# hasenbanck/opus-native

Measured on NVIDIA B200. Metric: concurrent_realtime_48k_streams_decoded, higher is better.
Workload: dtype u32+f32

## Files before the change

opus-native_b200/csrc/frame_warp.cuh:

```cuda
#pragma once
#include "imdct_warp.cuh"
#include "symbols.cuh"

namespace opn {

template <int C> struct WSmp;
template <> struct WSmp<1> {
    float a;
    __device__ __forceinline__ static WSmp ld(const float *p) { return WSmp{*p}; }
    __device__ __forceinline__ WSmp operator+(WSmp o) const { return WSmp{a + o.a}; }
    __device__ __forceinline__ WSmp scaled(float g) const { return WSmp{g * a}; }
};
template <> struct WSmp<2> {
    float a, b;
    __device__ __forceinline__ static WSmp ld(const float *p)
    {
        const float2 v = *reinterpret_cast<const float2 *>(p);
        return WSmp{v.x, v.y};
    }
    __device__ __forceinline__ WSmp operator+(WSmp o) const
    {
        const float2 r = p_add(make_float2(a, b), make_float2(o.a, o.b));
        return WSmp{r.x, r.y};
    }
// ... 55 lines not shown
        rows[i] = v.a;
        if constexpr (C == 2) rows[CHF + i] = v.b;
    }
    __device__ __forceinline__ S ld_hist(int i) const
    {
        int j = pos + i;
        if (j < 0) j += RING_SAMPLES;
        return S::ld(ring + (size_t)j * C);
    }
    __device__ __forceinline__ S ld(int i) const { return i >= 0 ? ld_row(i) : ld_hist(i); }
};

template <int C, int CHF, bool TS = false>
__device__ __forceinline__ void w_comb_ring(const FrameView<C, CHF> &V, int t0, int t1, int n, float g0, float g1, int tap0, int tap1,
                                            int overlap, int lane, const float *win_sq, const CombGains &kg)
{
    using S = WSmp<C>;
    if (g0 == 0.0f && g1 == 0.0f) return;
    t0 = max(t0, 15);
    t1 = max(t1, 15);
    const float g00 = kg.g00, g01 = kg.g01, g02 = kg.g02, g10 = kg.g10, g11 = kg.g11, g12 = kg.g12;
    if (fabsf(g0 - g1) < 1.1920929e-7f && t0 == t1 && tap0 == tap1) overlap = 0;
    const bool has0 = g0 != 0.0f, has1 = g1 != 0.0f;

    if (overlap > 0) {
        const int tmin = min(has0 ? t0 : 1 << 20, has1 ? t1 : 1 << 20);
        const int W = min(tmin - 2, 32);
        for (int base = 0; base < overlap; base += W) {
            const int i = base + lane;
            if (lane < W && i < overlap) {
                const float f = tab_ld<TS>(win_sq + i);
                S a[5], b[5];
#pragma unroll
                for (int k = 0; k < 5; k++) {
                    a[k] = has0 ? V.ld(i - t0 - 2 + k) : S{};
                    b[k] = has1 ? V.ld(i - t1 - 2 + k) : S{};
                }
                V.st_row(i, w_xfade<C>(V.ld_row(i), a, b, has0, has1, f, g00, g01, g02, g10, g11, g12));
            }
            __syncwarp();
        }
    }
    if (!has1) return;

    int at = overlap;
    {
        const int hend = max(at, min(n, t1 - 2));
        for (int base = at; base < hend; base += 128) {
#pragma unroll
            for (int e = 0; e < 4; e++) {
                const int i = base + lane + 32 * e;
                if (i < hend) {
                    int j = V.pos + i - t1 - 2;
                    if (j < 0) j += RING_SAMPLES;
                    if (j + 4 < RING_SAMPLES) {
                        const float *hp = V.ring + (size_t)j * C;
                        V.st_row(i, w_comb5<C>(V.ld_row(i), S::ld(hp + 4 * C), S::ld(hp + 3 * C), S::ld(hp + 2 * C), S::ld(hp + C), S::ld(hp), g10, g11, g12));
                    } else {
                        const int p = i - t1;
                        V.st_row(i, w_comb5<C>(V.ld_row(i), V.ld_hist(p + 2), V.ld_hist(p + 1), V.ld_hist(p), V.ld_hist(p - 1), V.ld_hist(p - 2),
                                               g10, g11, g12));
                    }
                }
            }
        }
        at = hend;
        __syncwarp();
    }
    const int W2 = min(t1 - 2, 128);
    const int rounds = (W2 + 31) >> 5;
    for (int base = at; base < n; base += W2) {
        const bool mixed = base - t1 - 2 < 0;
        for (int e = 0; e < rounds; e++) {
            const int l = lane + 32 * e, i = base + l;
            if (l < W2 && i < n) {
                const int p = i - t1;
                if (mixed)
                    V.st_row(i, w_comb5<C>(V.ld_row(i), V.ld(p + 2), V.ld(p + 1), V.ld(p), V.ld(p - 1), V.ld(p - 2), g10, g11, g12));
                else
                    V.st_row(i, w_comb5<C>(V.ld_row(i), V.ld_row(p + 2), V.ld_row(p + 1), V.ld_row(p), V.ld_row(p - 1), V.ld_row(p - 2), g10,
                                           g11, g12));
            }
        }
        __syncwarp();
    }
}

__device__ __forceinline__ void prefetch_l1(const void *p) { asm volatile("prefetch.global.L1 [%0];" ::"l"(p)); }
__device__ __forceinline__ void prefetch_l2(const void *p) { asm volatile("prefetch.global.L2 [%0];" ::"l"(p)); }

#ifndef OPN_FRAME_WARPS
#define OPN_FRAME_WARPS 5
#endif
#ifndef OPN_FRAME_CTAS
#define OPN_FRAME_CTAS 4
#endif
constexpr int FRAME_WARPS = OPN_FRAME_WARPS, FRAME_CTAS = OPN_FRAME_CTAS;
#ifndef OPN_STORE_UNROLL
#define OPN_STORE_UNROLL 3
#endif
constexpr int STORE_UNROLL = OPN_STORE_UNROLL;
__host__ __device__ constexpr size_t frame_warp_bytes(int lm, int channels) { return (size_t)channels * w_ch_floats(lm) * 4 + 16 + 48; }
__host__ __device__ constexpr size_t frame_smem_bytes(int lm, int channels, size_t blob_bytes)
{
    return 16 + blob_bytes + (size_t)FRAME_WARPS * frame_warp_bytes(lm, channels);
}

enum { FRAME_ROWS = 0, FRAME_SYNTH1 = 1, FRAME_SYNTH2 = 2 };
template <int LM, int C, int MODE, int CS = C>
__device__ __forceinline__ void frame_cta(const FrameArgs &A, uint32_t first_item, uint32_t item_end)
{
    constexpr bool EXPAND = MODE != FRAME_ROWS;
    constexpr int R = C > CS ? C : CS;
    static_assert(EXPAND || CS == C, "coefficient rows from memory are the decoder's channels already");
    extern __shared__ __align__(16) uint8_t smem[];
    constexpr int NF = 120 << LM;
    constexpr int CHF = w_ch_floats(LM);
    const int lane = threadIdx.x & 31, warp = threadIdx.x >> 5;
    uint64_t *tbar = reinterpret_cast<uint64_t *>(smem);
    const uint8_t *blob = smem + 16;
    const FBlobHdr H = g_tab.fblob_hdr[LM][CS - 1];
    float *o = reinterpret_cast<float *>(smem + 16 + H.total + (size_t)warp * frame_warp_bytes(LM, R));
    uint64_t *bar = reinterpret_cast<uint64_t *>(o + R * CHF);
    uint4 *stash = reinterpret_cast<uint4 *>(o + R * CHF + 4);

    if (threadIdx.x == 0) {
        mbar_init(tbar, 1);
        mbar_expect_tx(tbar, H.total);
        bulk_g2s(smem + 16, g_fblob[LM][CS - 1], H.total, tbar);
    }
    const uint32_t item = first_item + warp;
    const bool in_range = item < item_end;
    const uint32_t stream = in_range ? (A.stream_idx ? A.stream_idx[item] : item) : 0u;
    if constexpr (!EXPAND) {
        if (lane == 0 && in_range) {
            mbar_init(bar, 1);
            mbar_expect_tx(bar, C * NF * 4);
#pragma unroll
            for (int c = 0; c < C; c++) bulk_g2s(o + c * CHF, A.coef + ((size_t)stream * C + c) * NF, NF * 4, bar);
        }
    }
    const int32_t status = in_range ? A.status[stream] : -1;
    {
        uint4 v = make_uint4(0u, 0u, 0u, 0u);
        if (in_range) {
            if (lane == 0) v = A.hdr[stream];
            else if (lane == 1) v = *reinterpret_cast<const uint4 *>(A.pf + stream);
            else if (lane == 2) v.x = A.ring_pos[stream];
        }
        if (lane < 3) stash[lane] = v;
    }
    __syncwarp();
    const uint32_t hdr_x = stash[0].x;
    [[maybe_unused]] uint32_t ix0 = 0u, ix1 = 0u, ix2 = 0u;
    if constexpr (MODE == FRAME_SYNTH1) {
        if (in_range) {
            const uint32_t *ip = A.idx + (size_t)stream * SYNTH_MAX_ENTRIES;
            ix0 = __ldg(ip + lane);
            ix1 = __ldg(ip + 32 + lane);
            if (lane < SYNTH_MAX_ENTRIES - 64) ix2 = __ldg(ip + 64 + lane);
        }
    }
    float *carry_g = A.carry + (size_t)stream * C * 60;
    float4 carry = make_float4(0.f, 0.f, 0.f, 0.f);
    if (in_range && lane < 15 * C) carry = *reinterpret_cast<const float4 *>(carry_g + 4 * lane);
    float *ring = A.ring + (size_t)stream * RING_SAMPLES * C;
    if (in_range && status >= 0 && A.postfilter) {
        const int t_old = (int)stash[1].x, t_new = (hdr_x >> 1) & 1u ? (int)(hdr_x >> 16) : 0;
        const int pos0 = (int)stash[2].x;
        const int need = max(max(t_old, t_new), 15) + 2;
        for (int l = lane * (128 / (4 * C)); l < need + 128 / (4 * C); l += 32 * (128 / (4 * C))) {
            int j = pos0 - need + l;
            if (j >= pos0) j = pos0 - 1;
            if (j < 0) j += RING_SAMPLES;
            prefetch_l2(ring + (size_t)j * C);
        }
    }
    if constexpr (EXPAND) {
#pragma unroll
        for (int c = 0; c < R; c++)
            for (int i = lane; i < NF / 4; i += 32) reinterpret_cast<float4 *>(o + c * CHF)[i] = make_float4(0.f, 0.f, 0.f, 0.f);
    }
    __syncthreads();
    mbar_wait(tbar, 0);
    if (status < 0) {
        if (in_range && lane == 0 && A.result) A.result[stream] = status;
        if constexpr (!EXPAND) {
            if (in_range) mbar_wait(bar, 0);
        }
        return;
    }
    const float2 *t_long = reinterpret_cast<const float2 *>(blob + H.tp_long), *t_short = reinterpret_cast<const float2 *>(blob + H.tp_short);
    const float2 *t_tw = reinterpret_cast<const float2 *>(blob + H.tw);
    const float *t_win = reinterpret_cast<const float *>(blob + H.win), *t_winsq = reinterpret_cast<const float *>(blob + H.win_sq);
    const bool lost = status == ITEM_LOST;
    const int lmt = (LM > 0 && ((hdr_x >> 2) & 1u)) ? LM : 0;
    if constexpr (MODE == FRAME_SYNTH1) {
        if (!lost && !(hdr_x & 1u)) {
            const ExpandTables T{reinterpret_cast<const uint32_t *>(blob + H.pvq_u), reinterpret_cast<const uint2 *>(blob + H.pvq_cw),
                                 reinterpret_cast<const uint16_t *>(blob + H.pvq_row), blob + H.pvq_nmax,
                                 reinterpret_cast<const SynthEntry *>(blob + H.ent), blob + H.slots, (int)H.n_slots};
            w_expand<CS>(T, LM, (uint32_t)lane, [&](uint32_t e) {
                const int src = (int)(e & 31u);
                const uint32_t a = __shfl_sync(0xFFFFFFFFu, ix0, src), b2 = __shfl_sync(0xFFFFFFFFu, ix1, src), c2 = __shfl_sync(0xFFFFFFFFu, ix2, src);
                return e == 0xFFu ? 0u : e < 32u ? a : e < 64u ? b2 : c2;
            }, o, CHF, nullptr, lmt);
        }
        __syncwarp();
    } else if constexpr (MODE == FRAME_SYNTH2) {
        if (!lost && !(hdr_x & 1u)) {
            const ExpandTables T{g_tab.pvq_u_data, g_tab.pvq_cw_data, g_tab.pvq_u_row, g_tab.pvq_ev_nmax, nullptr, nullptr, 0};
            w_expand2<CS>(T, LM, (uint32_t)lane, A.parts + (size_t)stream * CELT2_MAX_PARTS, stash[0].w, A.bande + (size_t)stream * 42, o, CHF, nullptr, lmt);
        }
        __syncwarp();
    } else {
        mbar_wait(bar, 0);
    }
    if constexpr (CS == 1 && C == 2) {
        for (int i = lane; i < NF / 4; i += 32) reinterpret_cast<float4 *>(o + CHF)[i] = reinterpret_cast<const float4 *>(o)[i];
        __syncwarp();
    } else if constexpr (CS == 2 && C == 1) {
        for (int i = lane; i < NF / 4; i += 32) {
            const float4 a = reinterpret_cast<const float4 *>(o)[i], b = reinterpret_cast<const float4 *>(o + CHF)[i];
            reinterpret_cast<float4 *>(o)[i] = make_float4(0.5f * (a.x + b.x), 0.5f * (a.y + b.y), 0.5f * (a.z + b.z), 0.5f * (a.w + b.w));
        }
        __syncwarp();
    }
    if constexpr (LM > 0) {
        if ((hdr_x >> 2) & 1u) w_imdct<3, (1 << LM), C, true, EXPAND>(o, lane, carry, t_short, t_tw, t_win);
        else w_imdct<3 - LM, 1, C, true>(o, lane, carry, t_long, t_tw, t_win);
    } else {
        w_imdct<3, 1, C, true>(o, lane, carry, t_long, t_tw, t_win);
    }

    const uint4 hdr = stash[0];
    PfState old;
    {
        const uint4 q = stash[1];
        old.period = (int32_t)q.x;
        old.tapset = (int32_t)q.y;
        old.gain = __uint_as_float(q.z);
        old.pad = 0;
    }
    const uint32_t pos = stash[2].x;
    const int s_on = (hdr.x >> 1) & 1u, s_tapset = (hdr.x >> 4) & 15u, s_gain = (hdr.x >> 8) & 15u, s_period = hdr.x >> 16;
    int t1 = old.period, tap1 = old.tapset;
    float g1 = old.gain;
    if (!lost) {
        t1 = s_on ? s_period : 0;
        g1 = s_on ? 0.09375f * (float)(s_gain + 1) : 0.0f;
        tap1 = s_on ? s_tapset : 0;
    }
    const bool comb_on = A.postfilter && (old.gain != 0.0f || g1 != 0.0f);

    if (lane < 15 * C) {
        const int ch = (C == 2 && lane >= 15) ? 1 : 0;
        *reinterpret_cast<float4 *>(carry_g + 4 * lane) = *reinterpret_cast<const float4 *>(o + ch * CHF + NF + 4 * (lane - 15 * ch));
    }
    if (comb_on) {
        const FrameView<C, CHF> V{o, ring, (int)pos};
        w_comb_ring<C, CHF, true>(V, old.period, t1, NF, old.gain, g1, old.tapset, tap1, 120, lane, t_winsq,
                                  w_comb_gains(old.gain, g1, old.tapset, tap1));
        __syncwarp();
        if (A.hist_samples && lane == 0) atomicAdd(A.hist_samples, (unsigned long long)(C * (max(max(old.period, t1), 15) + 2)));
    }
    const uint32_t dense_off = (A.dense && A.dense_off) ? A.dense_off[item] : 0u;
    float *dense = A.dense ? A.dense + (size_t)stream * A.dense_stride + dense_off : nullptr;
    const float gain = A.gain;
    constexpr int VEC = C == 2 ? NF / 2 : NF / 4;
    constexpr int SPV = C == 2 ? 2 : 4;
    const int wrap_at = (int)(RING_SAMPLES - pos) / SPV;
    float4 *r0 = reinterpret_cast<float4 *>(ring + (size_t)pos * C);
    float4 *r1 = reinterpret_cast<float4 *>(ring) - wrap_at;
#pragma unroll STORE_UNROLL
    for (int i = lane; i < VEC; i += 32) {
        float4 v;
        if (C == 2) {
            const float2 a = *reinterpret_cast<const float2 *>(o + 2 * i), b = *reinterpret_cast<const float2 *>(o + CHF + 2 * i);
            v = make_float4(a.x, b.x, a.y, b.y);
        } else {
            v = *reinterpret_cast<const float4 *>(o + 4 * i);
        }
        (i < wrap_at ? r0 : r1)[i] = v;
        if (dense) {
            if (gain != 1.0f) { v.x *= gain; v.y *= gain; v.z *= gain; v.w *= gain; }
            reinterpret_cast<float4 *>(dense)[i] = v;
        }
    }
    if (lane == 0) {
        uint32_t np = pos + (uint32_t)NF;
        if (np >= RING_SAMPLES) np -= RING_SAMPLES;
        A.ring_pos[stream] = np;
        PfState nw;
        nw.period = t1;
        nw.tapset = tap1;
        nw.gain = g1;
        nw.pad = 0;
        A.pf[stream] = nw;
        if (A.result) A.result[stream] = NF;
        if (A.final_range) A.final_range[stream] = lost ? 0u : hdr.y;
        if (A.softclip_reset && !lost) *reinterpret_cast<float2 *>(A.softclip_reset + 2 * (size_t)stream) = make_float2(0.f, 0.f);
    }
}

template <int LM, int C, int MODE, int CS = C> __global__ void __launch_bounds__(32 * FRAME_WARPS, FRAME_CTAS) k_frame_w(FrameArgs A)
{
    frame_cta<LM, C, MODE, CS>(A, A.item0 + blockIdx.x * FRAME_WARPS, A.item_end);
}

template <int C, int MODE> __global__ void __launch_bounds__(32 * FRAME_WARPS, FRAME_CTAS) k_frame_mix(FrameArgs A)
{
    const MixPlan &P = *A.plan;
    const int g = A.group;
    const uint32_t c = blockIdx.x;
    if (c >= P.cta0[g][4]) return;
    const int j = (c >= P.cta0[g][1]) + (c >= P.cta0[g][2]) + (c >= P.cta0[g][3]), lm = 3 - j;
    const uint32_t first = P.start[g][lm] + (c - P.cta0[g][j]) * FRAME_WARPS, end = P.start[g][lm] + P.count[g][lm];
    switch (lm) {
    case 0: frame_cta<0, C, MODE>(A, first, end); break;
    case 1: frame_cta<1, C, MODE>(A, first, end); break;
    case 2: frame_cta<2, C, MODE>(A, first, end); break;
    default: frame_cta<3, C, MODE>(A, first, end); break;
    }
}

__global__ void __launch_bounds__(256) k_mix_key(MixArgs A)
{
    const uint32_t s = blockIdx.x * 256u + threadIdx.x;
    const bool on = s < A.n_streams;
    uint32_t key = MIX_NO_ITEM;
    int32_t err = 0;
    if (on) {
        const uint32_t len = A.lens[s];
        int lm = -1;
        if (len == 0u) {
            const uint32_t l = A.last_lm[s];
            lm = l != MIX_NO_ITEM ? (int)l : (A.capacity >= 960u ? 3 : A.capacity >= 480u ? 2 : A.capacity >= 240u ? 1 : 0);
        } else {
            const uint32_t toc = A.arena[A.offsets[s]];
            if ((toc & 0x80u) == 0u) err = OPN_ERR_UNIMPLEMENTED;
            else if ((toc & 0x3u) != 0u) err = OPN_ERR_UNIMPLEMENTED;
            else if (((toc & 0x4u) ? 2 : 1) != A.channels) err = OPN_ERR_UNIMPLEMENTED;
            else lm = (int)((toc >> 3) & 0x3u);
        }
        if (lm >= 0 && (120u << lm) > A.capacity) {
            err = OPN_ERR_FRAME_SIZE_TOO_SMALL;
            lm = -1;
        }
        if (lm >= 0) {
            uint32_t g = 0u;
            if (A.n_groups > 1) {
                const uint32_t G = (uint32_t)A.n_groups;
                g = (uint32_t)(((uint64_t)s * G) / A.n_streams);
                if (g + 1u < G && (uint32_t)(((uint64_t)A.n_streams * (g + 1u)) / G) <= s) g += 1u;
            }
            key = g * 4u + (uint32_t)lm;
            if (len > 1u) A.last_lm[s] = (uint8_t)lm;
        }
    }
    const uint32_t peers = __match_any_sync(0xFFFFFFFFu, key);
    uint32_t rank = 0u;
    if (key != MIX_NO_ITEM) {
        const int leader = __ffs(peers) - 1;
        uint32_t base = 0u;
// ... 82 lines not shown
```

opus-native_b200/csrc/host_runtime.cpp:

```cpp
#include <algorithm>
#include <cmath>
#include <cstdio>
#include <cstdlib>
#include <cstring>
#include <new>
#include <string>
#include <vector>

#include <nvtx3/nvToolsExt.h>

#include "opn_internal.h"
#include "celt2.cuh"

using namespace opn;

namespace {

thread_local std::string g_cuda_err;

int cuda_fail(cudaError_t e, const char *what)
{
    char buf[256];
    std::snprintf(buf, sizeof(buf), "%s: %s", what, cudaGetErrorString(e));
    g_cuda_err = buf;
    return OPN_ERR_CUDA;
}

#define CU(call)                                          \
    do {                                                  \
        cudaError_t e_ = (call);                          \
        if (e_ != cudaSuccess) return cuda_fail(e_, #call); \
    } while (0)

int lm_of_frame(size_t nf)
{
    switch (nf) {
    case 120: return 0;
    case 240: return 1;
    case 480: return 2;
    case 960: return 3;
    default: return -1;
    }
}

int select_device(int device)
{
    int n = 0;
    cudaError_t e = cudaGetDeviceCount(&n);
    if (e != cudaSuccess) return cuda_fail(e, "cudaGetDeviceCount");
    if (n == 0 || device < 0 || device >= n) return cuda_fail(cudaErrorInvalidDevice, "no such CUDA device");
    CU(cudaSetDevice(device));
    cudaDeviceProp p;
    CU(cudaGetDeviceProperties(&p, device));
    if (p.major < 10) {
        g_cuda_err = std::string("device '") + p.name + "' is not sm_100-class; libopusb200 ships sm_100a code only";
        return OPN_ERR_CUDA;
    }
    CU(upload_tables(device));
    return OPN_OK;
}

struct EventRing {
    static constexpr int N = 512;
    cudaEvent_t a[N], b[N];
    int used = 0;
    bool made = false;
    double ms = 0.0;
    uint64_t launches = 0;
    int make()
    {
        if (made) return OPN_OK;
        for (int i = 0; i < N; i++) {
            CU(cudaEventCreate(&a[i]));
            CU(cudaEventCreate(&b[i]));
        }
        made = true;
        return OPN_OK;
    }
    int resolve()
    {
        for (int i = 0; i < used; i++) {
            CU(cudaEventSynchronize(b[i]));
            float t = 0;
            CU(cudaEventElapsedTime(&t, a[i], b[i]));
            ms += t;
        }
        used = 0;
        return OPN_OK;
    }
    void destroy()
    {
        if (!made) return;
        for (int i = 0; i < N; i++) {
            cudaEventDestroy(a[i]);
            cudaEventDestroy(b[i]);
        }
        made = false;
    }
};

struct Item {
    uint32_t stream, offset, len, dense_off;
    int lm, wave;
    int cs;
};

}

struct opn_batch {
    int device = 0;
    uint32_t n = 0;
    opn_config cfg{};
    float gain = 1.0f;
    cudaStream_t stream = nullptr;
#ifndef OPN_NSETS
#define OPN_NSETS 8
#endif
#ifndef OPN_NRD
#define OPN_NRD 8
#endif
    static constexpr int NSETS = OPN_NSETS, NRD = OPN_NRD;
    cudaStream_t stream_rd[NRD] = {};
    cudaStream_t stream_ex = nullptr;
#ifndef OPN_FRAME_GROUPS
#define OPN_FRAME_GROUPS 3
#endif
    static constexpr int NGROUPS = OPN_FRAME_GROUPS;
    static constexpr uint32_t GROUP_MIN_ITEMS = 2048;
    cudaStream_t stream_fr[NGROUPS] = {};
    cudaEvent_t ev_fr[NSETS][NGROUPS] = {};
    cudaEvent_t ev_sw = nullptr;
    cudaEvent_t ev_tm[NGROUPS] = {};
    bool fr_pending[NGROUPS] = {};
    int fr_last_set[NGROUPS] = {};
    cudaEvent_t ev_k1[NSETS] = {};
    bool k1_recorded[NSETS] = {};
    bool k1_grouped[NSETS] = {};
    cudaEvent_t ev_rd[NSETS] = {};
    cudaEvent_t ev_ex[NSETS] = {};
    cudaEvent_t ev_in = nullptr;
    static constexpr int MAX_CHUNKS = 8;
    cudaStream_t stream_up = nullptr, stream_dn = nullptr;
    cudaEvent_t ev_chunk[MAX_CHUNKS] = {};
    int set = 0;
    bool unfused = false;
    float *d_carry = nullptr, *d_ring = nullptr, *d_coef[NSETS] = {};
    uint32_t *d_ring_pos = nullptr, *d_final = nullptr, *d_idx[NSETS] = {};
    PfState *d_pf = nullptr;
    uint4 *d_hdr[NSETS] = {};
    int32_t *d_status[NSETS] = {};
    Celt2Part *d_parts[NSETS] = {};
    int16_t *d_bande[NSETS] = {};
    struct Staging {
        uint8_t *d_arena = nullptr;
        size_t arena_cap = 0;
        uint32_t *d_items = nullptr, *h_items = nullptr;
        size_t items_cap = 0;
        float *d_dense = nullptr;
        size_t dense_cap = 0;
        void *d_conv = nullptr;
        size_t conv_cap = 0, conv_esize = 0;
        int32_t *d_cliplen = nullptr, *h_cliplen = nullptr;
        uint32_t *d_trans = nullptr, *h_trans = nullptr;
        cudaEvent_t done = nullptr;
        bool pending = false;
    } stg[2];
    int stg_next = 0;
    float *d_softclip = nullptr;
    uint8_t *d_last_lm = nullptr, *d_mix_key = nullptr;
    uint32_t *d_mix_rank = nullptr;
    uint32_t *d_mix_items[NSETS] = {};
    uint8_t *d_mix_lm[NSETS] = {};
    MixPlan *d_mix_plan[NSETS] = {};
    cudaEvent_t ev_mix[NSETS] = {};
    bool silk = false;
    SilkState d_silk{};
    SilkRec *d_silk_rec[NSETS] = {};
    std::vector<uint8_t> silk_cs;
    unsigned long long *d_hist_samples = nullptr;
    std::vector<int32_t> last_nf, bandwidth, last_duration, have_mode;
    bool timing = false;
    EventRing ev[3];
    uint64_t launches[3] = {0, 0, 0};
};

namespace {

struct Range {
    explicit Range(const char *name) { nvtxRangePushA(name); }
    ~Range() { nvtxRangePop(); }
    Range(const Range &) = delete;
    Range &operator=(const Range &) = delete;
};

int batch_alloc_staging(opn_batch *b, opn_batch::Staging &g, size_t arena_bytes, size_t n_items, size_t dense_floats, size_t conv_esize)
{
    if (!g.done) CU(cudaEventCreateWithFlags(&g.done, cudaEventDisableTiming));
    if (arena_bytes > g.arena_cap) {
        if (g.d_arena) cudaFree(g.d_arena);
        g.arena_cap = arena_bytes + arena_bytes / 4 + 256;
        CU(cudaMalloc(&g.d_arena, g.arena_cap));
    }
    if (n_items > g.items_cap) {
        if (g.d_items) cudaFree(g.d_items);
        if (g.h_items) cudaFreeHost(g.h_items);
        g.items_cap = n_items + n_items / 4 + 64;
        CU(cudaMalloc(&g.d_items, g.items_cap * 4 * sizeof(uint32_t)));
        CU(cudaMallocHost(&g.h_items, g.items_cap * 4 * sizeof(uint32_t)));
    }
    if (dense_floats > g.dense_cap) {
        if (g.d_dense) cudaFree(g.d_dense);
        g.dense_cap = dense_floats;
        CU(cudaMalloc(&g.d_dense, (size_t)b->n * (g.dense_cap + (b->silk ? 240 * (size_t)b->cfg.channels : 0)) * sizeof(float)));
    }
    if (conv_esize && (g.dense_cap > g.conv_cap || conv_esize > g.conv_esize)) {
        if (g.d_conv) cudaFree(g.d_conv);
        g.d_conv = nullptr;
        g.conv_cap = g.dense_cap;
        g.conv_esize = std::max(conv_esize, g.conv_esize);
        CU(cudaMalloc(&g.d_conv, (size_t)b->n * g.conv_cap * g.conv_esize));
    }
    if (conv_esize && !g.d_cliplen) {
        CU(cudaMalloc(&g.d_cliplen, (size_t)b->n * sizeof(int32_t)));
        CU(cudaMallocHost(&g.h_cliplen, (size_t)b->n * sizeof(int32_t)));
    }
    return OPN_OK;
}

int timed_launch(opn_batch *b, int kind, cudaError_t (*fn)(opn_batch *, const void *), const void *args)
{
    EventRing &r = b->ev[kind];
    if (b->timing) {
        if (r.used == EventRing::N) {
            int rc = r.resolve();
            if (rc) return rc;
        }
        CU(cudaEventRecord(r.a[r.used], b->stream));
    }
    CU(fn(b, args));
    if (b->timing) {
        CU(cudaEventRecord(r.b[r.used], b->stream));
        r.used++;
        r.launches++;
    }
    b->launches[kind]++;
    return OPN_OK;
}

cudaError_t do_rangedec(opn_batch *b, const void *a)
{
    const SymbolArgs &s = *static_cast<const SymbolArgs *>(a);
    return b->cfg.bitstream == OPN_BITSTREAM_SYNTH_CELT_2 ? launch_celt2_rangedec(s, b->stream) : launch_synth_rangedec(s, b->stream);
}
cudaError_t do_expand(opn_batch *b, const void *a) { return launch_synth_expand(*static_cast<const SymbolArgs *>(a), b->stream); }
bool frame_grouped(const opn_batch *b, const FrameArgs &m)
{
    return !b->unfused && opn_batch::NGROUPS > 1 && m.n_items >= opn_batch::GROUP_MIN_ITEMS && !m.stream_idx;
}
uint32_t group_first(uint32_t n, int g, int G) { return (uint32_t)((uint64_t)n * (uint32_t)g / (uint32_t)G); }
int mix_groups(const opn_batch *b) { return (opn_batch::NGROUPS > 1 && b->n >= opn_batch::GROUP_MIN_ITEMS) ? opn_batch::NGROUPS : 1; }
cudaError_t do_frame(opn_batch *b, const void *a)
{
    FrameArgs m = *static_cast<const FrameArgs *>(a);
    if (m.plan) {
        const int G = mix_groups(b);
        if (G == 1) return launch_frame_mix(m, b->n, b->stream);
        cudaError_t e = cudaEventRecord(b->ev_sw, b->stream);
        for (int g = 0; g < G && e == cudaSuccess; g++) {
            cudaStream_t st = g == 0 ? b->stream : b->stream_fr[g];
            if (g > 0) e = cudaStreamWaitEvent(st, b->ev_sw, 0);
            m.group = g;
            if (e == cudaSuccess) e = launch_frame_mix(m, group_first(b->n, g + 1, G) - group_first(b->n, g, G), st);
            if (g > 0 && e == cudaSuccess) e = cudaEventRecord(b->ev_tm[g], st);
            if (g > 0 && e == cudaSuccess) e = cudaStreamWaitEvent(b->stream, b->ev_tm[g], 0);
        }
        return e;
    }
    if (!frame_grouped(b, m)) return launch_frame(m, b->stream);
    cudaError_t e = cudaEventRecord(b->ev_sw, b->stream);
    const uint32_t n_items = m.n_items;
    for (int g = 0; g < opn_batch::NGROUPS && e == cudaSuccess; g++) {
        cudaStream_t st = g == 0 ? b->stream : b->stream_fr[g];
        if (g > 0) e = cudaStreamWaitEvent(st, b->ev_sw, 0);
        m.item0 = (uint32_t)((uint64_t)n_items * g / opn_batch::NGROUPS);
        m.item_end = (uint32_t)((uint64_t)n_items * (g + 1) / opn_batch::NGROUPS);
        if (e == cudaSuccess) e = launch_frame(m, st);
        if (g > 0 && e == cudaSuccess) e = cudaEventRecord(b->ev_tm[g], st);
        if (g > 0 && e == cudaSuccess) e = cudaStreamWaitEvent(b->stream, b->ev_tm[g], 0);
    }
    return e;
}

int join_groups(opn_batch *b)
{
    for (int g = 1; g < opn_batch::NGROUPS; g++)
        if (b->fr_pending[g]) {
            CU(cudaStreamWaitEvent(b->stream, b->ev_fr[b->fr_last_set[g]][g], 0));
            b->fr_pending[g] = false;
        }
    return OPN_OK;
}

int sync_pipeline(opn_batch *b)
{
    for (int q = 0; q < opn_batch::NRD; q++) CU(cudaStreamSynchronize(b->stream_rd[q]));
    CU(cudaStreamSynchronize(b->stream_ex));
    for (int g = 1; g < opn_batch::NGROUPS; g++) {
        CU(cudaStreamSynchronize(b->stream_fr[g]));
        b->fr_pending[g] = false;
    }
    CU(cudaStreamSynchronize(b->stream_up));
    CU(cudaStreamSynchronize(b->stream));
    CU(cudaStreamSynchronize(b->stream_dn));
    return OPN_OK;
}

int run_bucket(opn_batch *b, const uint8_t *d_arena, const uint32_t *d_offsets, const uint32_t *d_lens,
               const uint32_t *d_stream_idx, const uint32_t *d_dense_off, uint32_t n_items, int lm, int has_toc,
               uint32_t pkt_cap, float *dense, size_t dense_stride, int32_t *d_result, int inputs_on, bool softclip_reset,
               int stream_channels = 0)
{
    Range nv("opn: step (range decode + frame kernel)");
    if (stream_channels == 0) stream_channels = b->cfg.channels;
    if (stream_channels != b->cfg.channels && b->unfused) return OPN_ERR_UNIMPLEMENTED;
    const int p = b->set;
    b->set = (p + 1) % opn_batch::NSETS;
    cudaStream_t srd = b->stream_rd[p % opn_batch::NRD];
    SymbolArgs s{};
    s.arena = d_arena;
    s.offsets = d_offsets;
    s.lens = d_lens;
    s.stream_idx = d_stream_idx;
    s.n_items = n_items;
    s.lm = lm;
    s.channels = stream_channels;
    s.has_toc = has_toc;
    s.side = nullptr;
    s.hdr = b->d_hdr[p];
    s.status = b->d_status[p];
    s.coef = b->unfused ? b->d_coef[p] : nullptr;
    s.y_out = nullptr;
    s.idx = b->d_idx[p];
    s.pkt_cap = pkt_cap;
    s.parts = b->d_parts[p];
    s.bande = b->d_bande[p];
    s.side2 = nullptr;
    const bool celt2 = b->cfg.bitstream == OPN_BITSTREAM_SYNTH_CELT_2;
    int rc;
    if (b->timing) {
        if (inputs_on == 2) {
            CU(cudaEventRecord(b->ev_in, b->stream_up));
            CU(cudaStreamWaitEvent(b->stream, b->ev_in, 0));
        }
        rc = timed_launch(b, 0, do_rangedec, &s);
        if (rc) return rc;
        if (b->unfused) {
            rc = timed_launch(b, 2, do_expand, &s);
            if (rc) return rc;
        }
    } else {
        if (inputs_on == 1) {
            CU(cudaEventRecord(b->ev_in, b->stream));
            CU(cudaStreamWaitEvent(srd, b->ev_in, 0));
        } else if (inputs_on == 2) {
            CU(cudaEventRecord(b->ev_in, b->stream_up));
            CU(cudaStreamWaitEvent(srd, b->ev_in, 0));
        }
        if (b->k1_recorded[p]) {
            CU(cudaStreamWaitEvent(srd, b->ev_k1[p], 0));
            if (b->k1_grouped[p])
                for (int g = 1; g < opn_batch::NGROUPS; g++) CU(cudaStreamWaitEvent(srd, b->ev_fr[p][g], 0));
        }
        CU(celt2 ? launch_celt2_rangedec(s, srd) : launch_synth_rangedec(s, srd));
        CU(cudaEventRecord(b->ev_rd[p], srd));
        b->launches[0]++;
        if (b->unfused) {
            CU(cudaStreamWaitEvent(b->stream_ex, b->ev_rd[p], 0));
            CU(launch_synth_expand(s, b->stream_ex));
            CU(cudaEventRecord(b->ev_ex[p], b->stream_ex));
            CU(cudaStreamWaitEvent(b->stream, b->ev_ex[p], 0));
            b->launches[2]++;
        } else {
            CU(cudaStreamWaitEvent(b->stream, b->ev_rd[p], 0));
        }
    }
    FrameArgs m{};
    m.coef = b->unfused ? b->d_coef[p] : nullptr;
    m.idx = celt2 ? nullptr : b->d_idx[p];
    m.parts = celt2 ? b->d_parts[p] : nullptr;
    m.bande = b->d_bande[p];
    m.hdr = b->d_hdr[p];
    m.status = b->d_status[p];
    m.stream_idx = d_stream_idx;
    m.dense_off = d_dense_off;
    m.n_items = n_items;
    m.item0 = 0;
    m.item_end = n_items;
    m.lm = lm;
    m.channels = b->cfg.channels;
    m.stream_channels = stream_channels;
    m.postfilter = b->cfg.postfilter;
    m.carry = b->d_carry;
    m.ring = b->d_ring;
    m.ring_pos = b->d_ring_pos;
    m.pf = b->d_pf;
    m.dense = dense;
    m.dense_stride = dense_stride;
    m.gain = b->gain;
    m.result = d_result;
    m.final_range = b->d_final;
    m.softclip_reset = softclip_reset ? b->d_softclip : nullptr;
    m.hist_samples = b->timing ? b->d_hist_samples : nullptr;
    const bool grouped = !b->timing && frame_grouped(b, m);
    if (b->timing) {
        rc = join_groups(b);
        if (rc) return rc;
        rc = timed_launch(b, 1, do_frame, &m);
        if (rc) return rc;
        if (frame_grouped(b, m)) b->launches[1] += opn_batch::NGROUPS - 1;
    } else if (!grouped) {
        rc = join_groups(b);
        if (rc) return rc;
        CU(launch_frame(m, b->stream));
        b->launches[1]++;
    } else {
        CU(cudaEventRecord(b->ev_sw, b->stream));
        for (int g = 0; g < opn_batch::NGROUPS; g++) {
            cudaStream_t st = g == 0 ? b->stream : b->stream_fr[g];
            if (g > 0) {
                if (!b->fr_pending[g]) CU(cudaStreamWaitEvent(st, b->ev_sw, 0));
                CU(cudaStreamWaitEvent(st, b->ev_rd[p], 0));
            }
            m.item0 = (uint32_t)((uint64_t)n_items * g / opn_batch::NGROUPS);
            m.item_end = (uint32_t)((uint64_t)n_items * (g + 1) / opn_batch::NGROUPS);
            CU(launch_frame(m, st));
            b->launches[1]++;
            if (g > 0) {
                CU(cudaEventRecord(b->ev_fr[p][g], st));
                b->fr_pending[g] = true;
                b->fr_last_set[g] = p;
            }
        }
    }
    CU(cudaEventRecord(b->ev_k1[p], b->stream));
    b->k1_recorded[p] = true;
    b->k1_grouped[p] = grouped;
    return OPN_OK;
}

cudaError_t do_silk_rangedec(opn_batch *b, const void *a) { return launch_silk_rangedec(*static_cast<const SilkArgs *>(a), b->stream); }
cudaError_t do_silk_frame(opn_batch *b, const void *a) { return launch_silk_frame(*static_cast<const SilkArgs *>(a), b->stream); }

int run_silk_bucket(opn_batch *b, const uint8_t *d_arena, const uint32_t *d_offsets, const uint32_t *d_lens, const uint32_t *d_stream_idx,
                    const uint32_t *d_dense_off, uint32_t n_items, int frame_ms, int has_toc, int bandwidth, int stream_channels,
                    float *dense, size_t dense_stride, int32_t *d_result, int inputs_on, bool softclip_reset, int fec = 0)
{
    Range nv("opn: SILK step (range decode + frame kernel)");
    if (!b->silk) return OPN_ERR_UNIMPLEMENTED;
    const int p = b->set;
    b->set = (p + 1) % opn_batch::NSETS;
    cudaStream_t srd = b->stream_rd[p % opn_batch::NRD];
    SilkArgs a{};
    a.arena = d_arena;
    a.offsets = d_offsets;
    a.lens = d_lens;
    a.stream_idx = d_stream_idx;
    a.n_items = n_items;
    a.frame_ms = frame_ms;
    a.stream_channels = stream_channels;
    a.channels = b->cfg.channels;
    a.has_toc = has_toc;
    a.bandwidth = bandwidth;
    a.fec = fec;
    a.rec = b->d_silk_rec[p];
    a.hdr = b->d_hdr[p];
    a.status = b->d_status[p];
    a.st = b->d_silk;
    a.ring = b->d_ring;
    a.ring_pos = b->d_ring_pos;
    a.dense = dense;
    a.dense_stride = dense_stride;
    a.dense_off = d_dense_off;
    a.gain = b->gain;
    a.result = d_result;
    a.final_range = b->d_final;
    a.softclip_reset = softclip_reset ? b->d_softclip : nullptr;
    const bool grouped = !b->timing && opn_batch::NGROUPS > 1 && !d_stream_idx && n_items == b->n && n_items >= opn_batch::GROUP_MIN_ITEMS;
    int rc = OPN_OK;
    if (!grouped) rc = join_groups(b);
    if (rc) return rc;
    if (b->timing) {
        if (inputs_on == 2) {
            CU(cudaEventRecord(b->ev_in, b->stream_up));
            CU(cudaStreamWaitEvent(b->stream, b->ev_in, 0));
        }
        rc = timed_launch(b, 0, do_silk_rangedec, &a);
        if (rc) return rc;
        rc = timed_launch(b, 1, do_silk_frame, &a);
        if (rc) return rc;
    } else {
        if (inputs_on == 1) {
            CU(cudaEventRecord(b->ev_in, b->stream));
            CU(cudaStreamWaitEvent(srd, b->ev_in, 0));
        } else if (inputs_on == 2) {
            CU(cudaEventRecord(b->ev_in, b->stream_up));
            CU(cudaStreamWaitEvent(srd, b->ev_in, 0));
        }
        if (b->k1_recorded[p]) {
            CU(cudaStreamWaitEvent(srd, b->ev_k1[p], 0));
            if (b->k1_grouped[p])
                for (int g = 1; g < opn_batch::NGROUPS; g++) CU(cudaStreamWaitEvent(srd, b->ev_fr[p][g], 0));
        }
        CU(launch_silk_rangedec(a, srd));
        CU(cudaEventRecord(b->ev_rd[p], srd));
        b->launches[0]++;
        if (!grouped) {
            CU(cudaStreamWaitEvent(b->stream, b->ev_rd[p], 0));
            CU(launch_silk_frame(a, b->stream));
            b->launches[1]++;
        } else {
            CU(cudaEventRecord(b->ev_sw, b->stream));
            for (int g = 0; g < opn_batch::NGROUPS; g++) {
                cudaStream_t st = g == 0 ? b->stream : b->stream_fr[g];
                if (g > 0 && !b->fr_pending[g]) CU(cudaStreamWaitEvent(st, b->ev_sw, 0));
                CU(cudaStreamWaitEvent(st, b->ev_rd[p], 0));
                a.item0 = group_first(n_items, g, opn_batch::NGROUPS);
                a.item_end = group_first(n_items, g + 1, opn_batch::NGROUPS);
                CU(launch_silk_frame(a, st));
                b->launches[1]++;
                if (g > 0) {
                    CU(cudaEventRecord(b->ev_fr[p][g], st));
                    b->fr_pending[g] = true;
                    b->fr_last_set[g] = p;
                }
            }
        }
    }
    CU(cudaEventRecord(b->ev_k1[p], b->stream));
    b->k1_recorded[p] = true;
    b->k1_grouped[p] = grouped;
    return OPN_OK;
}

int mix_alloc(opn_batch *b)
{
    if (b->d_last_lm) return OPN_OK;
    const size_t n = b->n, cap = mix_item_cap(b->n);
    CU(cudaMalloc(&b->d_mix_key, n));
    CU(cudaMalloc(&b->d_mix_rank, n * sizeof(uint32_t)));
    for (int q = 0; q < opn_batch::NSETS; q++) {
        CU(cudaMalloc(&b->d_mix_items[q], 3 * cap * sizeof(uint32_t)));
        CU(cudaMalloc(&b->d_mix_lm[q], cap));
        CU(cudaMalloc(&b->d_mix_plan[q], sizeof(MixPlan)));
        CU(cudaEventCreateWithFlags(&b->ev_mix[q], cudaEventDisableTiming));
    }
    uint8_t *p = nullptr;
    CU(cudaMalloc(&p, n));
    CU(cudaMemsetAsync(p, MIX_NO_ITEM, n, b->stream_ex));
    b->d_last_lm = p;
    return OPN_OK;
}

int run_mixed(opn_batch *b, const uint8_t *d_arena, const uint32_t *d_offsets, const uint32_t *d_lens, size_t capacity, float *dense,
              size_t dense_stride, int32_t *d_result, int inputs_on, bool softclip_reset)
{
    if (b->unfused) return OPN_ERR_UNIMPLEMENTED;
    Range nv("opn: mixed-frame step (bucketing + range decode + frame kernel)");
    int rc = mix_alloc(b);
    if (rc) return rc;
    const int p = b->set;
    b->set = (p + 1) % opn_batch::NSETS;
    cudaStream_t srd = b->stream_rd[p % opn_batch::NRD];
    const uint32_t cap = mix_item_cap(b->n);
    const int G = mix_groups(b);
    MixArgs x{};
    x.arena = d_arena;
    x.offsets = d_offsets;
    x.lens = d_lens;
    x.n_streams = b->n;
    x.channels = b->cfg.channels;
    x.n_groups = G;
    x.capacity = (uint32_t)std::min<size_t>(capacity, 1u << 20);
    x.last_lm = b->d_last_lm;
    x.key = b->d_mix_key;
    x.rank = b->d_mix_rank;
    x.plan = b->d_mix_plan[p];
    x.item_offsets = b->d_mix_items[p];
    x.item_lens = b->d_mix_items[p] + cap;
    x.item_stream = b->d_mix_items[p] + 2 * (size_t)cap;
    x.item_lm = b->d_mix_lm[p];
    x.result = d_result;
    SymbolArgs s{};
    s.arena = d_arena;
    s.offsets = x.item_offsets;
    s.lens = x.item_lens;
    s.stream_idx = x.item_stream;
    s.item_lm = x.item_lm;
    s.n_items = cap;
    s.lm = 0;
    s.channels = b->cfg.channels;
    s.has_toc = 1;
    s.hdr = b->d_hdr[p];
    s.status = b->d_status[p];
    s.idx = b->d_idx[p];
    s.pkt_cap = 1280u;
    s.parts = b->d_parts[p];
    s.bande = b->d_bande[p];
    const bool celt2 = b->cfg.bitstream == OPN_BITSTREAM_SYNTH_CELT_2;
    FrameArgs m{};
    m.idx = celt2 ? nullptr : b->d_idx[p];
    m.parts = celt2 ? b->d_parts[p] : nullptr;
    m.bande = b->d_bande[p];
    m.hdr = b->d_hdr[p];
    m.status = b->d_status[p];
    m.stream_idx = x.item_stream;
    m.n_items = cap;
    m.channels = b->cfg.channels;
    m.postfilter = b->cfg.postfilter;
    m.carry = b->d_carry;
    m.ring = b->d_ring;
    m.ring_pos = b->d_ring_pos;
    m.pf = b->d_pf;
    m.dense = dense;
    m.dense_stride = dense_stride;
    m.gain = b->gain;
    m.result = d_result;
    m.final_range = b->d_final;
    m.softclip_reset = softclip_reset ? b->d_softclip : nullptr;
    m.hist_samples = b->timing ? b->d_hist_samples : nullptr;
    m.plan = b->d_mix_plan[p];
    if (b->timing) {
        rc = join_groups(b);
        if (rc) return rc;
        CU(cudaStreamSynchronize(b->stream_ex));
        CU(launch_mix_plan(x, b->stream));
        b->launches[2] += 2;
        rc = timed_launch(b, 0, do_rangedec, &s);
        if (rc) return rc;
        rc = timed_launch(b, 1, do_frame, &m);
        if (rc) return rc;
        b->launches[1] += G - 1;
    } else {
        cudaStream_t sx = b->stream_ex;
        if (inputs_on == 1) {
            CU(cudaEventRecord(b->ev_in, b->stream));
            CU(cudaStreamWaitEvent(sx, b->ev_in, 0));
        }
        if (b->k1_recorded[p]) {
            CU(cudaStreamWaitEvent(sx, b->ev_k1[p], 0));
            if (b->k1_grouped[p])
                for (int g = 1; g < opn_batch::NGROUPS; g++) CU(cudaStreamWaitEvent(sx, b->ev_fr[p][g], 0));
        }
        CU(launch_mix_plan(x, sx));
        b->launches[2] += 2;
        CU(cudaEventRecord(b->ev_mix[p], sx));
        CU(cudaStreamWaitEvent(srd, b->ev_mix[p], 0));
        CU(celt2 ? launch_celt2_rangedec(s, srd) : launch_synth_rangedec(s, srd));
        CU(cudaEventRecord(b->ev_rd[p], srd));
        b->launches[0]++;
        if (G == 1) {
            rc = join_groups(b);
            if (rc) return rc;
            CU(cudaStreamWaitEvent(b->stream, b->ev_rd[p], 0));
            CU(launch_frame_mix(m, b->n, b->stream));
            b->launches[1]++;
        } else {
            CU(cudaEventRecord(b->ev_sw, b->stream));
            for (int g = 0; g < G; g++) {
                cudaStream_t st = g == 0 ? b->stream : b->stream_fr[g];
                if (g > 0 && !b->fr_pending[g]) CU(cudaStreamWaitEvent(st, b->ev_sw, 0));
                CU(cudaStreamWaitEvent(st, b->ev_rd[p], 0));
                m.group = g;
                CU(launch_frame_mix(m, group_first(b->n, g + 1, G) - group_first(b->n, g, G), st));
                b->launches[1]++;
                if (g > 0) {
                    CU(cudaEventRecord(b->ev_fr[p][g], st));
                    b->fr_pending[g] = true;
                    b->fr_last_set[g] = p;
                }
            }
        }
    }
    CU(cudaEventRecord(b->ev_k1[p], b->stream));
    b->k1_recorded[p] = true;
    b->k1_grouped[p] = !b->timing && G > 1;
    return OPN_OK;
}

void plc_frames(size_t frame_size, int32_t last_nf, std::vector<uint32_t> &out)
{
    size_t done = 0;
    while (done < frame_size) {
        size_t a = std::min(frame_size - done, (size_t)last_nf);
        if (a > 960) a = 960;
        else if (a < 960) {
            if (a > 480) a = 480;
            else if (a > 240 && a < 480) a = 240;
        }
        out.push_back((uint32_t)a);
        done += a;
    }
}

}

extern "C" {

const char *opn_strerror(int code)
{
    switch (code) {
    case OPN_OK: return "ok";
    case OPN_ERR_BAD_ARG: return "bad arguments";
    case OPN_ERR_BUFFER_TOO_SMALL: return "buffer is too small";
    case OPN_ERR_INTERNAL: return "internal error";
    case OPN_ERR_INVALID_PACKET: return "invalid packet";
    case OPN_ERR_FRAME_SIZE_TOO_SMALL: return "the frame size is too small for the packet";
    case OPN_ERR_UNIMPLEMENTED: return "not implemented (the reference crate stubs this path too)";
    case OPN_ERR_CUDA: return "CUDA error";
    default: return "unknown error";
    }
}

const char *opn_last_cuda_error(void) { return g_cuda_err.c_str(); }

int opn_device_count(void)
{
    int n = 0;
    if (cudaGetDeviceCount(&n) != cudaSuccess) return 0;
    return n;
}

void *opn_host_alloc(size_t bytes)
{
    void *p = nullptr;
    if (bytes == 0 || cudaMallocHost(&p, bytes) != cudaSuccess) {
        cudaGetLastError();
        return nullptr;
    }
    return p;
}

void opn_host_free(void *p)
{
    if (p) cudaFreeHost(p);
}

int opn_host_register(void *p, size_t bytes)
{
    if (!p || bytes == 0) return OPN_ERR_BAD_ARG;
    CU(cudaHostRegister(p, bytes, cudaHostRegisterPortable));
    return OPN_OK;
}

int opn_host_unregister(void *p)
{
    if (!p) return OPN_ERR_BAD_ARG;
    CU(cudaHostUnregister(p));
    return OPN_OK;
}

int opn_batch_create(int device, uint32_t n_streams, const opn_config *cfg, opn_batch **out)
{
    if (!out || !cfg || n_streams == 0) return OPN_ERR_BAD_ARG;
    if (cfg->channels < 1 || cfg->channels > 2) return OPN_ERR_BAD_ARG;
    if (cfg->bitstream & ~(OPN_BITSTREAM_CELT_MASK | OPN_BITSTREAM_SYNTH_SILK_1)) return OPN_ERR_BAD_ARG;
    const int32_t celt_bitstream = cfg->bitstream & OPN_BITSTREAM_CELT_MASK;
    if (celt_bitstream != OPN_BITSTREAM_OPUS && celt_bitstream != OPN_BITSTREAM_SYNTH_CELT_1 && celt_bitstream != OPN_BITSTREAM_SYNTH_CELT_2)
        return OPN_ERR_BAD_ARG;
    switch (cfg->fs_hz) {
    case 48000: break;
    case 8000: case 12000: case 16000: case 24000: return OPN_ERR_UNIMPLEMENTED;
    default: return OPN_ERR_BAD_ARG;
    }
    int rc = select_device(device);
    if (rc) return rc;
    if (kernels_frame_groups() != OPN_FRAME_GROUPS) return OPN_ERR_INTERNAL;
    opn_batch *b = new (std::nothrow) opn_batch();
    if (!b) return OPN_ERR_INTERNAL;
    b->device = device;
    b->n = n_streams;
    b->cfg = *cfg;
    b->cfg.bitstream = celt_bitstream;
    b->silk = (cfg->bitstream & OPN_BITSTREAM_SYNTH_SILK_1) != 0;
    b->gain = host_gain_from_q8(cfg->gain_q8);
    const char *uf = std::getenv("OPN_UNFUSED_EXPAND");
    b->unfused = uf && uf[0] == '1' && celt_bitstream == OPN_BITSTREAM_SYNTH_CELT_1;
    const size_t n = n_streams, C = (size_t)cfg->channels;
    cudaError_t e = cudaStreamCreateWithFlags(&b->stream, cudaStreamNonBlocking);
    {
        const char *pr = std::getenv("OPN_RD_PRIORITY");
        const bool high = pr ? pr[0] == '1' : celt_bitstream == OPN_BITSTREAM_SYNTH_CELT_2;
        int lo_p = 0, hi_p = 0;
        if (high) cudaDeviceGetStreamPriorityRange(&lo_p, &hi_p);
        for (int q = 0; q < opn_batch::NRD && e == cudaSuccess; q++)
            e = cudaStreamCreateWithPriority(&b->stream_rd[q], cudaStreamNonBlocking, high ? hi_p : 0);
    }
    for (int q = 0; q < opn_batch::NSETS && e == cudaSuccess; q++) {
        e = cudaEventCreateWithFlags(&b->ev_rd[q], cudaEventDisableTiming);
        if (e == cudaSuccess) e = cudaEventCreateWithFlags(&b->ev_ex[q], cudaEventDisableTiming);
        if (e == cudaSuccess) e = cudaEventCreateWithFlags(&b->ev_k1[q], cudaEventDisableTiming);
        for (int g = 1; g < opn_batch::NGROUPS && e == cudaSuccess; g++) e = cudaEventCreateWithFlags(&b->ev_fr[q][g], cudaEventDisableTiming);
        if (e == cudaSuccess) e = cudaMalloc(&b->d_idx[q], n * 72 * sizeof(uint32_t));
        if (e == cudaSuccess && b->unfused) e = cudaMalloc(&b->d_coef[q], n * C * 960 * sizeof(float));
        if (e == cudaSuccess) e = cudaMalloc(&b->d_hdr[q], n * sizeof(uint4));
        if (e == cudaSuccess && celt_bitstream == OPN_BITSTREAM_SYNTH_CELT_2) e = cudaMalloc(&b->d_parts[q], n * CELT2_MAX_PARTS * sizeof(Celt2Part));
        if (e == cudaSuccess && b->silk) e = cudaMalloc(&b->d_silk_rec[q], n * 2 * sizeof(SilkRec));
        if (e == cudaSuccess && celt_bitstream == OPN_BITSTREAM_SYNTH_CELT_2) e = cudaMalloc(&b->d_bande[q], n * 42 * sizeof(int16_t));
        if (e == cudaSuccess) e = cudaMalloc(&b->d_status[q], n * sizeof(int32_t));
    }
    if (e == cudaSuccess) e = cudaStreamCreateWithFlags(&b->stream_ex, cudaStreamNonBlocking);
    for (int g = 1; g < opn_batch::NGROUPS && e == cudaSuccess; g++) e = cudaStreamCreateWithFlags(&b->stream_fr[g], cudaStreamNonBlocking);
    if (e == cudaSuccess) e = cudaEventCreateWithFlags(&b->ev_sw, cudaEventDisableTiming);
    for (int g = 1; g < opn_batch::NGROUPS && e == cudaSuccess; g++) e = cudaEventCreateWithFlags(&b->ev_tm[g], cudaEventDisableTiming);
    if (e == cudaSuccess) e = cudaEventCreateWithFlags(&b->ev_in, cudaEventDisableTiming);
    if (e == cudaSuccess) e = cudaStreamCreateWithFlags(&b->stream_up, cudaStreamNonBlocking);
    if (e == cudaSuccess) e = cudaStreamCreateWithFlags(&b->stream_dn, cudaStreamNonBlocking);
    for (int q = 0; q < opn_batch::MAX_CHUNKS && e == cudaSuccess; q++) e = cudaEventCreateWithFlags(&b->ev_chunk[q], cudaEventDisableTiming);
    if (e == cudaSuccess) e = cudaMalloc(&b->d_carry, n * C * 60 * sizeof(float));
    if (e == cudaSuccess) e = cudaMalloc(&b->d_ring, n * C * RING_SAMPLES * sizeof(float));
    if (e == cudaSuccess) e = cudaMalloc(&b->d_ring_pos, n * sizeof(uint32_t));
    if (e == cudaSuccess) e = cudaMalloc(&b->d_final, n * sizeof(uint32_t));
    if (e == cudaSuccess) e = cudaMalloc(&b->d_pf, n * sizeof(PfState));
    if (e == cudaSuccess) e = cudaMalloc(&b->d_softclip, n * 2 * sizeof(float));
    if (b->silk) {
        if (e == cudaSuccess) e = cudaMalloc(&b->d_silk.slpc, n * 2 * 16 * sizeof(int32_t));
        if (e == cudaSuccess) e = cudaMalloc(&b->d_silk.hist, n * 2 * SILK_HIST * sizeof(int32_t));
        if (e == cudaSuccess) e = cudaMalloc(&b->d_silk.a_q12, n * 2 * 16 * sizeof(int16_t));
        if (e == cudaSuccess) e = cudaMalloc(&b->d_silk.gain, n * 2 * sizeof(int32_t));
        if (e == cudaSuccess) e = cudaMalloc(&b->d_silk.rs, n * 2 * 8 * sizeof(float));
        if (e == cudaSuccess) e = cudaMalloc(&b->d_silk.fs, n * 2);
    }
    if (e == cudaSuccess) e = cudaMalloc(&b->d_hist_samples, sizeof(unsigned long long));
    if (e == cudaSuccess) e = cudaMemset(b->d_hist_samples, 0, sizeof(unsigned long long));
    if (e != cudaSuccess) {
        opn_batch_destroy(b);
        return cuda_fail(e, "opn_batch_create: allocation");
    }
    b->last_nf.assign(n, 120);
    b->bandwidth.assign(n, -1);
    b->last_duration.assign(n, -1);
    b->have_mode.assign(n, 0);
    b->silk_cs.assign(n, 0);
    *out = b;
    rc = opn_batch_reset(b);
    if (rc) {
        opn_batch_destroy(b);
        *out = nullptr;
    }
    return rc;
}

void opn_batch_destroy(opn_batch *b)
{
    if (!b) return;
    cudaSetDevice(b->device);
    for (int q = 0; q < opn_batch::NRD; q++)
        if (b->stream_rd[q]) cudaStreamSynchronize(b->stream_rd[q]);
    for (cudaStream_t st : {b->stream_ex, b->stream_up, b->stream, b->stream_dn})
        if (st) cudaStreamSynchronize(st);
    for (int g = 1; g < opn_batch::NGROUPS; g++)
        if (b->stream_fr[g]) {
            cudaStreamSynchronize(b->stream_fr[g]);
            cudaStreamDestroy(b->stream_fr[g]);
        }
    if (b->ev_sw) cudaEventDestroy(b->ev_sw);
    for (int g = 1; g < opn_batch::NGROUPS; g++)
        if (b->ev_tm[g]) cudaEventDestroy(b->ev_tm[g]);
    for (int q = 0; q < opn_batch::NSETS; q++) {
        for (int g = 1; g < opn_batch::NGROUPS; g++)
            if (b->ev_fr[q][g]) cudaEventDestroy(b->ev_fr[q][g]);
        if (b->ev_rd[q]) cudaEventDestroy(b->ev_rd[q]);
        if (b->ev_ex[q]) cudaEventDestroy(b->ev_ex[q]);
        if (b->ev_k1[q]) cudaEventDestroy(b->ev_k1[q]);
        cudaFree(b->d_idx[q]);
        cudaFree(b->d_coef[q]);
        cudaFree(b->d_hdr[q]);
        cudaFree(b->d_parts[q]);
        cudaFree(b->d_bande[q]);
        cudaFree(b->d_status[q]);
        cudaFree(b->d_silk_rec[q]);
    }
    cudaFree(b->d_silk.slpc);
    cudaFree(b->d_silk.hist);
    cudaFree(b->d_silk.a_q12);
    cudaFree(b->d_silk.gain);
    cudaFree(b->d_silk.rs);
    cudaFree(b->d_silk.fs);
    if (b->ev_in) cudaEventDestroy(b->ev_in);
    for (int q = 0; q < opn_batch::MAX_CHUNKS; q++)
        if (b->ev_chunk[q]) cudaEventDestroy(b->ev_chunk[q]);
    for (cudaStream_t st : {b->stream_ex, b->stream_up, b->stream_dn})
        if (st) cudaStreamDestroy(st);
    for (int q = 0; q < opn_batch::NRD; q++)
        if (b->stream_rd[q]) cudaStreamDestroy(b->stream_rd[q]);
    for (int k = 0; k < 3; k++) b->ev[k].destroy();
    cudaFree(b->d_carry);
    cudaFree(b->d_ring);
    cudaFree(b->d_ring_pos);
    cudaFree(b->d_final);
    cudaFree(b->d_pf);
    cudaFree(b->d_softclip);
    cudaFree(b->d_last_lm);
    cudaFree(b->d_mix_key);
    cudaFree(b->d_mix_rank);
    for (int q = 0; q < opn_batch::NSETS; q++) {
        cudaFree(b->d_mix_items[q]);
        cudaFree(b->d_mix_lm[q]);
        cudaFree(b->d_mix_plan[q]);
        if (b->ev_mix[q]) cudaEventDestroy(b->ev_mix[q]);
    }
    cudaFree(b->d_hist_samples);
    for (auto &g : b->stg) {
        cudaFree(g.d_arena);
        cudaFree(g.d_items);
        cudaFree(g.d_dense);
        cudaFree(g.d_conv);
        cudaFree(g.d_cliplen);
        cudaFree(g.d_trans);
        if (g.h_trans) cudaFreeHost(g.h_trans);
        if (g.h_cliplen) cudaFreeHost(g.h_cliplen);
        if (g.h_items) cudaFreeHost(g.h_items);
        if (g.done) cudaEventDestroy(g.done);
    }
    if (b->stream) cudaStreamDestroy(b->stream);
    delete b;
}

int opn_batch_reset(opn_batch *b)
{
    if (!b) return OPN_ERR_BAD_ARG;
    CU(cudaSetDevice(b->device));
    int rc = sync_pipeline(b);
    if (rc) return rc;
    for (auto &g : b->stg) g.pending = false;
    const size_t n = b->n, C = (size_t)b->cfg.channels;
    CU(cudaMemsetAsync(b->d_carry, 0, n * C * 60 * sizeof(float), b->stream));
    CU(cudaMemsetAsync(b->d_ring, 0, n * C * RING_SAMPLES * sizeof(float), b->stream));
    CU(cudaMemsetAsync(b->d_ring_pos, 0, n * sizeof(uint32_t), b->stream));
    CU(cudaMemsetAsync(b->d_final, 0, n * sizeof(uint32_t), b->stream));
    CU(cudaMemsetAsync(b->d_pf, 0, n * sizeof(PfState), b->stream));
    for (int q = 0; q < opn_batch::NSETS; q++) {
        CU(cudaMemsetAsync(b->d_hdr[q], 0, n * sizeof(uint4), b->stream));
        CU(cudaMemsetAsync(b->d_status[q], 0, n * sizeof(int32_t), b->stream));
        b->k1_recorded[q] = false;
    }
    b->set = 0;
    CU(cudaMemsetAsync(b->d_softclip, 0, n * 2 * sizeof(float), b->stream));
    if (b->d_last_lm) CU(cudaMemsetAsync(b->d_last_lm, MIX_NO_ITEM, n, b->stream));
    if (b->silk) {
        CU(cudaMemsetAsync(b->d_silk.slpc, 0, n * 2 * 16 * sizeof(int32_t), b->stream));
        CU(cudaMemsetAsync(b->d_silk.hist, 0, n * 2 * SILK_HIST * sizeof(int32_t), b->stream));
        CU(cudaMemsetAsync(b->d_silk.a_q12, 0, n * 2 * 16 * sizeof(int16_t), b->stream));
        CU(cudaMemsetAsync(b->d_silk.gain, 0, n * 2 * sizeof(int32_t), b->stream));
        CU(cudaMemsetAsync(b->d_silk.rs, 0, n * 2 * 8 * sizeof(float), b->stream));
        CU(cudaMemsetAsync(b->d_silk.fs, 0, n * 2, b->stream));
    }
    CU(cudaStreamSynchronize(b->stream));
    std::fill(b->last_nf.begin(), b->last_nf.end(), 120);
    std::fill(b->bandwidth.begin(), b->bandwidth.end(), -1);
    std::fill(b->last_duration.begin(), b->last_duration.end(), -1);
    std::fill(b->have_mode.begin(), b->have_mode.end(), 0);
    std::fill(b->silk_cs.begin(), b->silk_cs.end(), 0);
    return OPN_OK;
}

static int batch_decode_host(opn_batch *b, const uint8_t *arena, const uint32_t *offsets, const uint32_t *lens, float *pcm,
                             size_t pcm_stride, size_t frame_size, int32_t *results, uint32_t flags,
                             void *pcm_conv = nullptr, int sample_format = OPN_SAMPLE_F32)
{
    Range nv_call("opn: host-buffer call (parse, upload, decode, download)");
    const uint32_t n = b->n;
    const int C = b->cfg.channels;
    size_t arena_end = 0, items_ub = 0;
    for (uint32_t i = 0; i < n; i++) {
        if (lens[i] == 0) {
            items_ub += frame_size / 120;
            continue;
        }
        arena_end = std::max(arena_end, (size_t)offsets[i] + lens[i]);
        const int fc = opn_packet_frame_count(arena + offsets[i], lens[i]);
        items_ub += (fc > 0 ? (size_t)fc : 1) + (b->silk ? 1 : 0);
    }
    const size_t dense_stride = (frame_size * (size_t)C + 3) & ~(size_t)3;
    const int slot = b->stg_next;
    b->stg_next ^= 1;
    opn_batch::Staging &g = b->stg[slot];
    if (g.pending) {
        CU(cudaEventSynchronize(g.done));
        g.pending = false;
    }
    const size_t esize = pcm_conv ? opn_sample_size(sample_format) : 0;
    if (pcm_conv && esize == 0) return OPN_ERR_BAD_ARG;
    int rc = batch_alloc_staging(b, g, arena_end, items_ub, dense_stride, esize);
    if (rc) return rc;
    const bool want_pcm = (pcm != nullptr || pcm_conv != nullptr) && !(flags & OPN_FLAG_NO_PCM_COPY);
    if (arena_end) CU(cudaMemcpyAsync(g.d_arena, arena, arena_end, cudaMemcpyHostToDevice, b->stream_up));

    const uint32_t n_chunks = std::min<uint32_t>(opn_batch::MAX_CHUNKS, std::max<uint32_t>(1u, n / 1024u));
    const size_t cap = g.items_cap;
    std::vector<Item> items;
    items.reserve(items_ub / n_chunks + 64);
    std::vector<int32_t> res(n, 0);
    std::vector<uint32_t> plc;
    std::vector<uint32_t> silk_resets, celt_resets;
    size_t kbase = 0;
    for (uint32_t ch = 0; ch < n_chunks; ch++) {
        const uint32_t s0 = (uint32_t)((uint64_t)n * ch / n_chunks), s1 = (uint32_t)((uint64_t)n * (ch + 1) / n_chunks);
        Range nv_chunk("opn: chunk (host parse -> enqueue)");
        items.clear();
        silk_resets.clear();
        celt_resets.clear();
        bool any_gap = false;
        uint32_t max_len = 8;
        for (uint32_t i = s0; i < s1; i++) {
            const uint32_t len = lens[i];
            auto conceal = [&](uint32_t i, size_t n_samples, uint32_t at0, int w0) -> int {
                if (!b->have_mode[i]) return -1;
                plc.clear();
                plc_frames(n_samples, b->last_nf[i], plc);
                uint32_t at = at0;
                int w = w0;
                if (b->have_mode[i] == 1 + OPN_MODE_SILK) {
                    bool ok = b->silk;
                    for (uint32_t a : plc) ok = ok && (a == 480 || a == 960);
                    if (!ok) return -2;
                    for (uint32_t a : plc) {
                        items.push_back(Item{i, 0u, 0u, at * (uint32_t)C, 8 + (a == 960 ? 1 : 0), w++, (int)b->silk_cs[i]});
// ... 544 lines not shown
    CU(cudaMemcpy(out, dOut.p, (size_t)n_packets * n_ops * sizeof(opn_op_out), cudaMemcpyDeviceToHost));
    if (y_out && y_stride) CU(cudaMemcpy(y_out, dY.p, (size_t)n_packets * y_stride * 4, cudaMemcpyDeviceToHost));
    return OPN_OK;
}

int opn_op_imdct_tdac(int device, const float *input, size_t in_stride, float *output, size_t out_stride, uint32_t n_rows,
                      int shift, int stride, int blocks)
{
    if (!input || !output || n_rows == 0 || shift < 0 || shift > 3 || blocks < 1 || stride != blocks) return OPN_ERR_BAD_ARG;
    const size_t n2 = 960u >> shift;
    if (n2 * (size_t)blocks > 960 || in_stride < n2 * (size_t)blocks || out_stride < n2 * (size_t)blocks + 60) return OPN_ERR_BAD_ARG;
    int rc = select_device(device);
    if (rc) return rc;
    DevBuf dI, dO;
    CU(dI.alloc((size_t)n_rows * in_stride * 4));
    CU(dO.alloc((size_t)n_rows * out_stride * 4));
    CU(cudaMemcpy(dI.p, input, (size_t)n_rows * in_stride * 4, cudaMemcpyHostToDevice));
    CU(cudaMemcpy(dO.p, output, (size_t)n_rows * out_stride * 4, cudaMemcpyHostToDevice));
    CU(launch_op_imdct(dI.as<float>(), in_stride, dO.as<float>(), out_stride, n_rows, shift, blocks, nullptr));
    CU(cudaDeviceSynchronize());
    CU(cudaMemcpy(output, dO.p, (size_t)n_rows * out_stride * 4, cudaMemcpyDeviceToHost));
    return OPN_OK;
}

static int comb_args_ok(size_t offset, size_t n, uint32_t n_rows, const int32_t *p, const float *g, size_t row_stride,
                        size_t overlap)
{
    if (!p || !g || n_rows == 0 || offset + n > row_stride || overlap > 120 || overlap > n) return 0;
    for (uint32_t r = 0; r < n_rows; r++) {
        const int32_t t0 = std::max(p[4 * r], 15), t1 = std::max(p[4 * r + 1], 15);
        if (t0 > 1022 || t1 > 1022 || p[4 * r + 2] < 0 || p[4 * r + 2] > 2 || p[4 * r + 3] < 0 || p[4 * r + 3] > 2) return 0;
        if ((size_t)std::max(t0, t1) + 2 > offset) return 0;
    }
    return 1;
}

int opn_op_comb_filter_inplace(int device, float *y, size_t row_stride, size_t y_offset, size_t n, uint32_t n_rows,
                               const int32_t *params4, const float *gains2, size_t overlap)
{
    if (!y || !comb_args_ok(y_offset, n, n_rows, params4, gains2, row_stride, overlap)) return OPN_ERR_BAD_ARG;
    int rc = select_device(device);
    if (rc) return rc;
    DevBuf dY, dP, dG;
    CU(dY.alloc((size_t)n_rows * row_stride * 4));
    CU(dP.alloc((size_t)n_rows * 16));
    CU(dG.alloc((size_t)n_rows * 8));
    CU(cudaMemcpy(dY.p, y, (size_t)n_rows * row_stride * 4, cudaMemcpyHostToDevice));
    CU(cudaMemcpy(dP.p, params4, (size_t)n_rows * 16, cudaMemcpyHostToDevice));
    CU(cudaMemcpy(dG.p, gains2, (size_t)n_rows * 8, cudaMemcpyHostToDevice));
    CU(launch_op_comb_inplace(dY.as<float>(), row_stride, (int)y_offset, (int)n, n_rows, dP.as<int32_t>(), dG.as<float>(),
                              (int)overlap, nullptr));
    CU(cudaDeviceSynchronize());
    CU(cudaMemcpy(y, dY.p, (size_t)n_rows * row_stride * 4, cudaMemcpyDeviceToHost));
    return OPN_OK;
}

int opn_op_comb_filter(int device, float *y, const float *x, size_t row_stride, size_t offset, size_t n, uint32_t n_rows,
                       const int32_t *params4, const float *gains2, size_t overlap)
{
    if (!y || !x || !comb_args_ok(offset, n, n_rows, params4, gains2, row_stride, overlap)) return OPN_ERR_BAD_ARG;
    int rc = select_device(device);
    if (rc) return rc;
    DevBuf dY, dX, dP, dG;
    CU(dY.alloc((size_t)n_rows * row_stride * 4));
    CU(dX.alloc((size_t)n_rows * row_stride * 4));
    CU(dP.alloc((size_t)n_rows * 16));
    CU(dG.alloc((size_t)n_rows * 8));
    CU(cudaMemcpy(dY.p, y, (size_t)n_rows * row_stride * 4, cudaMemcpyHostToDevice));
    CU(cudaMemcpy(dX.p, x, (size_t)n_rows * row_stride * 4, cudaMemcpyHostToDevice));
    CU(cudaMemcpy(dP.p, params4, (size_t)n_rows * 16, cudaMemcpyHostToDevice));
    CU(cudaMemcpy(dG.p, gains2, (size_t)n_rows * 8, cudaMemcpyHostToDevice));
    CU(launch_op_comb(dY.as<float>(), dX.as<float>(), row_stride, (int)offset, (int)n, n_rows, dP.as<int32_t>(), dG.as<float>(),
                      (int)overlap, nullptr));
    CU(cudaDeviceSynchronize());
    CU(cudaMemcpy(y, dY.p, (size_t)n_rows * row_stride * 4, cudaMemcpyDeviceToHost));
    return OPN_OK;
}

int opn_op_pcm_soft_clip(int device, float *pcm, size_t row_stride, size_t row_len, int channels, uint32_t n_rows,
                         float *softclip_mem)
{
    if (!pcm || !softclip_mem || n_rows == 0 || channels < 1 || row_len > row_stride) return OPN_ERR_BAD_ARG;
    int rc = select_device(device);
    if (rc) return rc;
    DevBuf dP, dM;
    CU(dP.alloc((size_t)n_rows * row_stride * 4));
    CU(dM.alloc((size_t)n_rows * channels * 4));
    CU(cudaMemcpy(dP.p, pcm, (size_t)n_rows * row_stride * 4, cudaMemcpyHostToDevice));
    CU(cudaMemcpy(dM.p, softclip_mem, (size_t)n_rows * channels * 4, cudaMemcpyHostToDevice));
    CU(launch_op_soft_clip(dP.as<float>(), row_stride, row_len, channels, n_rows, dM.as<float>(), nullptr));
    CU(cudaDeviceSynchronize());
    CU(cudaMemcpy(pcm, dP.p, (size_t)n_rows * row_stride * 4, cudaMemcpyDeviceToHost));
    CU(cudaMemcpy(softclip_mem, dM.p, (size_t)n_rows * channels * 4, cudaMemcpyDeviceToHost));
    return OPN_OK;
}

int opn_op_smooth_fade(int device, const float *in1, const float *in2, float *out, size_t row_stride, size_t overlap, int channels,
                       int32_t fs_hz, uint32_t n_rows)
{
    if (!in1 || !in2 || !out || n_rows == 0 || channels < 1 || channels > 2 || overlap * (size_t)channels > row_stride) return OPN_ERR_BAD_ARG;
    if (fs_hz <= 0 || 48000 % fs_hz != 0 || (overlap > 0 && (overlap - 1) * (size_t)(48000 / fs_hz) >= 120)) return OPN_ERR_BAD_ARG;
    int rc = select_device(device);
    if (rc) return rc;
    const size_t bytes = (size_t)n_rows * row_stride * 4;
    DevBuf d1, d2;
    CU(d1.alloc(bytes));
    CU(d2.alloc(bytes));
    CU(cudaMemcpy(d1.p, in1, bytes, cudaMemcpyHostToDevice));
    CU(cudaMemcpy(d2.p, in2, bytes, cudaMemcpyHostToDevice));
    CU(launch_op_smooth_fade(d1.as<float>(), d2.as<float>(), d1.as<float>(), row_stride, (int)overlap, channels, fs_hz, n_rows, nullptr));
    CU(cudaDeviceSynchronize());
    CU(cudaMemcpy(out, d1.p, bytes, cudaMemcpyDeviceToHost));
    return OPN_OK;
}

int opn_op_bitexact_trig(int device, const int16_t *x, int16_t *cos_out, uint32_t n_cos, const int32_t *isin, const int32_t *icos,
                         int32_t *log2tan_out, uint32_t n_log2tan)
{
    if ((n_cos && (!x || !cos_out)) || (n_log2tan && (!isin || !icos || !log2tan_out))) return OPN_ERR_BAD_ARG;
    int rc = select_device(device);
    if (rc) return rc;
    DevBuf dX, dC, dS, dK, dL;
    CU(dX.alloc((size_t)n_cos * 2));
    CU(dC.alloc((size_t)n_cos * 2));
    CU(dS.alloc((size_t)n_log2tan * 4));
    CU(dK.alloc((size_t)n_log2tan * 4));
    CU(dL.alloc((size_t)n_log2tan * 4));
    if (n_cos) CU(cudaMemcpy(dX.p, x, (size_t)n_cos * 2, cudaMemcpyHostToDevice));
    if (n_log2tan) {
        CU(cudaMemcpy(dS.p, isin, (size_t)n_log2tan * 4, cudaMemcpyHostToDevice));
        CU(cudaMemcpy(dK.p, icos, (size_t)n_log2tan * 4, cudaMemcpyHostToDevice));
    }
    CU(launch_op_bitexact_trig(dX.as<int16_t>(), dC.as<int16_t>(), n_cos, dS.as<int32_t>(), dK.as<int32_t>(), dL.as<int32_t>(),
                               n_log2tan, nullptr));
    CU(cudaDeviceSynchronize());
    if (n_cos) CU(cudaMemcpy(cos_out, dC.p, (size_t)n_cos * 2, cudaMemcpyDeviceToHost));
    if (n_log2tan) CU(cudaMemcpy(log2tan_out, dL.p, (size_t)n_log2tan * 4, cudaMemcpyDeviceToHost));
    return OPN_OK;
}

int opn_op_synth_symbols(int device, const uint8_t *arena, const uint32_t *offsets, const uint32_t *lens, uint32_t n_packets,
                         int lm, int channels, opn_synth_side *side_out, int32_t *y_out, float *coef_out)
{
    if (!arena || !offsets || !lens || n_packets == 0 || lm < 0 || lm > 3 || channels < 1 || channels > 2) return OPN_ERR_BAD_ARG;
    int rc = select_device(device);
    if (rc) return rc;
    size_t arena_end = 0;
    uint32_t max_len = 8;
    for (uint32_t i = 0; i < n_packets; i++) {
        arena_end = std::max(arena_end, (size_t)offsets[i] + lens[i]);
        max_len = std::max(max_len, lens[i]);
    }
    const size_t row = (size_t)channels * (120u << lm);
    DevBuf dA, dO, dL, dS, dSt, dY, dC, dI, dH;
    CU(dA.alloc(arena_end));
    CU(dO.alloc(n_packets * 4));
    CU(dL.alloc(n_packets * 4));
    CU(dS.alloc((size_t)n_packets * sizeof(opn_synth_side)));
    CU(dSt.alloc(n_packets * 4));
    CU(dH.alloc((size_t)n_packets * sizeof(uint4)));
    CU(dY.alloc((size_t)n_packets * row * 4));
    CU(dC.alloc((size_t)n_packets * row * 4));
    CU(dI.alloc((size_t)n_packets * 72 * 4));
    CU(cudaMemcpy(dA.p, arena, arena_end, cudaMemcpyHostToDevice));
    CU(cudaMemcpy(dO.p, offsets, n_packets * 4, cudaMemcpyHostToDevice));
    CU(cudaMemcpy(dL.p, lens, n_packets * 4, cudaMemcpyHostToDevice));
    CU(cudaMemset(dS.p, 0, (size_t)n_packets * sizeof(opn_synth_side)));
    SymbolArgs s{};
    s.arena = dA.as<uint8_t>();
    s.offsets = dO.as<uint32_t>();
    s.lens = dL.as<uint32_t>();
    s.n_items = n_packets;
    s.lm = lm;
    s.channels = channels;
    s.has_toc = 0;
    s.side = dS.as<opn_synth_side>();
    s.hdr = dH.as<uint4>();
    s.status = dSt.as<int32_t>();
    s.coef = dC.as<float>();
    s.y_out = dY.as<int32_t>();
    s.idx = dI.as<uint32_t>();
    s.pkt_cap = (max_len + 15u) & ~15u;
    CU(launch_synth_symbols(s, nullptr));
    CU(cudaDeviceSynchronize());
    if (side_out) CU(cudaMemcpy(side_out, dS.p, (size_t)n_packets * sizeof(opn_synth_side), cudaMemcpyDeviceToHost));
    if (y_out) CU(cudaMemcpy(y_out, dY.p, (size_t)n_packets * row * 4, cudaMemcpyDeviceToHost));
    if (coef_out) CU(cudaMemcpy(coef_out, dC.p, (size_t)n_packets * row * 4, cudaMemcpyDeviceToHost));
    return OPN_OK;
}

int opn_op_celt2_symbols(int device, const uint8_t *arena, const uint32_t *offsets, const uint32_t *lens, uint32_t n_packets,
                         int lm, int channels, opn_celt2_side *side_out, int32_t *y_out, float *coef_out)
{
    if (!arena || !offsets || !lens || n_packets == 0 || lm < 0 || lm > 3 || channels < 1 || channels > 2) return OPN_ERR_BAD_ARG;
    int rc = select_device(device);
    if (rc) return rc;
    size_t arena_end = 0;
    for (uint32_t i = 0; i < n_packets; i++) arena_end = std::max(arena_end, (size_t)offsets[i] + lens[i]);
    const size_t row = (size_t)channels * (120u << lm);
    DevBuf dA, dO, dL, dS, dSt, dY, dC, dH, dP, dE;
    CU(dE.alloc((size_t)n_packets * 42 * sizeof(int16_t)));
    CU(dA.alloc(arena_end + 8));
    CU(dO.alloc(n_packets * 4));
    CU(dL.alloc(n_packets * 4));
    CU(dS.alloc((size_t)n_packets * sizeof(Celt2Side)));
    CU(dSt.alloc(n_packets * 4));
    CU(dH.alloc((size_t)n_packets * sizeof(uint4)));
    CU(dP.alloc((size_t)n_packets * CELT2_MAX_PARTS * sizeof(Celt2Part)));
    CU(dY.alloc((size_t)n_packets * row * 4));
    CU(dC.alloc((size_t)n_packets * row * 4));
    CU(cudaMemcpy(dA.p, arena, arena_end, cudaMemcpyHostToDevice));
    CU(cudaMemcpy(dO.p, offsets, n_packets * 4, cudaMemcpyHostToDevice));
    CU(cudaMemcpy(dL.p, lens, n_packets * 4, cudaMemcpyHostToDevice));
    CU(cudaMemset(dY.p, 0, (size_t)n_packets * row * 4));
    CU(cudaMemset(dC.p, 0, (size_t)n_packets * row * 4));
    SymbolArgs s{};
    s.arena = dA.as<uint8_t>();
    s.offsets = dO.as<uint32_t>();
    s.lens = dL.as<uint32_t>();
    s.n_items = n_packets;
    s.lm = lm;
    s.channels = channels;
    s.has_toc = 0;
    s.hdr = dH.as<uint4>();
    s.status = dSt.as<int32_t>();
    s.coef = dC.as<float>();
    s.y_out = dY.as<int32_t>();
    s.parts = dP.as<Celt2Part>();
    s.side2 = dS.as<Celt2Side>();
    s.bande = dE.as<int16_t>();
    CU(launch_celt2_rangedec(s, nullptr));
    CU(launch_celt2_expand(s, nullptr));
    CU(cudaDeviceSynchronize());
    if (side_out) CU(cudaMemcpy(side_out, dS.p, (size_t)n_packets * sizeof(Celt2Side), cudaMemcpyDeviceToHost));
    if (y_out) CU(cudaMemcpy(y_out, dY.p, (size_t)n_packets * row * 4, cudaMemcpyDeviceToHost));
    if (coef_out) CU(cudaMemcpy(coef_out, dC.p, (size_t)n_packets * row * 4, cudaMemcpyDeviceToHost));
    return OPN_OK;
}

int opn_op_silk_frames(int device, const uint8_t *arena, const uint32_t *offsets, const uint32_t *lens, uint32_t n_packets,
                       int stream_channels, int channels, size_t frame_size, int decode_fec, opn_silk_side *side_out, int32_t *exc_out,
                       int16_t *out16, float *pcm_out, int32_t *result)
{
    if (!arena || !offsets || !lens || n_packets == 0 || channels < 1 || channels > 2 || stream_channels < 1 || stream_channels > 2)
        return OPN_ERR_BAD_ARG;
    if (frame_size != 480 && frame_size != 960) return OPN_ERR_BAD_ARG;
    int rc = select_device(device);
    if (rc) return rc;
    size_t arena_end = 0;
    for (uint32_t i = 0; i < n_packets; i++) arena_end = std::max(arena_end, (size_t)offsets[i] + lens[i]);
    const size_t n = n_packets, row = frame_size * (size_t)channels;
    DevBuf dA, dO, dL, dS, dSt, dH, dR, dX, dY, dP, dRes, dRing, dPos, dFin;
    DevBuf sL, sH, sA, sG, sR, sF;
    CU(dA.alloc(arena_end + 8));
    CU(dO.alloc(n * 4));
    CU(dL.alloc(n * 4));
    CU(dS.alloc(n * sizeof(opn_silk_side)));
    CU(dSt.alloc(n * 4));
    CU(dH.alloc(n * sizeof(uint4)));
    CU(dR.alloc(n * 2 * sizeof(SilkRec)));
    CU(dX.alloc(n * 2 * SILK_MAX_FRAME * 4));
    CU(dY.alloc(n * 2 * SILK_MAX_FRAME * 2));
    CU(dP.alloc(n * row * 4));
    CU(dRes.alloc(n * 4));
    CU(dRing.alloc(n * (size_t)channels * RING_SAMPLES * 4));
    CU(dPos.alloc(n * 4));
    CU(dFin.alloc(n * 4));
    CU(sL.alloc(n * 2 * 16 * 4));
    CU(sH.alloc(n * 2 * SILK_HIST * 4));
    CU(sA.alloc(n * 2 * 16 * 2));
    CU(sG.alloc(n * 2 * 4));
    CU(sR.alloc(n * 2 * 8 * 4));
    CU(sF.alloc(n * 2));
    CU(cudaMemcpy(dA.p, arena, arena_end, cudaMemcpyHostToDevice));
    CU(cudaMemcpy(dO.p, offsets, n * 4, cudaMemcpyHostToDevice));
    CU(cudaMemcpy(dL.p, lens, n * 4, cudaMemcpyHostToDevice));
    CU(cudaMemset(dS.p, 0, n * sizeof(opn_silk_side)));
    CU(cudaMemset(dX.p, 0, n * 2 * SILK_MAX_FRAME * 4));
    CU(cudaMemset(dY.p, 0, n * 2 * SILK_MAX_FRAME * 2));
    CU(cudaMemset(dP.p, 0, n * row * 4));
    CU(cudaMemset(dPos.p, 0, n * 4));
    CU(cudaMemset(sL.p, 0, n * 2 * 16 * 4));
    CU(cudaMemset(sH.p, 0, n * 2 * SILK_HIST * 4));
    CU(cudaMemset(sA.p, 0, n * 2 * 16 * 2));
    CU(cudaMemset(sG.p, 0, n * 2 * 4));
    CU(cudaMemset(sR.p, 0, n * 2 * 8 * 4));
    CU(cudaMemset(sF.p, 0, n * 2));
    SilkArgs a{};
    a.arena = dA.as<uint8_t>();
    a.offsets = dO.as<uint32_t>();
    a.lens = dL.as<uint32_t>();
    a.n_items = n_packets;
    a.frame_ms = frame_size == 960 ? 20 : 10;
    a.stream_channels = stream_channels;
    a.channels = channels;
    a.has_toc = 1;
    a.bandwidth = -1;
    a.fec = decode_fec ? 1 : 0;
    a.rec = dR.as<SilkRec>();
    a.hdr = dH.as<uint4>();
    a.status = dSt.as<int32_t>();
    a.st = SilkState{sL.as<int32_t>(), sH.as<int32_t>(), sA.as<int16_t>(), sG.as<int32_t>(), sR.as<float>(), sF.as<uint8_t>()};
    a.ring = dRing.as<float>();
    a.ring_pos = dPos.as<uint32_t>();
    a.dense = dP.as<float>();
    a.dense_stride = row;
    a.gain = 1.0f;
    a.result = dRes.as<int32_t>();
    a.final_range = dFin.as<uint32_t>();
    a.side = dS.as<opn_silk_side>();
    a.exc_out = dX.as<int32_t>();
    a.out16 = dY.as<int16_t>();
    CU(launch_silk_rangedec(a, nullptr));
    CU(launch_silk_frame(a, nullptr));
    CU(cudaDeviceSynchronize());
    if (side_out) CU(cudaMemcpy(side_out, dS.p, n * sizeof(opn_silk_side), cudaMemcpyDeviceToHost));
    if (exc_out) CU(cudaMemcpy(exc_out, dX.p, n * 2 * SILK_MAX_FRAME * 4, cudaMemcpyDeviceToHost));
    if (out16) CU(cudaMemcpy(out16, dY.p, n * 2 * SILK_MAX_FRAME * 2, cudaMemcpyDeviceToHost));
    if (pcm_out) CU(cudaMemcpy(pcm_out, dP.p, n * row * 4, cudaMemcpyDeviceToHost));
    if (result) CU(cudaMemcpy(result, dRes.p, n * 4, cudaMemcpyDeviceToHost));
    return OPN_OK;
}

}
```

opus-native_b200/csrc/opn_device.cuh:

```cuda
#pragma once
#include <cuda_runtime.h>
#include <stdint.h>

#include "../../include/opusb200.h"

namespace opn {

struct alignas(16) SynthEntry {
    uint32_t ft_minus1;
    uint32_t magic;
    uint16_t base;
    uint16_t ft1;
    uint8_t n, k;
    uint8_t ftb;
    uint8_t sh;
};
constexpr int SYNTH_MAX_ENTRIES = 72;
constexpr int SYNTH_SLOTS = 3;

struct FBlobHdr {
    uint16_t tp_long;
    uint16_t tp_short;
    uint16_t tw;
    uint16_t win;
    uint16_t win_sq;
    uint16_t pvq_u;
    uint16_t pvq_cw;
    uint16_t pvq_row;
    uint16_t pvq_nmax;
    uint16_t ent;
    uint16_t slots;
    uint16_t total;
    uint16_t n_slots, n_entries, cols, pad;
};
constexpr int FBLOB_MAX_BYTES = 20 * 1024;

struct DevTables {
    float trig[1800];
    float window[120];
    float window_sq[120];
    float2 twiddles[480];
    float2 trig_pair[900];
    uint16_t bitrev[4][480];
    alignas(16) uint32_t pvq_u_data[1272];
    uint16_t pvq_u_row[16];
    alignas(16) uint2 pvq_cw_data[1272];
    uint8_t pvq_ev_nmax[16];
    uint8_t e_bands[24];
    uint8_t synth_sched[4][21][3];
    SynthEntry synth_entries[4][2][SYNTH_MAX_ENTRIES];
    uint8_t synth_n_entries[4][2];
    uint8_t synth_entry_of[4][2][2 * 960];
    uint8_t synth_slot_entries[4][2][SYNTH_SLOTS][32];
    uint8_t synth_slot_maxn[4][2][SYNTH_SLOTS];
    uint8_t synth_n_slots[4][2];
    uint8_t tapset_icdf[4];
    float comb_gains[9];
    FBlobHdr fblob_hdr[4][2];
    uint8_t log_n[24];
    uint8_t alloc_vectors[232];
    int16_t cache_index[106];
    uint8_t cache_bits[392];
    uint8_t cache_caps[168];
    uint8_t log2_frac[24];
};

__device__ DevTables g_tab;
__device__ __align__(128) uint8_t g_fblob[4][2][FBLOB_MAX_BYTES];
__device__ float g_exp2_q9[512];

}
```

opus-native_b200/csrc/opn_internal.h:

```cpp
#pragma once
#include <cuda_runtime.h>
#include <stddef.h>
#include <stdint.h>

#include "../../include/opusb200.h"

namespace opn {

struct Celt2Part;
struct Celt2Side;

constexpr int SYM_WARPS_PER_CTA = 4;
#ifndef OPN_RD_WARPS
#define OPN_RD_WARPS 1
#endif
constexpr int RANGEDEC_WARPS_PER_CTA = OPN_RD_WARPS;
#ifndef OPN_EXPAND_WARPS
#define OPN_EXPAND_WARPS 4
#endif
constexpr int EXPAND_WARPS_PER_CTA = OPN_EXPAND_WARPS;
constexpr int IM_TPC = 128;
constexpr int RING_SAMPLES = 2880;
constexpr int32_t ITEM_OK = 0, ITEM_LOST = 1;

struct PfState {
    int32_t period, tapset;
    float gain;
    int32_t pad;
};

__host__ __device__ inline uint32_t hdr_pack(uint32_t silence, uint32_t postfilter, uint32_t transient, uint32_t intra, uint32_t tapset,
                                             uint32_t gain_idx, uint32_t octave, uint32_t period)
{
    return silence | postfilter << 1 | transient << 2 | intra << 3 | tapset << 4 | gain_idx << 8 | octave << 12 | period << 16;
}

#ifndef OPN_FRAME_GROUPS
#define OPN_FRAME_GROUPS 3
#endif
constexpr int MIX_GROUPS = OPN_FRAME_GROUPS > 1 ? OPN_FRAME_GROUPS : 1;
constexpr uint32_t MIX_PAD = 32u * OPN_RD_WARPS;
constexpr uint8_t MIX_NO_ITEM = 0xFF;
struct MixPlan {
    uint32_t count[MIX_GROUPS][4];
    uint32_t start[MIX_GROUPS][4];
    uint32_t cta0[MIX_GROUPS][5];
    uint32_t items_padded;
};
__host__ __device__ constexpr uint32_t mix_item_cap(uint32_t n_streams) { return n_streams + MIX_GROUPS * 4u * MIX_PAD; }

struct SymbolArgs {
    const uint8_t *arena;
    const uint32_t *offsets;
    const uint32_t *lens;
    const uint32_t *stream_idx;
    uint32_t n_items;
    int lm, channels, has_toc;
    opn_synth_side *side;
    uint4 *hdr;
    int32_t *status;
    float *coef;
    int32_t *y_out;
    uint32_t *idx;
    uint32_t pkt_cap;
    struct Celt2Part *parts;
    struct Celt2Side *side2;
    int16_t *bande;
    const uint8_t *item_lm;
};

struct FrameArgs {
    const float *coef;
    const uint32_t *idx;
    const struct Celt2Part *parts;
    const uint4 *hdr;
    const int32_t *status;
    const uint32_t *stream_idx;
    uint32_t n_items;
    uint32_t item0, item_end;
    int lm, channels, postfilter;
    int stream_channels;
    float *carry;
    float *ring;
    uint32_t *ring_pos;
    PfState *pf;
    float *dense;
    size_t dense_stride;
    const uint32_t *dense_off;
    float gain;
    int32_t *result;
    uint32_t *final_range;
    float *softclip_reset;
    unsigned long long *hist_samples;
    const int16_t *bande;
    const MixPlan *plan;
    int group;
};

struct MixArgs {
    const uint8_t *arena;
    const uint32_t *offsets, *lens;
    uint32_t n_streams;
    int channels, n_groups;
    uint32_t capacity;
    uint8_t *last_lm;
    uint8_t *key;
    uint32_t *rank;
    MixPlan *plan;
    uint32_t *item_offsets, *item_lens, *item_stream;
    uint8_t *item_lm;
    int32_t *result;
};

constexpr int SILK_MAX_FRAME = 320;
constexpr int SILK_HIST = 320;
constexpr int SILK_ROWS = 32;
constexpr int SILK_WARPS = 8;
constexpr int SILK_RS = 33;

struct alignas(16) SilkRec {
    uint32_t index[20];
    uint16_t lag[4];
    uint8_t pulses[20];
    uint8_t rc[16];
    uint8_t gidx[4], ltp[4];
    uint8_t type, seed, pad[2];
    uint32_t pad2[2];
};
static_assert(sizeof(SilkRec) == 144, "SilkRec layout");

struct SilkState {
    int32_t *slpc;
    int32_t *hist;
    int16_t *a_q12;
    int32_t *gain;
    float *rs;
    uint8_t *fs;
};

struct SilkArgs {
    const uint8_t *arena;
    const uint32_t *offsets, *lens, *stream_idx;
    uint32_t n_items;
    uint32_t item0, item_end;
    int frame_ms;
    int stream_channels;
    int channels;
    int has_toc;
    int bandwidth;
    int fec;
    SilkRec *rec;
    uint4 *hdr;
    int32_t *status;
    SilkState st;
    float *ring;
    uint32_t *ring_pos;
    float *dense;
    size_t dense_stride;
    const uint32_t *dense_off;
    float gain;
    int32_t *result;
    uint32_t *final_range;
    float *softclip_reset;
    opn_silk_side *side;
    int32_t *exc_out;
    int16_t *out16;
    unsigned long long *phase_clk;
};

cudaError_t upload_tables(int device);
cudaError_t launch_rangedec_script(const uint8_t *arena, const uint32_t *offsets, const uint32_t *lens, uint32_t n_packets,
                                   const opn_op *ops, uint32_t n_ops, const uint8_t *icdf_pool, opn_op_out *out,
                                   int32_t *y_out, uint32_t y_stride, uint32_t pkt_cap, cudaStream_t st);
cudaError_t launch_synth_symbols(const SymbolArgs &a, cudaStream_t st);
cudaError_t launch_synth_rangedec(const SymbolArgs &a, cudaStream_t st);
cudaError_t launch_synth_expand(const SymbolArgs &a, cudaStream_t st);
cudaError_t launch_celt2_rangedec(const SymbolArgs &a, cudaStream_t st);
cudaError_t launch_celt2_expand(const SymbolArgs &a, cudaStream_t st);
cudaError_t launch_frame(const FrameArgs &a, cudaStream_t st);
cudaError_t launch_mix_plan(const MixArgs &a, cudaStream_t st);
cudaError_t launch_op_smooth_fade(const float *in1, const float *in2, float *out, size_t row_stride, int overlap, int channels, int fs,
                                  uint32_t n_rows, cudaStream_t st);
cudaError_t launch_silk_rangedec(const SilkArgs &a, cudaStream_t st);
cudaError_t launch_silk_frame(const SilkArgs &a, cudaStream_t st);
cudaError_t launch_transition_fade(float *dense, size_t dense_stride, const uint32_t *d_streams, uint32_t n_streams, uint32_t n_rows, int channels,
                                   cudaStream_t st);
int kernels_frame_groups();
cudaError_t launch_frame_mix(const FrameArgs &a, uint32_t n_streams_in_group, cudaStream_t st);
cudaError_t launch_op_imdct(const float *in, size_t in_stride, float *out, size_t out_stride, uint32_t n_rows, int shift,
                            int nblk, cudaStream_t st);
cudaError_t launch_op_comb_inplace(float *y, size_t row_stride, int y_offset, int n, uint32_t n_rows, const int32_t *params4,
                                   const float *gains2, int overlap, cudaStream_t st);
cudaError_t launch_op_comb(float *y, const float *x, size_t row_stride, int offset, int n, uint32_t n_rows,
                           const int32_t *params4, const float *gains2, int overlap, cudaStream_t st);
cudaError_t launch_op_bitexact_trig(const int16_t *x, int16_t *out_cos, uint32_t n_cos, const int32_t *isin, const int32_t *icos,
                                    int32_t *out_l2t, uint32_t n_l2t, cudaStream_t st);
cudaError_t launch_softclip_convert(int sample_format, const float *dense, size_t dense_stride, const int32_t *clip_len, int channels,
                                    uint32_t row_floats, uint32_t first_row, uint32_t n_rows, float *mem, void *out, size_t out_stride,
                                    cudaStream_t st);
cudaError_t launch_op_soft_clip(float *pcm, size_t row_stride, size_t row_len, int channels, uint32_t n_rows, float *mem,
                                cudaStream_t st);

float host_gain_from_q8(int16_t gain_q8);

}
```

opus-native_b200/csrc/opn_kernels.cu:

```cuda
#include <algorithm>
#include <cstdio>
#include <cstdlib>
#include <cstring>
#include <mutex>
#include <vector>

#include "imdct.cuh"
#include "imdct_warp.cuh"
#include "frame_warp.cuh"
#include "mathops.cuh"
#include "opn_tables.h"
#include "softclip.cuh"
#include "symbols.cuh"
#include "silk.cuh"

namespace opn {


static std::mutex g_tab_mutex;
static int g_sm_count = 148;
constexpr int W_CARVEOUT_PCT = 100;
static bool g_tab_done[64];
static uint16_t g_fblob_bytes[4][2];

template <int LM, int C> static cudaError_t set_carveout()
{
    const int smem = (int)frame_smem_bytes(LM, C, g_fblob_bytes[LM][C - 1]);
    cudaError_t e = cudaFuncSetAttribute(k_frame_w<LM, C, FRAME_SYNTH1>, cudaFuncAttributePreferredSharedMemoryCarveout, W_CARVEOUT_PCT);
    if (e == cudaSuccess) e = cudaFuncSetAttribute(k_frame_w<LM, C, FRAME_SYNTH1>, cudaFuncAttributeMaxDynamicSharedMemorySize, smem);
    if (e == cudaSuccess) e = cudaFuncSetAttribute(k_frame_w<LM, C, FRAME_SYNTH2>, cudaFuncAttributePreferredSharedMemoryCarveout, W_CARVEOUT_PCT);
    if (e == cudaSuccess) e = cudaFuncSetAttribute(k_frame_w<LM, C, FRAME_SYNTH2>, cudaFuncAttributeMaxDynamicSharedMemorySize, smem);
    if (e == cudaSuccess) e = cudaFuncSetAttribute(k_frame_w<LM, C, FRAME_ROWS>, cudaFuncAttributePreferredSharedMemoryCarveout, W_CARVEOUT_PCT);
    if (e == cudaSuccess) e = cudaFuncSetAttribute(k_frame_w<LM, C, FRAME_ROWS>, cudaFuncAttributeMaxDynamicSharedMemorySize, smem);
    return e;
}
template <int LM, int C, int CS> static cudaError_t set_carveout_cross()
{
    const int smem = (int)frame_smem_bytes(LM, 2, g_fblob_bytes[LM][CS - 1]);
    cudaError_t e = cudaFuncSetAttribute(k_frame_w<LM, C, FRAME_SYNTH1, CS>, cudaFuncAttributePreferredSharedMemoryCarveout, W_CARVEOUT_PCT);
    if (e == cudaSuccess) e = cudaFuncSetAttribute(k_frame_w<LM, C, FRAME_SYNTH1, CS>, cudaFuncAttributeMaxDynamicSharedMemorySize, smem);
    if (e == cudaSuccess) e = cudaFuncSetAttribute(k_frame_w<LM, C, FRAME_SYNTH2, CS>, cudaFuncAttributePreferredSharedMemoryCarveout, W_CARVEOUT_PCT);
    if (e == cudaSuccess) e = cudaFuncSetAttribute(k_frame_w<LM, C, FRAME_SYNTH2, CS>, cudaFuncAttributeMaxDynamicSharedMemorySize, smem);
    return e;
}
static size_t mix_smem_bytes(int C)
{
    size_t m = 0;
    for (int lm = 0; lm < 4; lm++) m = std::max(m, frame_smem_bytes(lm, C, g_fblob_bytes[lm][C - 1]));
    return m;
}
template <int C> static cudaError_t set_carveout_mix()
{
    const int smem = (int)mix_smem_bytes(C);
    cudaError_t e = cudaFuncSetAttribute(k_frame_mix<C, FRAME_SYNTH1>, cudaFuncAttributePreferredSharedMemoryCarveout, W_CARVEOUT_PCT);
    if (e == cudaSuccess) e = cudaFuncSetAttribute(k_frame_mix<C, FRAME_SYNTH1>, cudaFuncAttributeMaxDynamicSharedMemorySize, smem);
    if (e == cudaSuccess) e = cudaFuncSetAttribute(k_frame_mix<C, FRAME_SYNTH2>, cudaFuncAttributePreferredSharedMemoryCarveout, W_CARVEOUT_PCT);
    if (e == cudaSuccess) e = cudaFuncSetAttribute(k_frame_mix<C, FRAME_SYNTH2>, cudaFuncAttributeMaxDynamicSharedMemorySize, smem);
    return e;
}
static cudaError_t set_warp_kernel_attributes()
{
    cudaError_t e = set_carveout<0, 1>();
    if (e == cudaSuccess) e = set_carveout_cross<0, 1, 2>();
    if (e == cudaSuccess) e = set_carveout_cross<0, 2, 1>();
    if (e == cudaSuccess) e = set_carveout_cross<1, 1, 2>();
    if (e == cudaSuccess) e = set_carveout_cross<1, 2, 1>();
    if (e == cudaSuccess) e = set_carveout_cross<2, 1, 2>();
    if (e == cudaSuccess) e = set_carveout_cross<2, 2, 1>();
    if (e == cudaSuccess) e = set_carveout_cross<3, 1, 2>();
    if (e == cudaSuccess) e = set_carveout_cross<3, 2, 1>();
    if (e == cudaSuccess) e = set_carveout_mix<1>();
    if (e == cudaSuccess) e = set_carveout_mix<2>();
    if (e == cudaSuccess) e = set_carveout<0, 2>();
    if (e == cudaSuccess) e = set_carveout<1, 1>();
    if (e == cudaSuccess) e = set_carveout<1, 2>();
    if (e == cudaSuccess) e = set_carveout<2, 1>();
    if (e == cudaSuccess) e = set_carveout<2, 2>();
    if (e == cudaSuccess) e = set_carveout<3, 1>();
    if (e == cudaSuccess) e = set_carveout<3, 2>();
    return e;
}

cudaError_t upload_tables(int device)
{
    std::lock_guard<std::mutex> lock(g_tab_mutex);
    if (device < 0 || device >= 64) return cudaErrorInvalidDevice;
    if (g_tab_done[device]) return cudaSuccess;
    static DevTables h;
    for (int i = 0; i < 1800; i++) h.trig[i] = OPN_TRIG[i];
    for (int i = 0; i < 120; i++) {
        h.window[i] = OPN_WINDOW[i];
        h.window_sq[i] = OPN_WINDOW[i] * OPN_WINDOW[i];
    }
    for (int i = 0; i < 480; i++) h.twiddles[i] = make_float2(OPN_TWIDDLES[2 * i], OPN_TWIDDLES[2 * i + 1]);
    for (int s = 0, trigp = 0, nn = 1920; s < 4; s++) {
        const int n4 = 480 >> s;
        for (int i = 0; i < n4; i++) h.trig_pair[trig_pair_off(s) + i] = make_float2(OPN_TRIG[trigp + i], OPN_TRIG[trigp + n4 + i]);
        nn >>= 1;
        trigp += nn;
    }
    for (int i = 0; i < 480; i++) h.bitrev[0][i] = OPN_BITREV_480[i];
    for (int i = 0; i < 240; i++) h.bitrev[1][i] = OPN_BITREV_240[i];
    for (int i = 0; i < 120; i++) h.bitrev[2][i] = OPN_BITREV_120[i];
    for (int i = 0; i < 60; i++) h.bitrev[3][i] = OPN_BITREV_60[i];
    for (int i = 0; i < 1272; i++) h.pvq_u_data[i] = OPN_PVQ_U_DATA[i];
    for (int i = 0; i < 15; i++) h.pvq_u_row[i] = OPN_PVQ_U_ROW[i];
    for (int k = 0; k < 15; k++) {
        const int first = OPN_PVQ_U_ROW[k] + k, end = k < 14 ? OPN_PVQ_U_ROW[k + 1] + k + 1 : 1272;
        const int next_end = k < 13 ? OPN_PVQ_U_ROW[k + 2] + k + 2 : 1272;
        uint32_t acc = 0;
        for (int i = first; i < end; i++) {
            const int m = i - OPN_PVQ_U_ROW[k];
            h.pvq_cw_data[i].x = acc;
            acc += OPN_PVQ_U_DATA[i];
            const int up = k < 14 ? OPN_PVQ_U_ROW[k + 1] + m : 1272;
            h.pvq_cw_data[i].y = (m >= k + 1 && up < next_end) ? OPN_PVQ_U_DATA[up] - OPN_PVQ_U_DATA[i] : 0u;
        }
    }
    for (int k = 0; k < 16; k++) {
        h.pvq_ev_nmax[k] = 0;
        if (k > 13) continue;
        auto last_col = [](int r) { return (r < 14 ? OPN_PVQ_U_ROW[r + 1] + r : 1271) - OPN_PVQ_U_ROW[r]; };
        const int last = std::min(last_col(k), last_col(k + 1));
        uint64_t rowsum = 0;
        for (int n = k; n <= last && n < 256; n++) {
            rowsum += OPN_PVQ_U_DATA[OPN_PVQ_U_ROW[k] + n];
            if (n > k && rowsum + OPN_PVQ_U_DATA[OPN_PVQ_U_ROW[k + 1] + n] < (1ull << 32)) h.pvq_ev_nmax[k] = (uint8_t)n;
            else if (n > k) break;
        }
    }
    for (int i = 0; i < 22; i++) h.e_bands[i] = OPN_E_BANDS[i];
    for (int l = 0; l < 4; l++)
        for (int b = 0; b < 21; b++)
            for (int k = 0; k < 3; k++) h.synth_sched[l][b][k] = OPN_SYNTH_SCHED[l][b][k];
    for (int lm = 0; lm < 4; lm++)
        for (int C = 1; C <= 2; C++) {
            int ne = 0;
            const int nf = 120 << lm;
            for (int b = 0; b < 21; b++)
                for (int c = 0; c < C; c++) {
                    const uint32_t n = OPN_SYNTH_SCHED[lm][b][0], parts = OPN_SYNTH_SCHED[lm][b][1], k = OPN_SYNTH_SCHED[lm][b][2];
                    for (uint32_t p = 0; p < parts; p++) {
                        SynthEntry &e = h.synth_entries[lm][C - 1][ne++];
                        e.base = (uint16_t)(c * nf + ((int)OPN_E_BANDS[b] << lm) + (int)(p * n));
                        e.n = (uint8_t)n;
                        e.k = (uint8_t)k;
                        e.ft_minus1 = 0; e.magic = 0; e.ft1 = 0; e.ftb = 0; e.sh = 0;
                        if (n > 64 || k > 6) return cudaErrorInvalidValue;
                        if (n == 1) continue;
                        if (n > 2 && k < n) {
                            uint64_t rowsum = 0;
                            for (uint32_t j = k; j <= n; j++) rowsum += OPN_PVQ_U_DATA[OPN_PVQ_U_ROW[k] + j];
                            if (k >= 14 || rowsum + OPN_PVQ_U_DATA[OPN_PVQ_U_ROW[k + 1] + n] >= (1ull << 32)) return cudaErrorInvalidValue;
                            if (n > h.pvq_ev_nmax[k]) return cudaErrorInvalidValue;
                        }
                        auto U = [](uint32_t a, uint32_t bb) { return OPN_PVQ_U_DATA[OPN_PVQ_U_ROW[a < bb ? a : bb] + (a < bb ? bb : a)]; };
                        const uint32_t ft = U(n, k) + U(n, k + 1);
                        e.ft_minus1 = ft - 1;
                        uint32_t ftb = 32u - (uint32_t)__builtin_clz(ft - 1);
                        uint32_t ft1;
                        if (ftb > 8) { ftb -= 8; ft1 = ((ft - 1) >> ftb) + 1; } else { ftb = 0; ft1 = ft; }
                        e.ftb = (uint8_t)ftb;
                        e.ft1 = (uint16_t)ft1;
                        uint32_t sh = 0;
                        while ((1ull << sh) < ft1) sh++;
                        e.sh = (uint8_t)sh;
                        e.magic = (uint32_t)((((1ull << sh) - ft1) << 32) / ft1 + 1);
                    }
                }
            h.synth_n_entries[lm][C - 1] = (uint8_t)ne;
            uint8_t *eo = h.synth_entry_of[lm][C - 1];
            for (int i = 0; i < 2 * 960; i++) eo[i] = SYNTH_MAX_ENTRIES;
            for (int e = 0; e < ne; e++) {
                const SynthEntry &E = h.synth_entries[lm][C - 1][e];
                for (int j = 0; j < (int)E.n; j++) eo[E.base + j] = (uint8_t)e;
            }
            {
                auto walk = [&](int e) {
                    const SynthEntry &E = h.synth_entries[lm][C - 1][e];
                    return (E.n == 1 || E.k == 1) ? 0 : (int)E.n;
                };
                int order[SYNTH_MAX_ENTRIES];
                for (int e = 0; e < ne; e++) order[e] = e;
                for (int a = 1; a < ne; a++) {
                    const int v = order[a];
                    int b2 = a - 1;
                    while (b2 >= 0 && walk(order[b2]) < walk(v)) {
                        order[b2 + 1] = order[b2];
                        b2--;
                    }
                    order[b2 + 1] = v;
                }
                const int nslots = (ne + 31) / 32;
                if (nslots > SYNTH_SLOTS) return cudaErrorInvalidValue;
                h.synth_n_slots[lm][C - 1] = (uint8_t)nslots;
                for (int sl = 0; sl < SYNTH_SLOTS; sl++) {
                    h.synth_slot_maxn[lm][C - 1][sl] = 0;
                    for (int l = 0; l < 32; l++) {
                        const int r = sl * 32 + l;
                        h.synth_slot_entries[lm][C - 1][sl][l] = r < ne ? (uint8_t)order[r] : 0xFF;
                        if (r < ne && walk(order[r]) > h.synth_slot_maxn[lm][C - 1][sl]) h.synth_slot_maxn[lm][C - 1][sl] = (uint8_t)walk(order[r]);
                    }
                }
            }
        }
    for (int i = 0; i < 21; i++) h.log_n[i] = OPN_LOG_N[i];
    for (int i = 0; i < 231; i++) h.alloc_vectors[i] = OPN_ALLOC_VECTORS[i];
    for (int i = 0; i < 105; i++) h.cache_index[i] = OPN_CACHE_INDEX[i];
    for (int i = 0; i < 392; i++) h.cache_bits[i] = OPN_CACHE_BITS[i];
    for (int i = 0; i < 168; i++) h.cache_caps[i] = OPN_CACHE_CAPS[i];
    for (int i = 0; i < 24; i++) h.log2_frac[i] = OPN_LOG2_FRAC_TABLE[i];
    h.tapset_icdf[0] = 2; h.tapset_icdf[1] = 1; h.tapset_icdf[2] = 0; h.tapset_icdf[3] = 0;
    for (int i = 0; i < 9; i++) h.comb_gains[i] = OPN_COMB_GAINS[i];
    static uint8_t blobs[4][2][FBLOB_MAX_BYTES];
    for (int lm = 0; lm < 4; lm++)
        for (int C = 1; C <= 2; C++) {
            uint8_t *bl = blobs[lm][C - 1];
            std::memset(bl, 0, FBLOB_MAX_BYTES);
            FBlobHdr &H = h.fblob_hdr[lm][C - 1];
            size_t at = 0;
            auto put = [&](const void *src, size_t bytes) {
                const size_t off = at;
                if (off + bytes > FBLOB_MAX_BYTES) return (size_t)0xFFFF;
                if (src) std::memcpy(bl + off, src, bytes);
                at = (off + bytes + 15) & ~(size_t)15;
                return off;
            };
            const int shift = 3 - lm;
            H.tp_long = (uint16_t)put(h.trig_pair + trig_pair_off(shift), (size_t)(480 >> shift) * sizeof(float2));
            H.tp_short = (uint16_t)put(h.trig_pair + trig_pair_off(3), 60 * sizeof(float2));
            H.tw = (uint16_t)put(h.twiddles, 480 * sizeof(float2));
            H.win = (uint16_t)put(h.window, 120 * sizeof(float));
            H.win_sq = (uint16_t)put(h.window_sq, 120 * sizeof(float));
            const int ne = h.synth_n_entries[lm][C - 1];
            int kmax = 1, nmax = 2;
            for (int e2 = 0; e2 < ne; e2++) {
                kmax = std::max(kmax, (int)h.synth_entries[lm][C - 1][e2].k);
                nmax = std::max(nmax, (int)h.synth_entries[lm][C - 1][e2].n);
            }
            nmax = std::max(nmax, kmax + 1);
            const int rows = kmax + 2, cols = nmax + 1;
            if (rows > 15) return cudaErrorInvalidValue;
            std::vector<uint32_t> cu((size_t)rows * cols, 0u);
            std::vector<uint2> ccw((size_t)rows * cols, make_uint2(0u, 0u));
            auto last_col = [](int r) { return (r < 14 ? OPN_PVQ_U_ROW[r + 1] + r : 1271) - OPN_PVQ_U_ROW[r]; };
            for (int k = 0; k < rows; k++)
                for (int n = 0; n < cols; n++) {
                    const int lo = std::min(k, n), hi = std::max(k, n);
                    if (hi > last_col(lo)) return cudaErrorInvalidValue;
                    cu[(size_t)k * cols + n] = OPN_PVQ_U_DATA[OPN_PVQ_U_ROW[lo] + hi];
                    if (n >= k) ccw[(size_t)k * cols + n] = h.pvq_cw_data[OPN_PVQ_U_ROW[k] + n];
                }
            H.pvq_u = (uint16_t)put(cu.data(), cu.size() * sizeof(uint32_t));
            H.pvq_cw = (uint16_t)put(ccw.data(), ccw.size() * sizeof(uint2));
            uint16_t row16[16];
            for (int k = 0; k < 16; k++) row16[k] = (uint16_t)(std::min(k, rows - 1) * cols);
            H.pvq_row = (uint16_t)put(row16, sizeof(row16));
            H.pvq_nmax = (uint16_t)put(h.pvq_ev_nmax, 16);
            H.ent = (uint16_t)put(h.synth_entries[lm][C - 1], (size_t)ne * sizeof(SynthEntry));
            H.slots = (uint16_t)put(h.synth_slot_entries[lm][C - 1], SYNTH_SLOTS * 32);
            if (at > FBLOB_MAX_BYTES || at > 0xFFF0) return cudaErrorInvalidValue;
            H.total = (uint16_t)at;
            H.n_slots = h.synth_n_slots[lm][C - 1];
            H.n_entries = (uint16_t)ne;
            H.cols = (uint16_t)cols;
            H.pad = 0;
            g_fblob_bytes[lm][C - 1] = H.total;
        }
    cudaError_t e = cudaSetDevice(device);
    if (e != cudaSuccess) return e;
    e = cudaDeviceGetAttribute(&g_sm_count, cudaDevAttrMultiProcessorCount, device);
    if (e != cudaSuccess) return e;
    e = cudaMemcpyToSymbol(g_tab, &h, sizeof(h));
    if (e != cudaSuccess) return e;
    e = cudaMemcpyToSymbol(g_fblob, blobs, sizeof(blobs));
    if (e != cudaSuccess) return e;
    e = cudaMemcpyToSymbol(g_exp2_q9, OPN_EXP2_Q9, sizeof(float) * 512);
    if (e == cudaSuccess) {
        static SilkTables sk;
        std::memset(&sk, 0, sizeof(sk));
        for (int i = 0; i < 64; i++) sk.gain_q10[i] = OPN_SILK_GAIN_Q10[i];
        for (int i = 0; i < 40; i++) sk.ltp_q14[i] = OPN_SILK_LTP_Q14[i];
        for (int i = 0; i < 3; i++) sk.type_icdf[i] = OPN_SILK_TYPE_ICDF[i];
        for (int i = 0; i < 9; i++) sk.delta_icdf[i] = OPN_SILK_DELTA_GAIN_ICDF[i];
        for (int i = 0; i < 4; i++) sk.contour_icdf[i] = OPN_SILK_CONTOUR_ICDF[i];
        for (int i = 0; i < 8; i++) sk.ltp_icdf[i] = OPN_SILK_LTP_ICDF[i];
        for (int i = 0; i < 18; i++) sk.pulses_icdf[i] = OPN_SILK_PULSES_ICDF[i];
        static float up[3][48];
        std::memset(up, 0, sizeof(up));
        for (int i = 0; i < 48; i++) up[0][i] = OPN_SILK_UP6[i];
        for (int i = 0; i < 32; i++) up[1][i] = OPN_SILK_UP4[i];
        for (int i = 0; i < 24; i++) up[2][i] = OPN_SILK_UP3[i];
        e = cudaMemcpyToSymbol(g_silk, &sk, sizeof(sk));
        if (e == cudaSuccess) e = cudaMemcpyToSymbol(c_silk_up, up, sizeof(up));
        if (e == cudaSuccess) e = cudaFuncSetAttribute(k_silk_frame<1, 1>, cudaFuncAttributeMaxDynamicSharedMemorySize, (int)silk_frame_smem());
        if (e == cudaSuccess) e = cudaFuncSetAttribute(k_silk_frame<1, 2>, cudaFuncAttributeMaxDynamicSharedMemorySize, (int)silk_frame_smem());
        if (e == cudaSuccess) e = cudaFuncSetAttribute(k_silk_frame<2, 1>, cudaFuncAttributeMaxDynamicSharedMemorySize, (int)silk_frame_smem());
        if (e == cudaSuccess) e = cudaFuncSetAttribute(k_silk_frame<2, 2>, cudaFuncAttributeMaxDynamicSharedMemorySize, (int)silk_frame_smem());
    }
    if (e != cudaSuccess) return e;
    e = set_warp_kernel_attributes();
    if (e != cudaSuccess) return e;
    e = cudaFuncSetAttribute(k_rangedec_script, cudaFuncAttributeMaxDynamicSharedMemorySize, 64 * 1024);
    if (e != cudaSuccess) return e;
    e = cudaFuncSetAttribute(k_synth_expand, cudaFuncAttributeMaxDynamicSharedMemorySize, (int)synth_expand_smem());
    if (e != cudaSuccess) return e;
    g_tab_done[device] = true;
    return cudaSuccess;
}

template <int LM, int C> static cudaError_t launch_frame_w(const FrameArgs &a, cudaStream_t st)
{
    const size_t smem = frame_smem_bytes(LM, C, g_fblob_bytes[LM][C - 1]);
    const uint32_t grid = (a.item_end - a.item0 + FRAME_WARPS - 1) / FRAME_WARPS;
    if (a.coef) k_frame_w<LM, C, FRAME_ROWS><<<grid, 32 * FRAME_WARPS, smem, st>>>(a);
    else if (a.parts) k_frame_w<LM, C, FRAME_SYNTH2><<<grid, 32 * FRAME_WARPS, smem, st>>>(a);
    else k_frame_w<LM, C, FRAME_SYNTH1><<<grid, 32 * FRAME_WARPS, smem, st>>>(a);
    return cudaGetLastError();
}

template <int LM, int C, int CS> static cudaError_t launch_frame_cross(const FrameArgs &a, cudaStream_t st)
{
    if (a.coef) return cudaErrorInvalidValue;
    const size_t smem = frame_smem_bytes(LM, 2, g_fblob_bytes[LM][CS - 1]);
    const uint32_t grid = (a.item_end - a.item0 + FRAME_WARPS - 1) / FRAME_WARPS;
    if (a.parts) k_frame_w<LM, C, FRAME_SYNTH2, CS><<<grid, 32 * FRAME_WARPS, smem, st>>>(a);
    else k_frame_w<LM, C, FRAME_SYNTH1, CS><<<grid, 32 * FRAME_WARPS, smem, st>>>(a);
    return cudaGetLastError();
}

static size_t symbols_smem(uint32_t pkt_cap)
{
    return 3 * PVQ_TABLE_WORDS * 4 + 32 + 16 + (size_t)SYM_WARPS_PER_CTA * Y_STAGE * 4 + (size_t)SYM_WARPS_PER_CTA * pkt_cap;
}

cudaError_t launch_rangedec_script(const uint8_t *arena, const uint32_t *offsets, const uint32_t *lens, uint32_t n_packets,
                                   const opn_op *ops, uint32_t n_ops, const uint8_t *icdf_pool, opn_op_out *out,
                                   int32_t *y_out, uint32_t y_stride, uint32_t pkt_cap, cudaStream_t st)
{
    if (n_packets == 0) return cudaSuccess;
    const uint32_t grid = (n_packets + SYM_WARPS_PER_CTA - 1) / SYM_WARPS_PER_CTA;
    k_rangedec_script<<<grid, SYM_WARPS_PER_CTA * 32, symbols_smem(pkt_cap), st>>>(arena, offsets, lens, n_packets, ops, n_ops,
                                                                                 icdf_pool, out, y_out, y_stride, pkt_cap);
    return cudaGetLastError();
}

cudaError_t launch_synth_rangedec(const SymbolArgs &a, cudaStream_t st)
{
    if (a.n_items == 0) return cudaSuccess;
    if (!a.idx) return cudaErrorInvalidValue;
    constexpr uint32_t per_cta = RANGEDEC_WARPS_PER_CTA * 32u;
    k_synth_rangedec<<<(a.n_items + per_cta - 1u) / per_cta, per_cta, 0, st>>>(a);
    return cudaGetLastError();
}

cudaError_t launch_synth_expand(const SymbolArgs &a, cudaStream_t st)
{
    if (a.n_items == 0) return cudaSuccess;
    if (!a.idx) return cudaErrorInvalidValue;
    const uint32_t grid = (a.n_items + EXPAND_WARPS_PER_CTA - 1) / EXPAND_WARPS_PER_CTA;
    k_synth_expand<<<grid, EXPAND_WARPS_PER_CTA * 32, synth_expand_smem(), st>>>(a);
    return cudaGetLastError();
}

cudaError_t launch_celt2_rangedec(const SymbolArgs &a, cudaStream_t st)
{
    if (a.n_items == 0) return cudaSuccess;
    if (!a.parts || !a.hdr || !a.bande) return cudaErrorInvalidValue;
    k_celt2_rangedec<<<(a.n_items + C2_RD_ITEMS_PER_CTA - 1u) / C2_RD_ITEMS_PER_CTA, RANGEDEC_WARPS_PER_CTA * 32u, 0, st>>>(a);
    return cudaGetLastError();
}

cudaError_t launch_celt2_expand(const SymbolArgs &a, cudaStream_t st)
{
    if (a.n_items == 0) return cudaSuccess;
    k_celt2_expand<<<(a.n_items + 3u) / 4u, 128, 4 * 2 * 960 * sizeof(float), st>>>(a);
    return cudaGetLastError();
}

cudaError_t launch_synth_symbols(const SymbolArgs &a, cudaStream_t st)
{
    cudaError_t e = launch_synth_rangedec(a, st);
    if (e != cudaSuccess) return e;
    return launch_synth_expand(a, st);
}

cudaError_t launch_frame(const FrameArgs &a, cudaStream_t st)
{
    if (a.item_end <= a.item0) return cudaSuccess;
    if (!a.coef && !a.idx && !a.parts) return cudaErrorInvalidValue;
    if (a.stream_channels != 0 && a.stream_channels != a.channels) {
        switch (a.lm * 2 + (a.channels - 1)) {
        case 0: return launch_frame_cross<0, 1, 2>(a, st);
        case 1: return launch_frame_cross<0, 2, 1>(a, st);
        case 2: return launch_frame_cross<1, 1, 2>(a, st);
        case 3: return launch_frame_cross<1, 2, 1>(a, st);
        case 4: return launch_frame_cross<2, 1, 2>(a, st);
        case 5: return launch_frame_cross<2, 2, 1>(a, st);
        case 6: return launch_frame_cross<3, 1, 2>(a, st);
        case 7: return launch_frame_cross<3, 2, 1>(a, st);
        default: return cudaErrorInvalidValue;
        }
    }
    switch (a.lm * 2 + (a.channels - 1)) {
    case 0: return launch_frame_w<0, 1>(a, st);
    case 1: return launch_frame_w<0, 2>(a, st);
    case 2: return launch_frame_w<1, 1>(a, st);
    case 3: return launch_frame_w<1, 2>(a, st);
    case 4: return launch_frame_w<2, 1>(a, st);
    case 5: return launch_frame_w<2, 2>(a, st);
    case 6: return launch_frame_w<3, 1>(a, st);
    case 7: return launch_frame_w<3, 2>(a, st);
    default: return cudaErrorInvalidValue;
    }
}

int kernels_frame_groups() { return OPN_FRAME_GROUPS; }

cudaError_t launch_mix_plan(const MixArgs &a, cudaStream_t st)
{
    if (a.n_streams == 0) return cudaSuccess;
    if (!a.plan || !a.key || !a.rank || !a.last_lm || !a.item_lm || !a.item_offsets || !a.item_lens || !a.item_stream) return cudaErrorInvalidValue;
    if (a.n_groups != 1 && a.n_groups != MIX_GROUPS) return cudaErrorInvalidValue;
    cudaError_t e = cudaMemsetAsync(a.plan, 0, sizeof(MixPlan), st);
    if (e == cudaSuccess) e = cudaMemsetAsync(a.item_lm, MIX_NO_ITEM, mix_item_cap(a.n_streams), st);
    if (e != cudaSuccess) return e;
    const uint32_t grid = (a.n_streams + 255u) / 256u;
    k_mix_key<<<grid, 256, 0, st>>>(a);
    k_mix_place<<<grid, 256, 0, st>>>(a);
    return cudaGetLastError();
}

cudaError_t launch_frame_mix(const FrameArgs &a, uint32_t n_streams_in_group, cudaStream_t st)
{
    if (n_streams_in_group == 0) return cudaSuccess;
    if (!a.plan || a.group < 0 || a.group >= MIX_GROUPS || a.coef || (!a.idx && !a.parts) || !a.stream_idx) return cudaErrorInvalidValue;
    const uint32_t grid = (n_streams_in_group + FRAME_WARPS - 1) / FRAME_WARPS + 4u;
    const size_t smem = mix_smem_bytes(a.channels);
    if (a.channels == 2) {
        if (a.parts) k_frame_mix<2, FRAME_SYNTH2><<<grid, 32 * FRAME_WARPS, smem, st>>>(a);
        else k_frame_mix<2, FRAME_SYNTH1><<<grid, 32 * FRAME_WARPS, smem, st>>>(a);
    } else if (a.channels == 1) {
        if (a.parts) k_frame_mix<1, FRAME_SYNTH2><<<grid, 32 * FRAME_WARPS, smem, st>>>(a);
        else k_frame_mix<1, FRAME_SYNTH1><<<grid, 32 * FRAME_WARPS, smem, st>>>(a);
    } else {
        return cudaErrorInvalidValue;
    }
    return cudaGetLastError();
}

cudaError_t launch_op_imdct(const float *in, size_t in_stride, float *out, size_t out_stride, uint32_t n_rows, int shift,
                            int nblk, cudaStream_t st)
{
    if (n_rows == 0) return cudaSuccess;
    const size_t smem = (size_t)((960 >> shift) * nblk + 60) * 4;
    if (nblk == 1) {
        switch (shift) {
        case 0: k_op_imdct_w<0, 1><<<n_rows, 32, smem, st>>>(in, in_stride, out, out_stride); break;
        case 1: k_op_imdct_w<1, 1><<<n_rows, 32, smem, st>>>(in, in_stride, out, out_stride); break;
        case 2: k_op_imdct_w<2, 1><<<n_rows, 32, smem, st>>>(in, in_stride, out, out_stride); break;
        default: k_op_imdct_w<3, 1><<<n_rows, 32, smem, st>>>(in, in_stride, out, out_stride); break;
        }
    } else {
        if (shift != 3) return cudaErrorInvalidValue;
        switch (nblk) {
        case 2: k_op_imdct_w<3, 2><<<n_rows, 32, smem, st>>>(in, in_stride, out, out_stride); break;
        case 4: k_op_imdct_w<3, 4><<<n_rows, 32, smem, st>>>(in, in_stride, out, out_stride); break;
        case 8: k_op_imdct_w<3, 8><<<n_rows, 32, smem, st>>>(in, in_stride, out, out_stride); break;
        default: return cudaErrorInvalidValue;
        }
    }
    return cudaGetLastError();
}

cudaError_t launch_op_comb_inplace(float *y, size_t row_stride, int y_offset, int n, uint32_t n_rows, const int32_t *params4,
                                   const float *gains2, int overlap, cudaStream_t st)
{
    if (n_rows == 0) return cudaSuccess;
    const size_t smem = ((size_t)n * 4 + 15) & ~(size_t)15;
    if (smem > 48 * 1024) return cudaErrorInvalidValue;
    k_op_comb_inplace_w<<<n_rows, 32, smem, st>>>(y, row_stride, y_offset, n, params4, gains2, overlap);
    return cudaGetLastError();
}

cudaError_t launch_op_comb(float *y, const float *x, size_t row_stride, int offset, int n, uint32_t n_rows,
                           const int32_t *params4, const float *gains2, int overlap, cudaStream_t st)
{
    if (n_rows == 0) return cudaSuccess;
    k_op_comb<<<n_rows, IM_TPC, 0, st>>>(y, x, row_stride, offset, n, params4, gains2, overlap);
    return cudaGetLastError();
}

cudaError_t launch_op_bitexact_trig(const int16_t *x, int16_t *out_cos, uint32_t n_cos, const int32_t *isin, const int32_t *icos,
                                    int32_t *out_l2t, uint32_t n_l2t, cudaStream_t st)
{
    const uint32_t n = n_cos > n_l2t ? n_cos : n_l2t;
    if (n == 0) return cudaSuccess;
    k_op_bitexact_trig<<<(n + 255) / 256, 256, 0, st>>>(x, out_cos, n_cos, isin, icos, out_l2t, n_l2t);
    return cudaGetLastError();
}

template <typename T>
static cudaError_t launch_softclip_convert_t(const float *dense, size_t dense_stride, const int32_t *clip_len, int channels,
                                             uint32_t row_floats, uint32_t first_row, uint32_t n_rows, float *mem, void *out,
                                             size_t out_stride, cudaStream_t st)
{
    const size_t smem = (size_t)row_floats * sizeof(float);
    if (smem > 200 * 1024) return cudaErrorInvalidValue;
    if (smem > 48 * 1024) {
        cudaError_t e = cudaFuncSetAttribute(k_softclip_convert<T>, cudaFuncAttributeMaxDynamicSharedMemorySize, 200 * 1024);
        if (e != cudaSuccess) return e;
    }
    k_softclip_convert<T><<<n_rows, 32, smem, st>>>(dense, dense_stride, clip_len, channels, row_floats,
                                                                                   first_row, mem, static_cast<T *>(out), out_stride);
    return cudaGetLastError();
}

cudaError_t launch_softclip_convert(int sample_format, const float *dense, size_t dense_stride, const int32_t *clip_len, int channels,
                                    uint32_t row_floats, uint32_t first_row, uint32_t n_rows, float *mem, void *out, size_t out_stride,
                                    cudaStream_t st)
{
    if (n_rows == 0) return cudaSuccess;
    if (row_floats % 8u || (dense_stride & 3) || (out_stride & 7)) return cudaErrorInvalidValue;
    switch (sample_format) {
    case OPN_SAMPLE_F32: return launch_softclip_convert_t<float>(dense, dense_stride, clip_len, channels, row_floats, first_row, n_rows, mem, out, out_stride, st);
    case OPN_SAMPLE_I16: return launch_softclip_convert_t<int16_t>(dense, dense_stride, clip_len, channels, row_floats, first_row, n_rows, mem, out, out_stride, st);
    case OPN_SAMPLE_I32: return launch_softclip_convert_t<int32_t>(dense, dense_stride, clip_len, channels, row_floats, first_row, n_rows, mem, out, out_stride, st);
    case OPN_SAMPLE_U16: return launch_softclip_convert_t<uint16_t>(dense, dense_stride, clip_len, channels, row_floats, first_row, n_rows, mem, out, out_stride, st);
    case OPN_SAMPLE_U32: return launch_softclip_convert_t<uint32_t>(dense, dense_stride, clip_len, channels, row_floats, first_row, n_rows, mem, out, out_stride, st);
    case OPN_SAMPLE_F64: return launch_softclip_convert_t<double>(dense, dense_stride, clip_len, channels, row_floats, first_row, n_rows, mem, out, out_stride, st);
    default: return cudaErrorInvalidValue;
    }
}

cudaError_t launch_op_soft_clip(float *pcm, size_t row_stride, size_t row_len, int channels, uint32_t n_rows, float *mem,
                                cudaStream_t st)
{
    if (n_rows == 0 || channels <= 0) return cudaSuccess;
    const uint32_t total = n_rows * (uint32_t)channels;
    k_op_soft_clip<<<(total + 63) / 64, 64, 0, st>>>(pcm, row_stride, row_len, channels, n_rows, mem);
    return cudaGetLastError();
}

cudaError_t launch_op_smooth_fade(const float *in1, const float *in2, float *out, size_t row_stride, int overlap, int channels, int fs,
                                  uint32_t n_rows, cudaStream_t st)
{
    if (n_rows == 0 || overlap <= 0) return cudaSuccess;
    if (channels < 1 || fs <= 0 || 48000 % fs != 0 || (overlap - 1) * (48000 / fs) >= 120) return cudaErrorInvalidValue;
    const dim3 grid((uint32_t)(overlap * channels + 127) / 128, n_rows);
    k_op_smooth_fade<<<grid, 128, 0, st>>>(in1, in2, out, row_stride, overlap, channels, 48000 / fs);
    return cudaGetLastError();
}

cudaError_t launch_silk_rangedec(const SilkArgs &a, cudaStream_t st)
{
    if (a.n_items == 0) return cudaSuccess;
    k_silk_rangedec<<<(a.n_items + 31u) / 32u, 32, 0, st>>>(a);
    return cudaGetLastError();
}

cudaError_t launch_silk_frame(const SilkArgs &a0, cudaStream_t st)
{
    if (a0.n_items == 0) return cudaSuccess;
    SilkArgs a = a0;
    static unsigned long long *clk = [] {
        unsigned long long *p = nullptr;
        const char *e = std::getenv("OPN_SILK_CLK");
        if (e && e[0] == '1' && cudaMallocManaged(&p, 4 * sizeof(unsigned long long)) == cudaSuccess) {
            std::memset(p, 0, 4 * sizeof(unsigned long long));
            static unsigned long long *keep = p;
            std::atexit([] {
                if (keep[3]) fprintf(stderr, "k_silk_frame cycles per CTA: A %.0f  B %.0f  C %.0f  (%llu CTAs)\n", (double)keep[0] / keep[3],
                                     (double)keep[1] / keep[3], (double)keep[2] / keep[3], keep[3]);
            });
        }
        return p;
    }();
    a.phase_clk = clk;
    const int cs = a.stream_channels, c = a.channels;
    if (cs < 1 || cs > 2 || c < 1 || c > 2 || (a.frame_ms != 10 && a.frame_ms != 20)) return cudaErrorInvalidValue;
    if (a.item_end == 0) a.item_end = a.n_items;
    if (a.item_end <= a.item0) return cudaSuccess;
    const uint32_t items_per_cta = (uint32_t)(SILK_ROWS / cs), grid = (a.item_end - a.item0 + items_per_cta - 1u) / items_per_cta;
    const size_t smem = silk_frame_smem();
    if (cs == 1 && c == 1) k_silk_frame<1, 1><<<grid, 32 * SILK_WARPS, smem, st>>>(a);
    else if (cs == 1) k_silk_frame<1, 2><<<grid, 32 * SILK_WARPS, smem, st>>>(a);
    else if (c == 1) k_silk_frame<2, 1><<<grid, 32 * SILK_WARPS, smem, st>>>(a);
    else k_silk_frame<2, 2><<<grid, 32 * SILK_WARPS, smem, st>>>(a);
    return cudaGetLastError();
// ... 12 lines not shown
```

opus-native_b200/csrc/symbols.cuh:

```cuda
#pragma once
#include <type_traits>
#include "opn_device.cuh"
#include "opn_internal.h"
#include "rangedec.cuh"
#include "celt2.cuh"
#include "celt2_lane.cuh"

namespace opn {

constexpr int PVQ_TABLE_WORDS = 1272;
constexpr int Y_STAGE = 192;

__device__ __forceinline__ void stage_bytes(uint8_t *dst, const uint8_t *src, uint32_t len, uint32_t lane)
{
    if ((reinterpret_cast<uintptr_t>(src) & 3u) == 0u) {
        uint32_t words = len >> 2;
        const uint32_t *s4 = reinterpret_cast<const uint32_t *>(src);
        uint32_t *d4 = reinterpret_cast<uint32_t *>(dst);
        for (uint32_t w = lane; w < words; w += 32u) d4[w] = __ldg(s4 + w);
        for (uint32_t i = (words << 2) + lane; i < len; i += 32u) dst[i] = __ldg(src + i);
    } else {
        for (uint32_t i = lane; i < len; i += 32u) dst[i] = __ldg(src + i);
    }
    __syncwarp();
// ... 49 lines not shown
                T = n - max(k, 2u);
                const uint2 *pw = CW + rk + n;
                const uint32_t ic = i - (pw[0].x + U[rk + n]);
                uint32_t hi = T;
                while (lo < hi) {
                    const uint32_t mid = (lo + hi) >> 1;
                    const uint2 cw = pw[-(int32_t)mid];
                    const bool empty = ic + cw.x < cw.y;
                    lo = empty ? mid + 1u : lo;
                    hi = empty ? hi : mid;
                }
                if (lo) i = ic + pw[1 - (int32_t)lo].x;
            } else {
                T = 1u;
                const uint32_t p = U[rk + n];
                if (p <= i && i < U[rk1 + n]) {
                    i -= p;
                    lo = 1u;
                }
            }
            y += lo;
            n -= lo;
            if (lo < T) {
                const uint32_t q = U[rk1 + n];
                const int32_t sg = i >= q ? -1 : 0;
                i -= (uint32_t)((int32_t)q & sg);
                const uint32_t k0 = k;
                uint32_t p;
                do {
                    k -= 1u;
                    p = U[row[k] + n];
                } while (p > i);
                i -= p;
                const int32_t val = ((int32_t)k0 - (int32_t)k + sg) ^ sg;
                put(y, val);
                yy += val * val;
                rk = row[k];
                rk1 = row[k + 1u];
                y++;
                n -= 1u;
            }
        }
    }
    if (n == 2u) {
        uint32_t p = 2u * k + 1u;
        int32_t sg = i >= p ? -1 : 0;
        i -= (uint32_t)((int32_t)p & sg);
        const uint32_t k0 = k;
        k = (i + 1u) >> 1;
        if (k != 0u) i -= 2u * k - 1u;
        int32_t val = ((int32_t)k0 - (int32_t)k + sg) ^ sg;
        if (val) put(y, val);
        yy += val * val;
        sg = -(int32_t)i;
        val = ((int32_t)k + sg) ^ sg;
        if (val) put(y + 1u, val);
        yy += val * val;
    }
    return yy;
}

__global__ void __launch_bounds__(SYM_WARPS_PER_CTA * 32)
k_rangedec_script(const uint8_t *__restrict__ arena, const uint32_t *__restrict__ offsets,
                  const uint32_t *__restrict__ lens, uint32_t n_packets, const opn_op *__restrict__ ops,
                  uint32_t n_ops, const uint8_t *__restrict__ icdf_pool, opn_op_out *__restrict__ out,
                  int32_t *__restrict__ y_out, uint32_t y_stride, uint32_t pkt_cap)
{
    extern __shared__ __align__(16) uint8_t smem[];
    uint32_t *s_pvq = reinterpret_cast<uint32_t *>(smem);
    uint2 *s_cw = reinterpret_cast<uint2 *>(s_pvq + PVQ_TABLE_WORDS);
    uint16_t *s_row = reinterpret_cast<uint16_t *>(s_cw + PVQ_TABLE_WORDS);
    uint8_t *s_nmax = reinterpret_cast<uint8_t *>(s_row + 16);
    int32_t *s_y = reinterpret_cast<int32_t *>(s_nmax + 16) + (threadIdx.x >> 5) * Y_STAGE;
    uint8_t *s_pkt = reinterpret_cast<uint8_t *>(reinterpret_cast<int32_t *>(s_nmax + 16) + SYM_WARPS_PER_CTA * Y_STAGE) +
                     (threadIdx.x >> 5) * pkt_cap;
    for (int i = threadIdx.x; i < PVQ_TABLE_WORDS; i += blockDim.x) s_cw[i] = g_tab.pvq_cw_data[i];
    if (threadIdx.x < 16) s_nmax[threadIdx.x] = g_tab.pvq_ev_nmax[threadIdx.x];
    load_pvq_table(s_pvq, s_row);
    const uint32_t lane = threadIdx.x & 31u;
    const uint32_t pkt = blockIdx.x * SYM_WARPS_PER_CTA + (threadIdx.x >> 5);
    if (pkt >= n_packets) return;
    const uint32_t len = lens[pkt];
    const uint8_t *bytes = arena + offsets[pkt];
    if (len <= pkt_cap) {
        stage_bytes(s_pkt, bytes, len, lane);
        bytes = s_pkt;
    }
    PvqTable T{s_pvq, s_row};
    RangeDec d;
    d.init(bytes, len);
    uint32_t ny = 0u;
    for (uint32_t i = 0; i < n_ops; i++) {
        const uint32_t op = ops[i].op, a = ops[i].a, b = ops[i].b;
        uint32_t v = 0u;
        switch (op) {
        case OPN_OP_UINT: v = d.uint(a); break;
        case OPN_OP_BITS: v = d.bits(a); break;
        case OPN_OP_BIT_LOGP: v = d.bit_logp(a); break;
        case OPN_OP_ICDF: v = d.icdf(icdf_pool + a, b); break;
        case OPN_OP_LAPLACE: v = (uint32_t)d.laplace(a, b); break;
        case OPN_OP_BIT_VIA_DECODE: {
            uint32_t fs = d.decode(1u << a);
            uint32_t s = fs >= (1u << a) - 1u ? 1u : 0u;
            d.update(s ? (1u << a) - 1u : 0u, (1u << a) - (s ? 0u : 1u), 1u << a);
            v = s;
            break;
        }
        case OPN_OP_BIT_VIA_DECODE_BIN: {
            uint32_t fs = d.decode_bin(a);
            uint32_t s = fs >= (1u << a) - 1u ? 1u : 0u;
            d.update(s ? (1u << a) - 1u : 0u, (1u << a) - (s ? 0u : 1u), 1u << a);
            v = s;
            break;
        }
        case OPN_OP_PULSES: {
            float yy = decode_pulses_warp(d, T, s_y, a, b, lane);
            v = __float_as_uint(yy);
            if (y_out)
                for (uint32_t j = lane; j < a; j += 32u) y_out[(size_t)pkt * y_stride + ny + j] = s_y[j];
            ny += a;
            __syncwarp();
            break;
        }
        case OPN_OP_PULSES_EVENTS: {
            const uint32_t ci = d.uint(T.v(a, b));
            for (uint32_t j = lane; j < a; j += 32u) s_y[j] = 0;
            __syncwarp();
            int32_t yy = 0;
            if (lane == 0u) yy = cwrsi_events(s_pvq, s_cw, s_row, s_nmax, a, b, ci, [&](uint32_t at, int32_t val) { s_y[at] = val; });
            yy = __shfl_sync(0xFFFFFFFFu, yy, 0);
            __syncwarp();
            v = __float_as_uint((float)yy);
            if (y_out)
                for (uint32_t j = lane; j < a; j += 32u) y_out[(size_t)pkt * y_stride + ny + j] = s_y[j];
            ny += a;
            __syncwarp();
            break;
        }
        case OPN_OP_SHRINK: d.shrink_storage(a); break;
        case OPN_OP_TELL: v = d.tell(); break;
        default: break;
        }
        if (lane == 0u) {
            opn_op_out o;
            o.value = v;
            o.tell_frac = d.tell_frac();
            o.rng = d.rng;
            out[(size_t)pkt * n_ops + i] = o;
        }
    }
}

constexpr size_t SYM_EXPAND_WARP_BYTES = 2 * 960 * 4;
__host__ __device__ constexpr size_t synth_expand_smem()
{
    return 3 * PVQ_TABLE_WORDS * 4 + 32 + 16 + 16 + SYNTH_MAX_ENTRIES * sizeof(SynthEntry) + (size_t)EXPAND_WARPS_PER_CTA * SYM_EXPAND_WARP_BYTES;
}

__global__ void __launch_bounds__(RANGEDEC_WARPS_PER_CTA * 32) k_synth_rangedec(SymbolArgs A)
{
    __shared__ SynthEntry s_ent[SYNTH_MAX_ENTRIES];
    __shared__ uint32_t s_lfl[21][LAP_N + 1], s_lfs[21][LAP_N + 1];
    const uint32_t lane = threadIdx.x;
    const int C = A.channels;
    int lm = A.lm;
    if (A.item_lm) {
        const uint32_t l = A.item_lm[blockIdx.x * (RANGEDEC_WARPS_PER_CTA * 32u)];
        if (l == MIX_NO_ITEM) return;
        lm = (int)l;
    }
    if (lane < 21u) {
        const uint32_t decay = 6000u + 400u * lane;
        const uint32_t fs0 = ((32768u - 33u) * (16384u - decay)) / (16384u + decay) + 1u;
        laplace_table(fs0, decay, s_lfl[lane], s_lfs[lane]);
    }
    const int ne = g_tab.synth_n_entries[lm][C - 1];
    {
        const uint4 *src = reinterpret_cast<const uint4 *>(g_tab.synth_entries[lm][C - 1]);
        uint4 *dst = reinterpret_cast<uint4 *>(s_ent);
        for (int i = lane; i < ne; i += RANGEDEC_WARPS_PER_CTA * 32) dst[i] = src[i];
    }
    __syncthreads();
    const uint32_t item = blockIdx.x * (RANGEDEC_WARPS_PER_CTA * 32u) + lane;
    if (item >= A.n_items) return;
    if (A.item_lm && A.item_lm[item] == MIX_NO_ITEM) return;
    const uint32_t stream = A.stream_idx ? A.stream_idx[item] : item;
    uint32_t len = A.lens[item];
    const uint8_t *src = A.arena + A.offsets[item];

    int32_t status = len == 0u ? ITEM_LOST : ITEM_OK;
    if (A.has_toc && len > 0u) {
        const uint32_t toc = __ldg(src);
        if ((toc & 0x80u) == 0u) status = OPN_ERR_UNIMPLEMENTED;
        else if ((toc & 0x3u) != 0u) status = OPN_ERR_UNIMPLEMENTED;
        else if ((int)((toc >> 3) & 0x3u) != lm) status = OPN_ERR_FRAME_SIZE_TOO_SMALL;
        else if (((toc & 0x4u) ? 2 : 1) != C) status = OPN_ERR_UNIMPLEMENTED;
        src += 1;
        len -= 1u;
    }
    if (status == ITEM_OK && len <= 1u) status = ITEM_LOST;
    A.status[stream] = status;
    if (status < 0) return;

    opn_synth_side *sd = A.side ? A.side + stream : nullptr;
    uint32_t *sw = reinterpret_cast<uint32_t *>(sd);
    constexpr uint32_t SIDE_WORDS = sizeof(opn_synth_side) / 4u;
    if (status == ITEM_LOST) {
        if (sd)
            for (uint32_t i = 0; i < SIDE_WORDS; i++) sw[i] = 0u;
        A.hdr[stream] = make_uint4(0u, 0u, 0u, 0u);
        return;
    }
    LaneDec d;
    d.init(src, len);
    const uint32_t silence = d.bit_logp(15u);
    if (silence) {
        if (sd) {
            for (uint32_t i = 0; i < SIDE_WORDS; i++) sw[i] = 0u;
            sd->silence = 1;
            sd->final_rng = d.rng;
            sd->tell_frac = d.tell_frac();
        }
        A.hdr[stream] = make_uint4(1u, d.rng, d.tell_frac(), 0u);
        return;
    }
    const uint32_t postfilter = d.bit_logp(1u);
    uint32_t octave = 0u, period = 0u, gain_idx = 0u, tapset = 0u;
    if (postfilter) {
        octave = d.uint_small(6u);
        period = (16u << octave) + d.bits(4u + octave) - 1u;
        gain_idx = d.bits(3u);
        tapset = d.icdf(g_tab.tapset_icdf, 2u);
    }
    const uint32_t transient = d.bit_logp(3u);
    const uint32_t intra = d.bit_logp(3u);
    if (sd) {
        sd->silence = 0;
        sd->postfilter = (int32_t)postfilter;
        sd->octave = (int32_t)octave;
        sd->period = (int32_t)period;
        sd->gain_idx = (int32_t)gain_idx;
        sd->tapset = (int32_t)tapset;
        sd->transient = (int32_t)transient;
        sd->intra = (int32_t)intra;
    }
    for (int b = 0; b < 21; b++) {
        const uint32_t decay = 6000u + 400u * (uint32_t)b;
        for (int c = 0; c < C; c++) {
            const int32_t v = d.laplace(s_lfl[b], s_lfs[b], decay);
            if (sd) sd->coarse[c][b] = v;
        }
        if (sd && C == 1) sd->coarse[1][b] = 0;
    }
    for (int f0 = 0; f0 < 21 * C; f0 += 12) {
        const int nfld = min(12, 21 * C - f0);
        uint32_t w = d.bits(2u * (uint32_t)nfld);
        if (sd)
            for (int f = f0; f < f0 + nfld; f++, w >>= 2) sd->fine[f % C][f / C] = (int32_t)(w & 3u);
    }
    if (sd && C == 1)
        for (int b = 0; b < 21; b++) sd->fine[1][b] = 0;
    uint32_t *idx = A.idx + (size_t)stream * SYNTH_MAX_ENTRIES;
    uint32_t n_pulses = 0u;
    for (int e = 0; e < ne; e++) {
        const SynthEntry E = s_ent[e];
        uint32_t v;
        if (E.n == 1) {
            v = d.bits(1u);
            n_pulses += 1u;
        } else {
            v = d.uint_precomputed(E.ft_minus1, E.ft1, E.ftb, E.magic, E.sh);
            n_pulses += E.k;
        }
        idx[e] = v;
    }
    const uint32_t tf = d.tell_frac();
    if (sd) {
        sd->final_rng = d.rng;
        sd->tell_frac = tf;
        sd->n_pulses = n_pulses;
    }
    A.hdr[stream] = make_uint4(hdr_pack(0u, postfilter, transient, intra, tapset, gain_idx, octave, period), d.rng, tf, n_pulses);
}

struct ExpandTables {
    const uint32_t *U;
    const uint2 *CW;
    const uint16_t *row;
    const uint8_t *nmax;
    const SynthEntry *ent;
    const uint8_t *slots;
    int n_slots;
};
__device__ __forceinline__ uint32_t block_major(uint32_t j, int lmt, int nf) { return (j & ((1u << lmt) - 1u)) * (uint32_t)(nf >> lmt) + (j >> lmt); }
template <int C, class IdxFn>
__device__ __forceinline__ void w_expand(const ExpandTables &T, int lm, uint32_t lane, IdxFn get_idx, float *rows, int chs,
                                         int32_t *__restrict__ y_out, int lmt = 0)
{
    const int nf = 120 << lm;
    const int nslots = T.n_slots;
    uint32_t ee[SYNTH_SLOTS], ii[SYNTH_SLOTS];
#pragma unroll
    for (int slot = 0; slot < SYNTH_SLOTS; slot++) {
        ee[slot] = slot < nslots ? T.slots[slot * 32 + lane] : 0xFFu;
        ii[slot] = get_idx(ee[slot]);
    }
#pragma unroll 1
    for (int slot = 0; slot < nslots; slot++) {
        uint32_t e = ee[0], i = ii[0];
#pragma unroll
        for (int q = 1; q < SYNTH_SLOTS; q++)
            if (slot == q) { e = ee[q]; i = ii[q]; }
        const bool has = e != 0xFFu;
        const SynthEntry E = T.ent[has ? e : 0u];
        uint32_t n = has ? E.n : 0u;
        const uint32_t k = E.k;
        uint64_t rec = 0ull;
        uint32_t cnt = 0u;
        auto put = [&](uint32_t at, int32_t val) {
            rec |= (uint64_t)((at << 4) | ((uint32_t)val & 15u)) << (10u * cnt);
            cnt += 1u;
        };
        int32_t yy = 0;
        if (has && n == 1u) {
            put(0u, i ? -1 : 1);
            yy = 1;
        } else if (has && k == 1u) {
            if (i < n) put(i, 1);
            else put(2u * n - 1u - i, -1);
            yy = 1;
            n = 0u;
        }
        yy += cwrsi_events(T.U, T.CW, T.row, T.nmax, n, k, i, put);
        if (has) {
            const float gain = 0.03125f / sqrtf((float)yy);
            const uint32_t ch = E.base >= (uint32_t)nf ? 1u : 0u;
            const uint32_t bin0 = E.base - ch * (uint32_t)nf;
            float *dst = rows + ch * (uint32_t)chs;
            auto store = [&](auto remap) {
#pragma unroll
                for (uint32_t j = 0; j < 6u; j++) {
                    if (j < cnt) {
                        const uint32_t r = (uint32_t)(rec >> (10u * j)) & 1023u;
                        const int32_t val = ((int32_t)(r << 28)) >> 28;
                        const uint32_t at = bin0 + (r >> 4);
                        dst[decltype(remap)::value ? block_major(at, lmt, nf) : at] = (float)val * gain;
                        if (y_out) y_out[E.base + (r >> 4)] = val;
                    }
                }
            };
            if (lmt) store(std::true_type{});
            else store(std::false_type{});
        }
    }
}

__global__ void __launch_bounds__(EXPAND_WARPS_PER_CTA * 32) k_synth_expand(SymbolArgs A)
{
    extern __shared__ __align__(16) uint8_t smem[];
    const uint32_t warp = threadIdx.x >> 5, lane = threadIdx.x & 31u;
    uint32_t *s_pvq = reinterpret_cast<uint32_t *>(smem);
    uint2 *s_cw = reinterpret_cast<uint2 *>(s_pvq + PVQ_TABLE_WORDS);
    uint16_t *s_row = reinterpret_cast<uint16_t *>(s_cw + PVQ_TABLE_WORDS);
    uint8_t *s_nmax = reinterpret_cast<uint8_t *>(s_row + 16);
    uint64_t *bar = reinterpret_cast<uint64_t *>(s_nmax + 16);
    SynthEntry *s_ent = reinterpret_cast<SynthEntry *>(bar + 2);
    float *s_rows = reinterpret_cast<float *>(reinterpret_cast<uint8_t *>(s_ent + SYNTH_MAX_ENTRIES) + (size_t)warp * SYM_EXPAND_WARP_BYTES);

    const int lm = A.lm, C = A.channels, nf = 120 << lm;
    const int ne = g_tab.synth_n_entries[lm][C - 1];
    if (threadIdx.x == 0) {
        mbar_init(bar, 1);
        mbar_expect_tx(bar, 3 * PVQ_TABLE_WORDS * 4);
        bulk_g2s(s_pvq, g_tab.pvq_u_data, PVQ_TABLE_WORDS * 4, bar);
        bulk_g2s(s_cw, g_tab.pvq_cw_data, 2 * PVQ_TABLE_WORDS * 4, bar);
    }
    if (threadIdx.x < 15) s_row[threadIdx.x] = g_tab.pvq_u_row[threadIdx.x];
    if (threadIdx.x < 16) s_nmax[threadIdx.x] = g_tab.pvq_ev_nmax[threadIdx.x];
    {
        const uint4 *src = reinterpret_cast<const uint4 *>(g_tab.synth_entries[lm][C - 1]);
        uint4 *dst = reinterpret_cast<uint4 *>(s_ent);
        for (int i = threadIdx.x; i < ne; i += blockDim.x) dst[i] = src[i];
    }
    const uint32_t item = blockIdx.x * EXPAND_WARPS_PER_CTA + warp;
    const bool in_range = item < A.n_items;
    const uint32_t stream = in_range ? (A.stream_idx ? A.stream_idx[item] : item) : 0u;
    const int32_t status = in_range ? A.status[stream] : -1;
    const int32_t silence = in_range ? (int32_t)(A.hdr[stream].x & 1u) : 0;
    const bool zero_frame = status == ITEM_LOST || (status >= 0 && silence != 0);
    const int nvec = C * nf / 4;
    for (int i = lane; i < nvec; i += 32) reinterpret_cast<float4 *>(s_rows)[i] = make_float4(0.f, 0.f, 0.f, 0.f);
    __syncthreads();
    mbar_wait(bar, 0);
    if (status < 0) return;
    float4 *coef4 = A.coef ? reinterpret_cast<float4 *>(A.coef + (size_t)stream * C * nf) : nullptr;
    int32_t *yo = A.y_out ? A.y_out + (size_t)stream * C * nf : nullptr;
    if (yo)
        for (int i = lane; i < nvec; i += 32) reinterpret_cast<int4 *>(yo)[i] = make_int4(0, 0, 0, 0);
    __syncwarp();
    if (!zero_frame) {
        const ExpandTables T{s_pvq, s_cw, s_row, s_nmax, s_ent, &g_tab.synth_slot_entries[lm][C - 1][0][0], g_tab.synth_n_slots[lm][C - 1]};
        const uint32_t *ip = A.idx + (size_t)stream * SYNTH_MAX_ENTRIES;
        auto get_idx = [&](uint32_t e) { return e != 0xFFu ? __ldg(ip + e) : 0u; };
        if (C == 2) w_expand<2>(T, lm, lane, get_idx, s_rows, nf, yo);
        else w_expand<1>(T, lm, lane, get_idx, s_rows, nf, yo);
    }
    __syncwarp();
    if (coef4)
        for (int i = lane; i < nvec; i += 32) coef4[i] = reinterpret_cast<const float4 *>(s_rows)[i];
}

__device__ __forceinline__ Celt2Tabs device_celt2_tabs()
{
    return Celt2Tabs{g_tab.e_bands, g_tab.log_n, g_tab.alloc_vectors, g_tab.cache_bits, g_tab.cache_caps, g_tab.log2_frac, g_tab.cache_index,
                     g_tab.pvq_u_data, g_tab.pvq_u_row};
}

#ifndef OPN_C2_RD_MIN_CTAS
#define OPN_C2_RD_MIN_CTAS 16
#endif
#ifndef OPN_C2_RD_LANES
#define OPN_C2_RD_LANES 32
#endif
constexpr uint32_t C2_RD_LANES = OPN_C2_RD_LANES;
constexpr uint32_t C2_RD_ITEMS_PER_CTA = RANGEDEC_WARPS_PER_CTA * C2_RD_LANES;
static_assert(32u % C2_RD_LANES == 0u, "a mixed-frame bucket starts on a multiple of MIX_PAD items: a CTA must not span two");
__global__ void __launch_bounds__(RANGEDEC_WARPS_PER_CTA * 32, OPN_C2_RD_MIN_CTAS) k_celt2_rangedec(SymbolArgs A)
{
    __shared__ uint32_t s_lfl[21][LAP_N + 1], s_lfs[21][LAP_N + 1];
    __shared__ int16_t s_e9[2 * 21][RANGEDEC_WARPS_PER_CTA * 32];
    const uint32_t lane = threadIdx.x;
    const int C = A.channels;
    int lm = A.lm;
    if (A.item_lm) {
        const uint32_t l = A.item_lm[blockIdx.x * C2_RD_ITEMS_PER_CTA];
        if (l == MIX_NO_ITEM) return;
        lm = (int)l;
    }
    if (lane < 21u) {
        const uint32_t decay = 6000u + 400u * lane;
        const uint32_t fs0 = ((32768u - 33u) * (16384u - decay)) / (16384u + decay) + 1u;
        laplace_table(fs0, decay, s_lfl[lane], s_lfs[lane]);
    }
    __syncthreads();
    if ((lane & 31u) >= C2_RD_LANES) return;
    const uint32_t item = blockIdx.x * C2_RD_ITEMS_PER_CTA + (lane >> 5) * C2_RD_LANES + (lane & 31u);
    if (item >= A.n_items) return;
    if (A.item_lm && A.item_lm[item] == MIX_NO_ITEM) return;
    const uint32_t stream = A.stream_idx ? A.stream_idx[item] : item;
    uint32_t len = A.lens[item];
    const uint8_t *src = A.arena + A.offsets[item];
    int32_t status = len == 0u ? ITEM_LOST : ITEM_OK;
    if (A.has_toc && len > 0u) {
        const uint32_t toc = __ldg(src);
        if ((toc & 0x80u) == 0u) status = OPN_ERR_UNIMPLEMENTED;
        else if ((toc & 0x3u) != 0u) status = OPN_ERR_UNIMPLEMENTED;
        else if ((int)((toc >> 3) & 0x3u) != lm) status = OPN_ERR_FRAME_SIZE_TOO_SMALL;
        else if (((toc & 0x4u) ? 2 : 1) != C) status = OPN_ERR_UNIMPLEMENTED;
        src += 1;
        len -= 1u;
    }
    if (status == ITEM_OK && len <= 1u) status = ITEM_LOST;
    Celt2Side *sd = A.side2 ? A.side2 + stream : nullptr;
    if (sd) {
        uint32_t *sw = reinterpret_cast<uint32_t *>(sd);
        for (uint32_t i = 0; i < sizeof(Celt2Side) / 4u; i++) sw[i] = 0u;
    }
    if (status != ITEM_OK) {
        A.status[stream] = status;
        if (status == ITEM_LOST) A.hdr[stream] = make_uint4(0u, 0u, 0u, 0u);
        return;
    }
    LaneCoder ec;
    ec.lfl = s_lfl;
    ec.lfs = s_lfs;
    ec.d.init(src, len);
    LanePartSink sink{A.parts + (size_t)stream * CELT2_MAX_PARTS, 0u, 0u, 0u, &s_e9[0][lane], RANGEDEC_WARPS_PER_CTA * 32u};
    for (int i = 0; i < 2 * 21; i++) s_e9[i][lane] = 0;
    uint32_t flags = 0u, n_pulses = 0u;
    celt2_frame(ec, device_celt2_tabs(), len, lm, C, sd, sink, flags, n_pulses);
    if (A.bande) {
        uint32_t *be = reinterpret_cast<uint32_t *>(A.bande + (size_t)stream * 42);
        for (int i = 0; i < 21; i++) be[i] = (uint32_t)(uint16_t)s_e9[2 * i][lane] | (uint32_t)(uint16_t)s_e9[2 * i + 1][lane] << 16;
    }
    const uint32_t tf = ec.d.tell_frac();
    if (sd) {
        sd->n_parts = sink.n - sink.nsign;
        sd->n_pulses = n_pulses;
        sd->final_rng = ec.d.rng;
        sd->tell_frac = tf;
    }
    if (sink.n > (uint32_t)CELT2_MAX_PARTS) status = OPN_ERR_INTERNAL;
    A.status[stream] = status;
    A.hdr[stream] = make_uint4(flags, ec.d.rng, tf, sink.n);
}

template <int C>
__device__ __forceinline__ void w_expand2(const ExpandTables &T, int lm, uint32_t lane, const Celt2Part *__restrict__ parts, uint32_t n_parts,
                                          const int16_t *__restrict__ bande, float *rows, int chs, int32_t *__restrict__ y_out, int lmt = 0)
{
    const int nf = 120 << lm;
    for (uint32_t p = lane; p < n_parts; p += 32u) {
        const Celt2Part P = parts[p];
        const uint32_t pos = P.base & (uint32_t)C2_POS_MASK, band = P.base >> C2_BAND_SHIFT;
        const uint32_t ch = pos >= (uint32_t)nf ? 1u : 0u;
        const uint32_t bin0 = pos - ch * (uint32_t)nf;
        float *dst = rows + ch * (uint32_t)chs;
        int32_t *yo = y_out ? y_out + pos : nullptr;
        const float bg = c2_band_gain(g_exp2_q9, (int)bande[ch * 21u + band]);
        if (P.n == 1u) {
            dst[block_major(bin0, lmt, nf)] = (P.index ? -P.gain : P.gain) * bg;
            if (yo) yo[0] = P.index ? -1 : 1;
            continue;
        }
        const int32_t yy = cwrsi_events(T.U, T.CW, T.row, T.nmax, (uint32_t)P.n, (uint32_t)P.k, P.index, [&](uint32_t at, int32_t val) {
            dst[block_major(bin0 + at, lmt, nf)] = (float)val;
            if (yo) yo[at] = val;
        });
        const float g = P.gain / sqrtf((float)yy);
        for (uint32_t j = 0; j < P.n; j++) {
            float *q = dst + block_major(bin0 + j, lmt, nf);
            const float v = *q;
            if (v != 0.0f) *q = (v * g) * bg;
        }
    }
}

__global__ void __launch_bounds__(128) k_celt2_expand(SymbolArgs A)
{
    extern __shared__ __align__(16) float s_rows_all[];
    const uint32_t warp = threadIdx.x >> 5, lane = threadIdx.x & 31u;
    const int lm = A.lm, C = A.channels, nf = 120 << lm;
    float *rows = s_rows_all + (size_t)warp * 2 * 960;
    const uint32_t item = blockIdx.x * 4u + warp;
    if (item >= A.n_items) return;
    const uint32_t stream = A.stream_idx ? A.stream_idx[item] : item;
    const int32_t status = A.status[stream];
    if (status < 0) return;
    const uint4 hdr = A.hdr[stream];
    const int nvec = C * nf / 4;
    for (int i = lane; i < nvec; i += 32) reinterpret_cast<float4 *>(rows)[i] = make_float4(0.f, 0.f, 0.f, 0.f);
    int32_t *yo = A.y_out ? A.y_out + (size_t)stream * C * nf : nullptr;
    if (yo)
        for (int i = lane; i < nvec; i += 32) reinterpret_cast<int4 *>(yo)[i] = make_int4(0, 0, 0, 0);
    __syncwarp();
    if (status == ITEM_OK && !(hdr.x & 1u)) {
        const ExpandTables T{g_tab.pvq_u_data, g_tab.pvq_cw_data, g_tab.pvq_u_row, g_tab.pvq_ev_nmax, nullptr, nullptr, 0};
        if (C == 2) w_expand2<2>(T, lm, lane, A.parts + (size_t)stream * CELT2_MAX_PARTS, hdr.w, A.bande + (size_t)stream * 42, rows, nf, yo);
        else w_expand2<1>(T, lm, lane, A.parts + (size_t)stream * CELT2_MAX_PARTS, hdr.w, A.bande + (size_t)stream * 42, rows, nf, yo);
    }
    __syncwarp();
    if (A.coef) {
        float4 *coef4 = reinterpret_cast<float4 *>(A.coef + (size_t)stream * C * nf);
        for (int i = lane; i < nvec; i += 32) coef4[i] = reinterpret_cast<const float4 *>(rows)[i];
    }
}

}
```

Baseline: 1.654 million.

## Split PVQ pulse decoding into a separate entry-parallel kernel before frame synthesis

Adds a k_synth_pulses kernel that decodes PVQ codewords into packed pulse records and gains, one warp per entry across 32 streams per CTA, using a small per-(lm,C) PVQ table slice staged in shared memory. The frame and expand kernels then only scatter precomputed pulses instead of walking PVQ tables per lane with shuffles, and the frame blob shrinks because it no longer carries the PVQ tables and slot ordering. The intent is to remove per-warp serial PVQ walking and lane imbalance from the frame kernel. In exchange it adds an extra kernel launch and a global round trip for the pulse buffer. The new kernel reads idx as entry-major (e*n_streams+stream), which presumes the rangedec output layout matches.

```diff
diff --git a/opus-native_b200/csrc/frame_warp.cuh b/opus-native_b200/csrc/frame_warp.cuh
--- a/opus-native_b200/csrc/frame_warp.cuh
+++ b/opus-native_b200/csrc/frame_warp.cuh
@@ -231,13 +231,20 @@
     }
     __syncwarp();
     const uint32_t hdr_x = stash[0].x;
-    [[maybe_unused]] uint32_t ix0 = 0u, ix1 = 0u, ix2 = 0u;
+    [[maybe_unused]] uint2 rc0 = make_uint2(0u, 0u), rc1 = make_uint2(0u, 0u), rc2 = make_uint2(0u, 0u);
+    [[maybe_unused]] float gn0 = 0.0f, gn1 = 0.0f, gn2 = 0.0f;
     if constexpr (MODE == FRAME_SYNTH1) {
         if (in_range) {
-            const uint32_t *ip = A.idx + (size_t)stream * SYNTH_MAX_ENTRIES;
-            ix0 = __ldg(ip + lane);
-            ix1 = __ldg(ip + 32 + lane);
-            if (lane < SYNTH_MAX_ENTRIES - 64) ix2 = __ldg(ip + 64 + lane);
+            const uint2 *rp = reinterpret_cast<const uint2 *>(A.pulse + (size_t)stream * SYNTH_PULSE_WORDS);
+            const float *gp = reinterpret_cast<const float *>(A.pulse + (size_t)stream * SYNTH_PULSE_WORDS + 2 * SYNTH_MAX_ENTRIES);
+            rc0 = __ldg(rp + lane);
+            rc1 = __ldg(rp + 32 + lane);
+            gn0 = __ldg(gp + lane);
+            gn1 = __ldg(gp + 32 + lane);
+            if (lane < SYNTH_MAX_ENTRIES - 64) {
+                rc2 = __ldg(rp + 64 + lane);
+                gn2 = __ldg(gp + 64 + lane);
+            }
         }
     }
     float *carry_g = A.carry + (size_t)stream * C * 60;
@@ -276,19 +283,16 @@
     const int lmt = (LM > 0 && ((hdr_x >> 2) & 1u)) ? LM : 0;
     if constexpr (MODE == FRAME_SYNTH1) {
         if (!lost && !(hdr_x & 1u)) {
-            const ExpandTables T{reinterpret_cast<const uint32_t *>(blob + H.pvq_u), reinterpret_cast<const uint2 *>(blob + H.pvq_cw),
-                                 reinterpret_cast<const uint16_t *>(blob + H.pvq_row), blob + H.pvq_nmax,
-                                 reinterpret_cast<const SynthEntry *>(blob + H.ent), blob + H.slots, (int)H.n_slots};
-            w_expand<CS>(T, LM, (uint32_t)lane, [&](uint32_t e) {
-                const int src = (int)(e & 31u);
-                const uint32_t a = __shfl_sync(0xFFFFFFFFu, ix0, src), b2 = __shfl_sync(0xFFFFFFFFu, ix1, src), c2 = __shfl_sync(0xFFFFFFFFu, ix2, src);
-                return e == 0xFFu ? 0u : e < 32u ? a : e < 64u ? b2 : c2;
-            }, o, CHF, nullptr, lmt);
+            const SynthEntry *ent = reinterpret_cast<const SynthEntry *>(blob + H.ent);
+            const int ne = H.n_entries;
+            if (lane < ne) synth_scatter(ent[lane], rc0, gn0, o, CHF, NF, lmt, nullptr);
+            if (lane + 32 < ne) synth_scatter(ent[lane + 32], rc1, gn1, o, CHF, NF, lmt, nullptr);
+            if (lane + 64 < ne) synth_scatter(ent[lane + 64], rc2, gn2, o, CHF, NF, lmt, nullptr);
         }
         __syncwarp();
     } else if constexpr (MODE == FRAME_SYNTH2) {
         if (!lost && !(hdr_x & 1u)) {
-            const ExpandTables T{g_tab.pvq_u_data, g_tab.pvq_cw_data, g_tab.pvq_u_row, g_tab.pvq_ev_nmax, nullptr, nullptr, 0};
+            const ExpandTables T{g_tab.pvq_u_data, g_tab.pvq_cw_data, g_tab.pvq_u_row, g_tab.pvq_ev_nmax};
             w_expand2<CS>(T, LM, (uint32_t)lane, A.parts + (size_t)stream * CELT2_MAX_PARTS, stash[0].w, A.bande + (size_t)stream * 42, o, CHF, nullptr, lmt);
         }
         __syncwarp();
diff --git a/opus-native_b200/csrc/host_runtime.cpp b/opus-native_b200/csrc/host_runtime.cpp
--- a/opus-native_b200/csrc/host_runtime.cpp
+++ b/opus-native_b200/csrc/host_runtime.cpp
@@ -146,6 +146,7 @@
     bool unfused = false;
     float *d_carry = nullptr, *d_ring = nullptr, *d_coef[NSETS] = {};
     uint32_t *d_ring_pos = nullptr, *d_final = nullptr, *d_idx[NSETS] = {};
+    uint32_t *d_pulse[NSETS] = {};
     PfState *d_pf = nullptr;
     uint4 *d_hdr[NSETS] = {};
     int32_t *d_status[NSETS] = {};
@@ -252,6 +253,7 @@
     const SymbolArgs &s = *static_cast<const SymbolArgs *>(a);
     return b->cfg.bitstream == OPN_BITSTREAM_SYNTH_CELT_2 ? launch_celt2_rangedec(s, b->stream) : launch_synth_rangedec(s, b->stream);
 }
+cudaError_t do_pulses(opn_batch *b, const void *a) { return launch_synth_pulses(*static_cast<const SymbolArgs *>(a), b->stream); }
 cudaError_t do_expand(opn_batch *b, const void *a) { return launch_synth_expand(*static_cast<const SymbolArgs *>(a), b->stream); }
 bool frame_grouped(const opn_batch *b, const FrameArgs &m)
 {
@@ -341,6 +343,8 @@
     s.coef = b->unfused ? b->d_coef[p] : nullptr;
     s.y_out = nullptr;
     s.idx = b->d_idx[p];
+    s.pulse = b->d_pulse[p];
+    s.n_streams = b->n;
     s.pkt_cap = pkt_cap;
     s.parts = b->d_parts[p];
     s.bande = b->d_bande[p];
@@ -354,6 +358,10 @@
         }
         rc = timed_launch(b, 0, do_rangedec, &s);
         if (rc) return rc;
+        if (!celt2) {
+            rc = timed_launch(b, 2, do_pulses, &s);
+            if (rc) return rc;
+        }
         if (b->unfused) {
             rc = timed_launch(b, 2, do_expand, &s);
             if (rc) return rc;
@@ -372,8 +380,12 @@
                 for (int g = 1; g < opn_batch::NGROUPS; g++) CU(cudaStreamWaitEvent(srd, b->ev_fr[p][g], 0));
         }
         CU(celt2 ? launch_celt2_rangedec(s, srd) : launch_synth_rangedec(s, srd));
+        b->launches[0]++;
+        if (!celt2) {
+            CU(launch_synth_pulses(s, srd));
+            b->launches[2]++;
+        }
         CU(cudaEventRecord(b->ev_rd[p], srd));
-        b->launches[0]++;
         if (b->unfused) {
             CU(cudaStreamWaitEvent(b->stream_ex, b->ev_rd[p], 0));
             CU(launch_synth_expand(s, b->stream_ex));
@@ -386,7 +398,7 @@
     }
     FrameArgs m{};
     m.coef = b->unfused ? b->d_coef[p] : nullptr;
-    m.idx = celt2 ? nullptr : b->d_idx[p];
+    m.pulse = celt2 ? nullptr : b->d_pulse[p];
     m.parts = celt2 ? b->d_parts[p] : nullptr;
     m.bande = b->d_bande[p];
     m.hdr = b->d_hdr[p];
@@ -603,12 +615,14 @@
     s.hdr = b->d_hdr[p];
     s.status = b->d_status[p];
     s.idx = b->d_idx[p];
+    s.pulse = b->d_pulse[p];
+    s.n_streams = b->n;
     s.pkt_cap = 1280u;
     s.parts = b->d_parts[p];
     s.bande = b->d_bande[p];
     const bool celt2 = b->cfg.bitstream == OPN_BITSTREAM_SYNTH_CELT_2;
     FrameArgs m{};
-    m.idx = celt2 ? nullptr : b->d_idx[p];
+    m.pulse = celt2 ? nullptr : b->d_pulse[p];
     m.parts = celt2 ? b->d_parts[p] : nullptr;
     m.bande = b->d_bande[p];
     m.hdr = b->d_hdr[p];
@@ -637,6 +651,10 @@
         b->launches[2] += 2;
         rc = timed_launch(b, 0, do_rangedec, &s);
         if (rc) return rc;
+        if (!celt2) {
+            rc = timed_launch(b, 2, do_pulses, &s);
+            if (rc) return rc;
+        }
         rc = timed_launch(b, 1, do_frame, &m);
         if (rc) return rc;
         b->launches[1] += G - 1;
@@ -656,8 +674,12 @@
         CU(cudaEventRecord(b->ev_mix[p], sx));
         CU(cudaStreamWaitEvent(srd, b->ev_mix[p], 0));
         CU(celt2 ? launch_celt2_rangedec(s, srd) : launch_synth_rangedec(s, srd));
+        b->launches[0]++;
+        if (!celt2) {
+            CU(launch_synth_pulses(s, srd));
+            b->launches[2]++;
+        }
         CU(cudaEventRecord(b->ev_rd[p], srd));
-        b->launches[0]++;
         if (G == 1) {
             rc = join_groups(b);
             if (rc) return rc;
@@ -801,6 +823,7 @@
         if (e == cudaSuccess) e = cudaEventCreateWithFlags(&b->ev_k1[q], cudaEventDisableTiming);
         for (int g = 1; g < opn_batch::NGROUPS && e == cudaSuccess; g++) e = cudaEventCreateWithFlags(&b->ev_fr[q][g], cudaEventDisableTiming);
         if (e == cudaSuccess) e = cudaMalloc(&b->d_idx[q], n * 72 * sizeof(uint32_t));
+        if (e == cudaSuccess && celt_bitstream == OPN_BITSTREAM_SYNTH_CELT_1) e = cudaMalloc(&b->d_pulse[q], n * SYNTH_PULSE_WORDS * sizeof(uint32_t));
         if (e == cudaSuccess && b->unfused) e = cudaMalloc(&b->d_coef[q], n * C * 960 * sizeof(float));
         if (e == cudaSuccess) e = cudaMalloc(&b->d_hdr[q], n * sizeof(uint4));
         if (e == cudaSuccess && celt_bitstream == OPN_BITSTREAM_SYNTH_CELT_2) e = cudaMalloc(&b->d_parts[q], n * CELT2_MAX_PARTS * sizeof(Celt2Part));
@@ -873,6 +896,7 @@
         if (b->ev_ex[q]) cudaEventDestroy(b->ev_ex[q]);
         if (b->ev_k1[q]) cudaEventDestroy(b->ev_k1[q]);
         cudaFree(b->d_idx[q]);
+        cudaFree(b->d_pulse[q]);
         cudaFree(b->d_coef[q]);
         cudaFree(b->d_hdr[q]);
         cudaFree(b->d_parts[q]);
@@ -1723,7 +1747,7 @@
         max_len = std::max(max_len, lens[i]);
     }
     const size_t row = (size_t)channels * (120u << lm);
-    DevBuf dA, dO, dL, dS, dSt, dY, dC, dI, dH;
+    DevBuf dA, dO, dL, dS, dSt, dY, dC, dI, dP, dH;
     CU(dA.alloc(arena_end));
     CU(dO.alloc(n_packets * 4));
     CU(dL.alloc(n_packets * 4));
@@ -1733,6 +1757,7 @@
     CU(dY.alloc((size_t)n_packets * row * 4));
     CU(dC.alloc((size_t)n_packets * row * 4));
     CU(dI.alloc((size_t)n_packets * 72 * 4));
+    CU(dP.alloc((size_t)n_packets * SYNTH_PULSE_WORDS * 4));
     CU(cudaMemcpy(dA.p, arena, arena_end, cudaMemcpyHostToDevice));
     CU(cudaMemcpy(dO.p, offsets, n_packets * 4, cudaMemcpyHostToDevice));
     CU(cudaMemcpy(dL.p, lens, n_packets * 4, cudaMemcpyHostToDevice));
@@ -1751,6 +1776,8 @@
     s.coef = dC.as<float>();
     s.y_out = dY.as<int32_t>();
     s.idx = dI.as<uint32_t>();
+    s.pulse = dP.as<uint32_t>();
+    s.n_streams = n_packets;
     s.pkt_cap = (max_len + 15u) & ~15u;
     CU(launch_synth_symbols(s, nullptr));
     CU(cudaDeviceSynchronize());
diff --git a/opus-native_b200/csrc/opn_device.cuh b/opus-native_b200/csrc/opn_device.cuh
--- a/opus-native_b200/csrc/opn_device.cuh
+++ b/opus-native_b200/csrc/opn_device.cuh
@@ -16,7 +16,6 @@
     uint8_t sh;
 };
 constexpr int SYNTH_MAX_ENTRIES = 72;
-constexpr int SYNTH_SLOTS = 3;
 
 struct FBlobHdr {
     uint16_t tp_long;
@@ -24,16 +23,21 @@
     uint16_t tw;
     uint16_t win;
     uint16_t win_sq;
-    uint16_t pvq_u;
-    uint16_t pvq_cw;
-    uint16_t pvq_row;
-    uint16_t pvq_nmax;
     uint16_t ent;
-    uint16_t slots;
     uint16_t total;
-    uint16_t n_slots, n_entries, cols, pad;
+    uint16_t n_entries;
 };
 constexpr int FBLOB_MAX_BYTES = 20 * 1024;
+
+struct PvqSliceHdr {
+    uint16_t u;
+    uint16_t cw;
+    uint16_t row;
+    uint16_t nmax;
+    uint16_t total;
+    uint16_t pad[3];
+};
+constexpr int PVQ_SLICE_MAX_BYTES = 4096;
 
 struct DevTables {
     float trig[1800];
@@ -51,12 +55,10 @@
     SynthEntry synth_entries[4][2][SYNTH_MAX_ENTRIES];
     uint8_t synth_n_entries[4][2];
     uint8_t synth_entry_of[4][2][2 * 960];
-    uint8_t synth_slot_entries[4][2][SYNTH_SLOTS][32];
-    uint8_t synth_slot_maxn[4][2][SYNTH_SLOTS];
-    uint8_t synth_n_slots[4][2];
     uint8_t tapset_icdf[4];
     float comb_gains[9];
     FBlobHdr fblob_hdr[4][2];
+    PvqSliceHdr pvq_slice_hdr[4][2];
     uint8_t log_n[24];
     uint8_t alloc_vectors[232];
     int16_t cache_index[106];
@@ -67,6 +69,7 @@
 
 __device__ DevTables g_tab;
 __device__ __align__(128) uint8_t g_fblob[4][2][FBLOB_MAX_BYTES];
+__device__ __align__(16) uint8_t g_pvq_slice[4][2][PVQ_SLICE_MAX_BYTES];
 __device__ float g_exp2_q9[512];
 
 }
diff --git a/opus-native_b200/csrc/opn_internal.h b/opus-native_b200/csrc/opn_internal.h
--- a/opus-native_b200/csrc/opn_internal.h
+++ b/opus-native_b200/csrc/opn_internal.h
@@ -19,8 +19,13 @@
 #define OPN_EXPAND_WARPS 4
 #endif
 constexpr int EXPAND_WARPS_PER_CTA = OPN_EXPAND_WARPS;
+#ifndef OPN_PULSE_WARPS
+#define OPN_PULSE_WARPS 4
+#endif
+constexpr int PULSE_WARPS = OPN_PULSE_WARPS;
 constexpr int IM_TPC = 128;
 constexpr int RING_SAMPLES = 2880;
+constexpr int SYNTH_PULSE_WORDS = 3 * 72;
 constexpr int32_t ITEM_OK = 0, ITEM_LOST = 1;
 
 struct PfState {
@@ -62,6 +67,8 @@
     float *coef;
     int32_t *y_out;
     uint32_t *idx;
+    uint32_t *pulse;
+    uint32_t n_streams;
     uint32_t pkt_cap;
     struct Celt2Part *parts;
     struct Celt2Side *side2;
@@ -71,7 +78,7 @@
 
 struct FrameArgs {
     const float *coef;
-    const uint32_t *idx;
+    const uint32_t *pulse;
     const struct Celt2Part *parts;
     const uint4 *hdr;
     const int32_t *status;
@@ -174,6 +181,7 @@
                                    int32_t *y_out, uint32_t y_stride, uint32_t pkt_cap, cudaStream_t st);
 cudaError_t launch_synth_symbols(const SymbolArgs &a, cudaStream_t st);
 cudaError_t launch_synth_rangedec(const SymbolArgs &a, cudaStream_t st);
+cudaError_t launch_synth_pulses(const SymbolArgs &a, cudaStream_t st);
 cudaError_t launch_synth_expand(const SymbolArgs &a, cudaStream_t st);
 cudaError_t launch_celt2_rangedec(const SymbolArgs &a, cudaStream_t st);
 cudaError_t launch_celt2_expand(const SymbolArgs &a, cudaStream_t st);
diff --git a/opus-native_b200/csrc/opn_kernels.cu b/opus-native_b200/csrc/opn_kernels.cu
--- a/opus-native_b200/csrc/opn_kernels.cu
+++ b/opus-native_b200/csrc/opn_kernels.cu
@@ -175,34 +175,6 @@
                 const SynthEntry &E = h.synth_entries[lm][C - 1][e];
                 for (int j = 0; j < (int)E.n; j++) eo[E.base + j] = (uint8_t)e;
             }
-            {
-                auto walk = [&](int e) {
-                    const SynthEntry &E = h.synth_entries[lm][C - 1][e];
-                    return (E.n == 1 || E.k == 1) ? 0 : (int)E.n;
-                };
-                int order[SYNTH_MAX_ENTRIES];
-                for (int e = 0; e < ne; e++) order[e] = e;
-                for (int a = 1; a < ne; a++) {
-                    const int v = order[a];
-                    int b2 = a - 1;
-                    while (b2 >= 0 && walk(order[b2]) < walk(v)) {
-                        order[b2 + 1] = order[b2];
-                        b2--;
-                    }
-                    order[b2 + 1] = v;
-                }
-                const int nslots = (ne + 31) / 32;
-                if (nslots > SYNTH_SLOTS) return cudaErrorInvalidValue;
-                h.synth_n_slots[lm][C - 1] = (uint8_t)nslots;
-                for (int sl = 0; sl < SYNTH_SLOTS; sl++) {
-                    h.synth_slot_maxn[lm][C - 1][sl] = 0;
-                    for (int l = 0; l < 32; l++) {
-                        const int r = sl * 32 + l;
-                        h.synth_slot_entries[lm][C - 1][sl][l] = r < ne ? (uint8_t)order[r] : 0xFF;
-                        if (r < ne && walk(order[r]) > h.synth_slot_maxn[lm][C - 1][sl]) h.synth_slot_maxn[lm][C - 1][sl] = (uint8_t)walk(order[r]);
-                    }
-                }
-            }
         }
     for (int i = 0; i < 21; i++) h.log_n[i] = OPN_LOG_N[i];
     for (int i = 0; i < 231; i++) h.alloc_vectors[i] = OPN_ALLOC_VECTORS[i];
@@ -233,6 +205,30 @@
             H.win = (uint16_t)put(h.window, 120 * sizeof(float));
             H.win_sq = (uint16_t)put(h.window_sq, 120 * sizeof(float));
             const int ne = h.synth_n_entries[lm][C - 1];
+            H.ent = (uint16_t)put(h.synth_entries[lm][C - 1], (size_t)ne * sizeof(SynthEntry));
+            if (at > FBLOB_MAX_BYTES || at > 0xFFF0) return cudaErrorInvalidValue;
+            H.total = (uint16_t)at;
+            H.n_entries = (uint16_t)ne;
+            g_fblob_bytes[lm][C - 1] = H.total;
+        }
+    static uint8_t slices[4][2][PVQ_SLICE_MAX_BYTES];
+    for (int lm = 0; lm < 4; lm++)
+        for (int C = 1; C <= 2; C++) {
+            uint8_t *bl = slices[lm][C - 1];
+            std::memset(bl, 0, PVQ_SLICE_MAX_BYTES);
+            PvqSliceHdr &H = h.pvq_slice_hdr[lm][C - 1];
+            size_t at = 0;
+            auto put = [&](const void *src, size_t bytes) {
+                const size_t off = at;
+                if (off + bytes > PVQ_SLICE_MAX_BYTES) {
+                    at = PVQ_SLICE_MAX_BYTES + 1;
+                    return (size_t)0;
+                }
+                std::memcpy(bl + off, src, bytes);
+                at = (off + bytes + 15) & ~(size_t)15;
+                return off;
+            };
+            const int ne = h.synth_n_entries[lm][C - 1];
             int kmax = 1, nmax = 2;
             for (int e2 = 0; e2 < ne; e2++) {
                 kmax = std::max(kmax, (int)h.synth_entries[lm][C - 1][e2].k);
@@ -251,21 +247,14 @@
                     cu[(size_t)k * cols + n] = OPN_PVQ_U_DATA[OPN_PVQ_U_ROW[lo] + hi];
                     if (n >= k) ccw[(size_t)k * cols + n] = h.pvq_cw_data[OPN_PVQ_U_ROW[k] + n];
                 }
-            H.pvq_u = (uint16_t)put(cu.data(), cu.size() * sizeof(uint32_t));
-            H.pvq_cw = (uint16_t)put(ccw.data(), ccw.size() * sizeof(uint2));
+            H.u = (uint16_t)put(cu.data(), cu.size() * sizeof(uint32_t));
+            H.cw = (uint16_t)put(ccw.data(), ccw.size() * sizeof(uint2));
             uint16_t row16[16];
             for (int k = 0; k < 16; k++) row16[k] = (uint16_t)(std::min(k, rows - 1) * cols);
-            H.pvq_row = (uint16_t)put(row16, sizeof(row16));
-            H.pvq_nmax = (uint16_t)put(h.pvq_ev_nmax, 16);
-            H.ent = (uint16_t)put(h.synth_entries[lm][C - 1], (size_t)ne * sizeof(SynthEntry));
-            H.slots = (uint16_t)put(h.synth_slot_entries[lm][C - 1], SYNTH_SLOTS * 32);
-            if (at > FBLOB_MAX_BYTES || at > 0xFFF0) return cudaErrorInvalidValue;
+            H.row = (uint16_t)put(row16, sizeof(row16));
+            H.nmax = (uint16_t)put(h.pvq_ev_nmax, 16);
+            if (at > PVQ_SLICE_MAX_BYTES) return cudaErrorInvalidValue;
             H.total = (uint16_t)at;
-            H.n_slots = h.synth_n_slots[lm][C - 1];
-            H.n_entries = (uint16_t)ne;
-            H.cols = (uint16_t)cols;
-            H.pad = 0;
-            g_fblob_bytes[lm][C - 1] = H.total;
         }
     cudaError_t e = cudaSetDevice(device);
     if (e != cudaSuccess) return e;
@@ -274,6 +263,8 @@
     e = cudaMemcpyToSymbol(g_tab, &h, sizeof(h));
     if (e != cudaSuccess) return e;
     e = cudaMemcpyToSymbol(g_fblob, blobs, sizeof(blobs));
+    if (e != cudaSuccess) return e;
+    e = cudaMemcpyToSymbol(g_pvq_slice, slices, sizeof(slices));
     if (e != cudaSuccess) return e;
     e = cudaMemcpyToSymbol(g_exp2_q9, OPN_EXP2_Q9, sizeof(float) * 512);
     if (e == cudaSuccess) {
@@ -354,10 +345,19 @@
     return cudaGetLastError();
 }
 
+cudaError_t launch_synth_pulses(const SymbolArgs &a, cudaStream_t st)
+{
+    if (a.n_items == 0) return cudaSuccess;
+    if (!a.idx || !a.pulse) return cudaErrorInvalidValue;
+    const dim3 grid((a.n_items + 31u) / 32u, (SYNTH_MAX_ENTRIES + PULSE_WARPS - 1) / PULSE_WARPS);
+    k_synth_pulses<<<grid, PULSE_WARPS * 32, 0, st>>>(a);
+    return cudaGetLastError();
+}
+
 cudaError_t launch_synth_expand(const SymbolArgs &a, cudaStream_t st)
 {
     if (a.n_items == 0) return cudaSuccess;
-    if (!a.idx) return cudaErrorInvalidValue;
+    if (!a.pulse) return cudaErrorInvalidValue;
     const uint32_t grid = (a.n_items + EXPAND_WARPS_PER_CTA - 1) / EXPAND_WARPS_PER_CTA;
     k_synth_expand<<<grid, EXPAND_WARPS_PER_CTA * 32, synth_expand_smem(), st>>>(a);
     return cudaGetLastError();
@@ -381,6 +381,7 @@
 cudaError_t launch_synth_symbols(const SymbolArgs &a, cudaStream_t st)
 {
     cudaError_t e = launch_synth_rangedec(a, st);
+    if (e == cudaSuccess) e = launch_synth_pulses(a, st);
     if (e != cudaSuccess) return e;
     return launch_synth_expand(a, st);
 }
@@ -388,7 +389,7 @@
 cudaError_t launch_frame(const FrameArgs &a, cudaStream_t st)
 {
     if (a.item_end <= a.item0) return cudaSuccess;
-    if (!a.coef && !a.idx && !a.parts) return cudaErrorInvalidValue;
+    if (!a.coef && !a.pulse && !a.parts) return cudaErrorInvalidValue;
     if (a.stream_channels != 0 && a.stream_channels != a.channels) {
         switch (a.lm * 2 + (a.channels - 1)) {
         case 0: return launch_frame_cross<0, 1, 2>(a, st);
@@ -434,7 +435,7 @@
 cudaError_t launch_frame_mix(const FrameArgs &a, uint32_t n_streams_in_group, cudaStream_t st)
 {
     if (n_streams_in_group == 0) return cudaSuccess;
-    if (!a.plan || a.group < 0 || a.group >= MIX_GROUPS || a.coef || (!a.idx && !a.parts) || !a.stream_idx) return cudaErrorInvalidValue;
+    if (!a.plan || a.group < 0 || a.group >= MIX_GROUPS || a.coef || (!a.pulse && !a.parts) || !a.stream_idx) return cudaErrorInvalidValue;
     const uint32_t grid = (n_streams_in_group + FRAME_WARPS - 1) / FRAME_WARPS + 4u;
     const size_t smem = mix_smem_bytes(a.channels);
     if (a.channels == 2) {
diff --git a/opus-native_b200/csrc/symbols.cuh b/opus-native_b200/csrc/symbols.cuh
--- a/opus-native_b200/csrc/symbols.cuh
+++ b/opus-native_b200/csrc/symbols.cuh
@@ -225,10 +225,7 @@
 }
 
 constexpr size_t SYM_EXPAND_WARP_BYTES = 2 * 960 * 4;
-__host__ __device__ constexpr size_t synth_expand_smem()
-{
-    return 3 * PVQ_TABLE_WORDS * 4 + 32 + 16 + 16 + SYNTH_MAX_ENTRIES * sizeof(SynthEntry) + (size_t)EXPAND_WARPS_PER_CTA * SYM_EXPAND_WARP_BYTES;
-}
+__host__ __device__ constexpr size_t synth_expand_smem() { return (size_t)EXPAND_WARPS_PER_CTA * SYM_EXPAND_WARP_BYTES; }
 
 __global__ void __launch_bounds__(RANGEDEC_WARPS_PER_CTA * 32) k_synth_rangedec(SymbolArgs A)
 {
@@ -333,7 +330,7 @@
     }
     if (sd && C == 1)
         for (int b = 0; b < 21; b++) sd->fine[1][b] = 0;
-    uint32_t *idx = A.idx + (size_t)stream * SYNTH_MAX_ENTRIES;
+    uint32_t *idx = A.idx + stream;
     uint32_t n_pulses = 0u;
     for (int e = 0; e < ne; e++) {
         const SynthEntry E = s_ent[e];
@@ -345,7 +342,7 @@
             v = d.uint_precomputed(E.ft_minus1, E.ft1, E.ftb, E.magic, E.sh);
             n_pulses += E.k;
         }
-        idx[e] = v;
+        idx[(size_t)e * A.n_streams] = v;
     }
     const uint32_t tf = d.tell_frac();
     if (sd) {
@@ -361,70 +358,96 @@
     const uint2 *CW;
     const uint16_t *row;
     const uint8_t *nmax;
-    const SynthEntry *ent;
-    const uint8_t *slots;
-    int n_slots;
 };
+
+__device__ __forceinline__ float synth_part_pulses(const ExpandTables &T, uint32_t n, uint32_t k, uint32_t i, uint64_t &rec)
+{
+    rec = 0ull;
+    uint32_t cnt = 0u;
+    auto put = [&](uint32_t at, int32_t val) {
+        rec |= (uint64_t)((at << 4) | ((uint32_t)val & 15u)) << (10u * cnt);
+        cnt += 1u;
+    };
+    int32_t yy = 0;
+    if (n == 1u) {
+        put(0u, i ? -1 : 1);
+        yy = 1;
+    } else if (k == 1u) {
+        if (i < n) put(i, 1);
+        else put(2u * n - 1u - i, -1);
+        yy = 1;
+    } else {
+        yy = cwrsi_events(T.U, T.CW, T.row, T.nmax, n, k, i, put);
+    }
+    return 0.03125f / sqrtf((float)yy);
+}
+
 __device__ __forceinline__ uint32_t block_major(uint32_t j, int lmt, int nf) { return (j & ((1u << lmt) - 1u)) * (uint32_t)(nf >> lmt) + (j >> lmt); }
-template <int C, class IdxFn>
-__device__ __forceinline__ void w_expand(const ExpandTables &T, int lm, uint32_t lane, IdxFn get_idx, float *rows, int chs,
-                                         int32_t *__restrict__ y_out, int lmt = 0)
-{
-    const int nf = 120 << lm;
-    const int nslots = T.n_slots;
-    uint32_t ee[SYNTH_SLOTS], ii[SYNTH_SLOTS];
-#pragma unroll
-    for (int slot = 0; slot < SYNTH_SLOTS; slot++) {
-        ee[slot] = slot < nslots ? T.slots[slot * 32 + lane] : 0xFFu;
-        ii[slot] = get_idx(ee[slot]);
-    }
-#pragma unroll 1
-    for (int slot = 0; slot < nslots; slot++) {
-        uint32_t e = ee[0], i = ii[0];
-#pragma unroll
-        for (int q = 1; q < SYNTH_SLOTS; q++)
-            if (slot == q) { e = ee[q]; i = ii[q]; }
-        const bool has = e != 0xFFu;
-        const SynthEntry E = T.ent[has ? e : 0u];
-        uint32_t n = has ? E.n : 0u;
-        const uint32_t k = E.k;
-        uint64_t rec = 0ull;
-        uint32_t cnt = 0u;
-        auto put = [&](uint32_t at, int32_t val) {
-            rec |= (uint64_t)((at << 4) | ((uint32_t)val & 15u)) << (10u * cnt);
-            cnt += 1u;
-        };
-        int32_t yy = 0;
-        if (has && n == 1u) {
-            put(0u, i ? -1 : 1);
-            yy = 1;
-        } else if (has && k == 1u) {
-            if (i < n) put(i, 1);
-            else put(2u * n - 1u - i, -1);
-            yy = 1;
-            n = 0u;
-        }
-        yy += cwrsi_events(T.U, T.CW, T.row, T.nmax, n, k, i, put);
-        if (has) {
-            const float gain = 0.03125f / sqrtf((float)yy);
-            const uint32_t ch = E.base >= (uint32_t)nf ? 1u : 0u;
-            const uint32_t bin0 = E.base - ch * (uint32_t)nf;
-            float *dst = rows + ch * (uint32_t)chs;
-            auto store = [&](auto remap) {
-#pragma unroll
-                for (uint32_t j = 0; j < 6u; j++) {
-                    if (j < cnt) {
-                        const uint32_t r = (uint32_t)(rec >> (10u * j)) & 1023u;
-                        const int32_t val = ((int32_t)(r << 28)) >> 28;
-                        const uint32_t at = bin0 + (r >> 4);
-                        dst[decltype(remap)::value ? block_major(at, lmt, nf) : at] = (float)val * gain;
-                        if (y_out) y_out[E.base + (r >> 4)] = val;
-                    }
-                }
-            };
-            if (lmt) store(std::true_type{});
-            else store(std::false_type{});
-        }
+
+__device__ __forceinline__ void synth_scatter(const SynthEntry &E, uint2 r, float g, float *rows, int chs, int nf, int lmt,
+                                              int32_t *__restrict__ y_out)
+{
+    const uint32_t ch = E.base >= (uint32_t)nf ? 1u : 0u;
+    const uint32_t bin0 = E.base - ch * (uint32_t)nf;
+    float *dst = rows + ch * (uint32_t)chs;
+    uint64_t rec = (uint64_t)r.y << 32 | r.x;
+    while (rec) {
+        const uint32_t f = (uint32_t)rec & 1023u;
+        rec >>= 10;
+        const int32_t val = ((int32_t)(f << 28)) >> 28;
+        const uint32_t at = bin0 + (f >> 4);
+        dst[lmt ? block_major(at, lmt, nf) : at] = (float)val * g;
+        if (y_out) y_out[E.base + (f >> 4)] = val;
+    }
+}
+
+__global__ void __launch_bounds__(PULSE_WARPS * 32) k_synth_pulses(SymbolArgs A)
+{
+    __shared__ __align__(16) uint8_t s_tab[PVQ_SLICE_MAX_BYTES];
+    __shared__ uint2 s_rec[PULSE_WARPS][32];
+    __shared__ float s_gain[PULSE_WARPS][32];
+    __shared__ uint32_t s_stream[32];
+    const uint32_t lane = threadIdx.x & 31u, warp = threadIdx.x >> 5;
+    const int C = A.channels;
+    int lm = A.lm;
+    const uint32_t item0 = blockIdx.x * 32u;
+    if (A.item_lm) {
+        const uint32_t l = A.item_lm[item0];
+        if (l == MIX_NO_ITEM) return;
+        lm = (int)l;
+    }
+    const int ne = g_tab.synth_n_entries[lm][C - 1], e0 = (int)blockIdx.y * PULSE_WARPS;
+    if (e0 >= ne) return;
+    const PvqSliceHdr H = g_tab.pvq_slice_hdr[lm][C - 1];
+    {
+        const uint4 *src = reinterpret_cast<const uint4 *>(g_pvq_slice[lm][C - 1]);
+        for (uint32_t i = threadIdx.x; i < H.total / 16u; i += blockDim.x) reinterpret_cast<uint4 *>(s_tab)[i] = src[i];
+    }
+    const uint32_t item = item0 + lane;
+    bool on = item < A.n_items && !(A.item_lm && A.item_lm[item] == MIX_NO_ITEM);
+    const uint32_t stream = on ? (A.stream_idx ? A.stream_idx[item] : item) : 0u;
+    on = on && A.status[stream] == ITEM_OK && !(A.hdr[stream].x & 1u);
+    if (warp == 0u) s_stream[lane] = on ? stream : ~0u;
+    __syncthreads();
+    const ExpandTables T{reinterpret_cast<const uint32_t *>(s_tab + H.u), reinterpret_cast<const uint2 *>(s_tab + H.cw),
+                         reinterpret_cast<const uint16_t *>(s_tab + H.row), s_tab + H.nmax};
+    const int e = e0 + (int)warp;
+    if (on && e < ne) {
+        const SynthEntry E = g_tab.synth_entries[lm][C - 1][e];
+        uint64_t rec;
+        const float g = synth_part_pulses(T, E.n, E.k, __ldg(A.idx + (size_t)e * A.n_streams + stream), rec);
+        s_rec[warp][lane] = make_uint2((uint32_t)rec, (uint32_t)(rec >> 32));
+        s_gain[warp][lane] = g;
+    }
+    __syncthreads();
+    const int m = min(PULSE_WARPS, ne - e0), per = 3 * m;
+    for (int q = threadIdx.x; q < 32 * per; q += blockDim.x) {
+        const int it = q / per, w = q - it * per;
+        const uint32_t st = s_stream[it];
+        if (st == ~0u) continue;
+        uint32_t *row = A.pulse + (size_t)st * SYNTH_PULSE_WORDS;
+        if (w < 2 * m) row[2 * e0 + w] = reinterpret_cast<const uint32_t *>(&s_rec[w >> 1][it])[w & 1];
+        else row[2 * SYNTH_MAX_ENTRIES + e0 + (w - 2 * m)] = __float_as_uint(s_gain[w - 2 * m][it]);
     }
 }
 
@@ -432,55 +455,31 @@
 {
     extern __shared__ __align__(16) uint8_t smem[];
     const uint32_t warp = threadIdx.x >> 5, lane = threadIdx.x & 31u;
-    uint32_t *s_pvq = reinterpret_cast<uint32_t *>(smem);
-    uint2 *s_cw = reinterpret_cast<uint2 *>(s_pvq + PVQ_TABLE_WORDS);
-    uint16_t *s_row = reinterpret_cast<uint16_t *>(s_cw + PVQ_TABLE_WORDS);
-    uint8_t *s_nmax = reinterpret_cast<uint8_t *>(s_row + 16);
-    uint64_t *bar = reinterpret_cast<uint64_t *>(s_nmax + 16);
-    SynthEntry *s_ent = reinterpret_cast<SynthEntry *>(bar + 2);
-    float *s_rows = reinterpret_cast<float *>(reinterpret_cast<uint8_t *>(s_ent + SYNTH_MAX_ENTRIES) + (size_t)warp * SYM_EXPAND_WARP_BYTES);
-
+    float *s_rows = reinterpret_cast<float *>(smem + (size_t)warp * SYM_EXPAND_WARP_BYTES);
     const int lm = A.lm, C = A.channels, nf = 120 << lm;
-    const int ne = g_tab.synth_n_entries[lm][C - 1];
-    if (threadIdx.x == 0) {
-        mbar_init(bar, 1);
-        mbar_expect_tx(bar, 3 * PVQ_TABLE_WORDS * 4);
-        bulk_g2s(s_pvq, g_tab.pvq_u_data, PVQ_TABLE_WORDS * 4, bar);
-        bulk_g2s(s_cw, g_tab.pvq_cw_data, 2 * PVQ_TABLE_WORDS * 4, bar);
-    }
-    if (threadIdx.x < 15) s_row[threadIdx.x] = g_tab.pvq_u_row[threadIdx.x];
-    if (threadIdx.x < 16) s_nmax[threadIdx.x] = g_tab.pvq_ev_nmax[threadIdx.x];
-    {
-        const uint4 *src = reinterpret_cast<const uint4 *>(g_tab.synth_entries[lm][C - 1]);
-        uint4 *dst = reinterpret_cast<uint4 *>(s_ent);
-        for (int i = threadIdx.x; i < ne; i += blockDim.x) dst[i] = src[i];
-    }
     const uint32_t item = blockIdx.x * EXPAND_WARPS_PER_CTA + warp;
-    const bool in_range = item < A.n_items;
-    const uint32_t stream = in_range ? (A.stream_idx ? A.stream_idx[item] : item) : 0u;
-    const int32_t status = in_range ? A.status[stream] : -1;
-    const int32_t silence = in_range ? (int32_t)(A.hdr[stream].x & 1u) : 0;
-    const bool zero_frame = status == ITEM_LOST || (status >= 0 && silence != 0);
+    if (item >= A.n_items) return;
+    const uint32_t stream = A.stream_idx ? A.stream_idx[item] : item;
+    const int32_t status = A.status[stream];
+    if (status < 0) return;
+    const bool zero_frame = status == ITEM_LOST || (A.hdr[stream].x & 1u);
     const int nvec = C * nf / 4;
     for (int i = lane; i < nvec; i += 32) reinterpret_cast<float4 *>(s_rows)[i] = make_float4(0.f, 0.f, 0.f, 0.f);
-    __syncthreads();
-    mbar_wait(bar, 0);
-    if (status < 0) return;
-    float4 *coef4 = A.coef ? reinterpret_cast<float4 *>(A.coef + (size_t)stream * C * nf) : nullptr;
     int32_t *yo = A.y_out ? A.y_out + (size_t)stream * C * nf : nullptr;
     if (yo)
         for (int i = lane; i < nvec; i += 32) reinterpret_cast<int4 *>(yo)[i] = make_int4(0, 0, 0, 0);
     __syncwarp();
     if (!zero_frame) {
-        const ExpandTables T{s_pvq, s_cw, s_row, s_nmax, s_ent, &g_tab.synth_slot_entries[lm][C - 1][0][0], g_tab.synth_n_slots[lm][C - 1]};
-        const uint32_t *ip = A.idx + (size_t)stream * SYNTH_MAX_ENTRIES;
-        auto get_idx = [&](uint32_t e) { return e != 0xFFu ? __ldg(ip + e) : 0u; };
-        if (C == 2) w_expand<2>(T, lm, lane, get_idx, s_rows, nf, yo);
-        else w_expand<1>(T, lm, lane, get_idx, s_rows, nf, yo);
+        const int ne = g_tab.synth_n_entries[lm][C - 1];
+        const uint2 *rp = reinterpret_cast<const uint2 *>(A.pulse + (size_t)stream * SYNTH_PULSE_WORDS);
+        const float *gp = reinterpret_cast<const float *>(A.pulse + (size_t)stream * SYNTH_PULSE_WORDS + 2 * SYNTH_MAX_ENTRIES);
+        for (int e = lane; e < ne; e += 32) synth_scatter(g_tab.synth_entries[lm][C - 1][e], rp[e], gp[e], s_rows, nf, nf, 0, yo);
     }
     __syncwarp();
-    if (coef4)
+    if (A.coef) {
+        float4 *coef4 = reinterpret_cast<float4 *>(A.coef + (size_t)stream * C * nf);
         for (int i = lane; i < nvec; i += 32) coef4[i] = reinterpret_cast<const float4 *>(s_rows)[i];
+    }
 }
 
 __device__ __forceinline__ Celt2Tabs device_celt2_tabs()
@@ -618,7 +617,7 @@
         for (int i = lane; i < nvec; i += 32) reinterpret_cast<int4 *>(yo)[i] = make_int4(0, 0, 0, 0);
     __syncwarp();
     if (status == ITEM_OK && !(hdr.x & 1u)) {
-        const ExpandTables T{g_tab.pvq_u_data, g_tab.pvq_cw_data, g_tab.pvq_u_row, g_tab.pvq_ev_nmax, nullptr, nullptr, 0};
+        const ExpandTables T{g_tab.pvq_u_data, g_tab.pvq_cw_data, g_tab.pvq_u_row, g_tab.pvq_ev_nmax};
         if (C == 2) w_expand2<2>(T, lm, lane, A.parts + (size_t)stream * CELT2_MAX_PARTS, hdr.w, A.bande + (size_t)stream * 42, rows, nf, yo);
         else w_expand2<1>(T, lm, lane, A.parts + (size_t)stream * CELT2_MAX_PARTS, hdr.w, A.bande + (size_t)stream * 42, rows, nf, yo);
     }
```

New measurement: 1.769 million, median of 6. +7.0%, better.
